# kanyu369/ADNM-UNet

Measured on AMD Instinct MI355X. Metric: sequences/sec training ADNM-UNet 5->20x128x128, higher is better.
Workload: dtype bf16; 1 GPU; ADNM-UNet create_ADNMUNet(5,20,6) 128x128 full training step (fwd + enRainfallLoss + bwd + clip_grad_norm_ + AdamW), recipe parameters, synthetic radar frames in HBM; per_gpu_batch=4, global_batch=4, frames=5->20, parallelism=single, launch=hipGraph replay

## Files before the change

adnm-unet_amd/adnm_hip/ops.py:

```python
import math
import os
import threading

import torch

from . import lib

_DT = {torch.float32: lib.F32, torch.bfloat16: lib.BF16}

MFMA_PREC = [0]
_PREC_NAMES = {"f32": 0, "fp32": 0, "bf16": 1, "fp8": 2}


def set_mfma_precision(name):
    MFMA_PREC[0] = _PREC_NAMES[name]


def mfma_precision():
    return ("f32", "bf16", "fp8")[MFMA_PREC[0]]


class QuantTable:
    CAP = 2048

# ... 623 lines not shown
                row = ent["rows"][k]
                if row < 0:
                    return None
                return ent["shadow"].data_ptr() + off, 2, QUANT.scale_b_view(ent["dev"], row)
        return None


FOLDS = FoldRegistry()
SPLITWS = SplitWorkspaces()
SHADOWS = ShadowRegistry()
GRADS = GradRegistry()
SIDE = SideStreams()
grad_dst = GRADS.take


class _NoDefer:
    def deferring(self):
        return False

    def __enter__(self):
        return False

    def __exit__(self, *exc):
        return False


_NODEFER = _NoDefer()


def _need_gpu(t):
    if not t.is_cuda:
        raise RuntimeError("adnm_hip kernels run on the GPU only (there is no CPU fallback); got a CPU tensor")


def k_rownorm_fwd(x2, w, b, scale, shift, eps, mean, out=None):
    _need_gpu(x2)
    M, d = x2.shape
    y = out if out is not None else torch.empty((M, d), dtype=x2.dtype, device=x2.device)
    mu = torch.empty(M if mean else 1, dtype=torch.float32, device=x2.device)
    rstd = torch.empty(M, dtype=torch.float32, device=x2.device)
    px, ldx = _rows(x2)
    py, ldy = _rows(y)
    lib.call("adnm_rownorm_fwd", px, ldx, _p(_f32(w)), _p(_f32(b)), _p(scale), _p(shift), py, ldy, mu.data_ptr(),
             rstd.data_ptr(), M, d, float(eps), int(mean), _dt(x2), _stream())
    return y, mu, rstd


def k_rownorm_bwd(dy2, x2, w, b, scale, mu, rstd, mean, want_b, want_affine, dx_out=None, dres=None, shift=None, defer=False):
    M, d = x2.shape
    dev = x2.device
    dx = dx_out if dx_out is not None else torch.empty((M, d), dtype=x2.dtype, device=dev)
    dw = grad_dst(w.data_ptr(), (d,), dev)
    db = grad_dst(b.data_ptr(), (d,), dev) if want_b else None
    dsc = grad_dst(scale.data_ptr() if scale is not None else 0, (), dev) if want_affine else None
    dsh = grad_dst(shift.data_ptr() if shift is not None else 0, (), dev) if want_affine else None
    nb = lib.query("adnm_rownorm_bwd_ws_bytes", M, d)
    ws = _ws(nb, dev)
    pdy, lddy = _rows(dy2)
    px, ldx = _rows(x2)
    pdx, lddx = _rows(dx)
    pres, ldres = _rows(dres) if dres is not None else (None, 0)
    with FOLDS.defer(dev, ws) if defer else _NODEFER:
        lib.call("adnm_rownorm_bwd", pdy, lddy, px, ldx, _p(w), _p(b), _p(scale), mu.data_ptr(), rstd.data_ptr(), pdx, lddx,
                 dw.data_ptr(), _p(db), _p(dsc), _p(dsh), pres, ldres, ws.data_ptr(), nb, M, d, int(mean), _dt(x2), _stream())
    return dx, dw, db, dsc, dsh


def k_ssd_fwd(x, Bm, Cm, dt_raw, dt_bias, A_log, D, B, L, H, P, N, G, y=None, ln=None):
    _need_gpu(x)
    dev = x.device
    M = B * L
    if y is None:
        y = torch.empty((M, H * P), dtype=x.dtype, device=dev)
    kv = torch.empty((B, H, N, P), dtype=torch.float32, device=dev)
    nb = lib.query("adnm_ssd_ws_bytes", B, L, H, P, N, G)
    ws = _ws(nb, dev)
    px, ldx = _rows(x)
    pb, ldb = _rows(Bm)
    pc, ldc = _rows(Cm)
    pt, ldt = _rows(dt_raw)
    py, ldy = _rows(y)
    if ln is not None:
        lw, lb, yn, eps = ln
        mu = torch.empty(M, dtype=torch.float32, device=dev)
        rstd = torch.empty(M, dtype=torch.float32, device=dev)
        pn, ldn = _rows(yn)
        extra = (_p(_f32(lw)), _p(_f32(lb)), pn, ldn, mu.data_ptr(), rstd.data_ptr(), float(eps))
    else:
        extra = (None, None, None, 0, None, None, 0.0)
    lib.call("adnm_ssd_reduce_fwd", px, ldx, pb, ldb, pc, ldc, pt, ldt, 1, _p(_f32(dt_bias)), _p(_f32(A_log)), _p(_f32(D)), 1, py,
             ldy, kv.data_ptr(), *extra, ws.data_ptr(), nb, B, L, H, P, N, G, _dt(x), _stream())
    return (y, kv, mu, rstd) if ln is not None else (y, kv)


def k_ssd_bwd(dy, x, Bm, Cm, dt_raw, dt_bias, A_log, D, kv, dx, dBm, dCm, ddt, B, L, H, P, N, G):
    dev = x.device
    dbias = torch.empty(H, dtype=torch.float32, device=dev)
    dA = torch.empty(H, dtype=torch.float32, device=dev)
    dD = torch.empty(H, dtype=torch.float32, device=dev)
    nb = lib.query("adnm_ssd_ws_bytes", B, L, H, P, N, G)
    ws = _ws(nb, dev)
    a = []
    for t in (dy, x, Bm, Cm, dt_raw):
        a += list(_rows(t))
    g = []
    for t in (dx, dBm, dCm, ddt):
        g += list(_rows(t))
    with FOLDS.defer(dev, ws):
        lib.call("adnm_ssd_reduce_bwd", a[0], a[1], a[2], a[3], a[4], a[5], a[6], a[7], a[8], a[9], 1, _p(dt_bias), _p(A_log), _p(D), 1,
                 kv.data_ptr(), g[0], g[1], g[2], g[3], g[4], g[5], g[6], g[7], dbias.data_ptr(), dA.data_ptr(), dD.data_ptr(),
                 ws.data_ptr(), nb, B, L, H, P, N, G, _dt(x), _stream())
    return dbias, dA, dD


def k_dwconv_fwd(x, wt, bias, B, H, W, C, K, act, y=None, addend=None, chan_major=False):
    _need_gpu(x)
    if y is None:
        y = torch.empty((B * H * W, C), dtype=x.dtype, device=x.device)
    px, ldx = _rows(x)
    py, ldy = _rows(y)
    pa, lda = _rows(addend) if addend is not None else (None, 0)
    lib.call("adnm_dwconv_fwd", px, ldx, _p(_f32(wt)), _p(_f32(bias)), pa, lda, py, ldy, B, H, W, C, K, K, act, int(chan_major), _dt(x), _stream())
    return y


def k_dwconv_bwd(dy, x, wt, bias, B, H, W, C, K, act, dx=None, want_bias=False, want_w=True, chan_major=False, want_dx=True):
    dev = x.device
    if not want_dx:
        assert act == lib.ACT_NONE and want_w
    if dx is None and want_dx:
        dx = torch.empty((B * H * W, C), dtype=x.dtype, device=dev)
    dwt = torch.empty((C, K * K) if chan_major else (K * K, C), dtype=torch.float32, device=dev) if want_w else None
    db = torch.empty(C, dtype=torch.float32, device=dev) if want_bias else None
    dpre = torch.empty((B * H * W, C), dtype=x.dtype, device=dev) if act != lib.ACT_NONE else None
    nb = lib.query("adnm_dwconv_bwd_ws_bytes", B, H, W, C, K, K)
    ws = _ws(nb, dev)
    pdy, lddy = _rows(dy)
    px, ldx = _rows(x)
    pdx, lddx = _rows(dx) if dx is not None else (None, 0)
    if not want_w:
        lib.call("adnm_dwconv_bwd", pdy, lddy, px, ldx, _p(wt), _p(bias), _p(dpre), pdx, lddx, None, None, ws.data_ptr(),
                 nb, B, H, W, C, K, K, act, int(chan_major), _dt(x), _stream())
        return dx, dwt, db
    if want_dx:
        lib.call("adnm_dwconv_bwd", pdy, lddy, px, ldx, _p(wt), _p(bias), _p(dpre), pdx, lddx, None, None, ws.data_ptr(),
                 nb, B, H, W, C, K, K, act, int(chan_major), _dt(x), _stream())
    g, ldg = (dpre.data_ptr(), C) if dpre is not None else (pdy, lddy)
    pdw, pdb, dt_ = _p(dwt), _p(db), _dt(x)
    SIDE.submit(dev, (dy, x, dpre), FOLDS.defer(dev, ws, dy, x, dpre), lambda: lib.call(
        "adnm_dwconv_wgrad", g, ldg, px, ldx, pdw, pdb, ws.data_ptr(), nb, B, H, W, C, K, K, int(chan_major), dt_, _stream()))
    return dx, dwt, db


def k_haar_dwt(x, B, H, W, C, cx=1):
    _need_gpu(x)
    h2, w2 = (H + 1) // 2, (W + 1) // 2
    y = torch.empty((B * h2 * w2, 4 * C), dtype=x.dtype, device=x.device)
    px, ldx = _rows(x)
    lib.call("adnm_haar_dwt", px, ldx, cx, y.data_ptr(), B, H, W, C, _dt(x), _stream())
    return y


def k_wt_level(x, B, H, W, C, cx, taps, K, flip=False):
    _need_gpu(x)
    h2, w2 = (H + 1) // 2, (W + 1) // 2
    sub = torch.empty((B * h2 * w2, 4 * C), dtype=torch.float32, device=x.device)
    tag = torch.empty_like(sub)
    px, ldx = _rows(x)
    lib.call("adnm_wt_level", px, ldx, cx, _f32(taps).data_ptr(), sub.data_ptr(), tag.data_ptr(), B, H, W, C, K, int(flip), _stream())
    return sub, tag


def k_haar_idwt(s, ll_add, B, H, W, C, y_add=(), up=()):
    _need_gpu(s)
    assert s.is_contiguous() and (ll_add is None or ll_add.is_contiguous()) and len(up) <= 2 and all(u.is_contiguous() and u.dtype == s.dtype for u in up)
    adds = [a if a.is_contiguous() else a.contiguous() for a in y_add if a is not None]
    assert len(adds) <= 2
    adds += [None] * (2 - len(adds))
    ups = list(up) + [None] * (2 - len(up))
    y = torch.empty((B * H * W, C), dtype=s.dtype, device=s.device)
    lib.call("adnm_haar_idwt", s.data_ptr(), _p(ups[0]), _p(ups[1]), _p(ll_add), _p(adds[0]), _p(adds[1]), y.data_ptr(), B, H, W, C, _dt(s), _stream())
    return y


def k_haar_synthesis(bands, shapes, B, C, y_add=()):
    n = len(bands)
    nxt, top = None, n
    while top > 0:
        lo = max(top - 3, 0)
        hh, ww = shapes[lo]
        nxt = k_haar_idwt(bands[lo], nxt, B, hh, ww, C, y_add=y_add if lo == 0 else (), up=tuple(bands[lo + 1:top]))
        top = lo
    return nxt


def k_instnorm_fwd(x, scale, shift, B, HW, C, eps, act):
    _need_gpu(x)
    assert x.is_contiguous()
    dev = x.device
    y = torch.empty_like(x)
    mu = torch.empty((B, C), dtype=torch.float32, device=dev)
    rstd = torch.empty((B, C), dtype=torch.float32, device=dev)
    nb = lib.query("adnm_instnorm_ws_bytes", B, HW, C)
    ws = _ws(nb, dev)
    lib.call("adnm_instnorm_fwd", x.data_ptr(), _p(scale), _p(shift), y.data_ptr(), mu.data_ptr(), rstd.data_ptr(), ws.data_ptr(), nb,
             B, HW, C, float(eps), act, _dt(x), _stream())
    return y, mu, rstd


def k_instnorm_bwd(dy, x, scale, shift, mu, rstd, B, HW, C, act, want_affine=True):
    dev = x.device
    assert dy.is_contiguous() and x.is_contiguous()
    dx = torch.empty_like(x)
    dsc = grad_dst(scale.data_ptr() if scale is not None else 0, (), dev) if want_affine else None
    dsh = grad_dst(shift.data_ptr() if shift is not None else 0, (), dev) if want_affine else None
    nb = lib.query("adnm_instnorm_ws_bytes", B, HW, C)
    ws = _ws(nb, dev)
    with FOLDS.defer(dev, ws):
        lib.call("adnm_instnorm_bwd", dy.data_ptr(), x.data_ptr(), _p(scale), _p(shift), mu.data_ptr(), rstd.data_ptr(), dx.data_ptr(),
                 _p(dsc), _p(dsh), ws.data_ptr(), nb, B, HW, C, act, _dt(x), _stream())
    return dx, dsc, dsh


def k_gate_fwd(h, F):
    _need_gpu(h)
    M = h.shape[0]
    y = torch.empty((M, F), dtype=h.dtype, device=h.device)
    ph, ldh = _rows(h)
    lib.call("adnm_gate_fwd", ph, ldh, y.data_ptr(), F, M, F, _dt(h), _stream())
    return y


def k_gate_bwd(dy, h, F):
    M = h.shape[0]
    dh = torch.empty((M, 2 * F), dtype=h.dtype, device=h.device)
    pdy, lddy = _rows(dy)
    ph, ldh = _rows(h)
    lib.call("adnm_gate_bwd", pdy, lddy, ph, ldh, dh.data_ptr(), 2 * F, M, F, _dt(h), _stream())
    return dh


def tap_major(w):
    c = w.shape[0]
    return w.reshape(c, -1).t().contiguous().float()


class RowNormFn(torch.autograd.Function):

    @staticmethod
    def forward(ctx, x, w, b, scale, shift, eps, mean):
        shp = x.shape
        x2 = x.reshape(-1, shp[-1])
        if x2.stride(-1) != 1:
            x2 = x2.contiguous()
        y, mu, rstd = k_rownorm_fwd(x2, w, b, scale, shift, eps, mean)
        ctx.save_for_backward(x2, w, b, scale, mu, rstd)
        ctx.mean, ctx.shp, ctx.has_shift, ctx.shift = mean, shp, shift is not None, shift
        return y.view(shp)

    @staticmethod
    def backward(ctx, dy):
        x2, w, b, scale, mu, rstd = ctx.saved_tensors
        dy2 = dy.reshape(-1, ctx.shp[-1])
        if dy2.stride(-1) != 1:
            dy2 = dy2.contiguous()
        dx, dw, db, dsc, dsh = k_rownorm_bwd(dy2, x2, w, b, scale, mu, rstd, ctx.mean, b is not None,
                                            scale is not None or ctx.has_shift, shift=ctx.shift, defer=True)
        return (dx.view(ctx.shp), dw, db, dsc if scale is not None else None, dsh if ctx.has_shift else None, None, None)


def rownorm(x, w, b=None, scale=None, shift=None, eps=1e-5, mean=True):
    return RowNormFn.apply(x, w, b, scale, shift, eps, mean)


class RowNormTapFn(torch.autograd.Function):

    @staticmethod
    def forward(ctx, x, w, b, scale, shift, eps, mean):
        shp = x.shape
        x2 = x.reshape(-1, shp[-1])
        if x2.stride(-1) != 1:
            x2 = x2.contiguous()
        y, mu, rstd = k_rownorm_fwd(x2, w, b, scale, shift, eps, mean)
        ctx.save_for_backward(x2, w, b, scale, mu, rstd)
        ctx.mean, ctx.shp, ctx.has_shift, ctx.shift = mean, shp, shift is not None, shift
        ctx.set_materialize_grads(False)
        return y.view(shp), x

    @staticmethod
    def backward(ctx, dy, dres):
        x2, w, b, scale, mu, rstd = ctx.saved_tensors
        d = ctx.shp[-1]
        if dy is None:
            return (dres, None, None, None, None, None, None)
        dy2 = dy.reshape(-1, d)
        if dy2.stride(-1) != 1:
            dy2 = dy2.contiguous()
        if dres is not None:
            dres = dres.reshape(-1, d)
            if dres.stride(-1) != 1:
                dres = dres.contiguous()
        dx, dw, db, dsc, dsh = k_rownorm_bwd(dy2, x2, w, b, scale, mu, rstd, ctx.mean, b is not None,
                                            scale is not None or ctx.has_shift, dres=dres, shift=ctx.shift, defer=True)
        return (dx.view(ctx.shp), dw, db, dsc if scale is not None else None, dsh if ctx.has_shift else None, None, None)


def rownorm_tap(x, w, b=None, scale=None, shift=None, eps=1e-5, mean=True):
    return RowNormTapFn.apply(x, w, b, scale, shift, eps, mean)


class CatMixFn(torch.autograd.Function):

    @staticmethod
    def forward(ctx, x, r, f, a1, a2, a3, a4):
        shp = x.shape
        d = shp[-1]
        rows = lambda t: t.reshape(-1, d) if t.reshape(-1, d).stride(-1) == 1 else t.reshape(-1, d).contiguous()
        x2, r2 = rows(x), rows(r)
        f2 = rows(f) if f is not None else None
        _need_gpu(x2)
        M = x2.shape[0]
        y = torch.empty((M, 2 * d), dtype=x.dtype, device=x.device)
        (px, ldx), (pr, ldr) = _rows(x2), _rows(r2)
        pf, ldf = _rows(f2) if f2 is not None else (None, 0)
        lib.call("adnm_catmix_fwd", px, ldx, pr, ldr, pf, ldf, _p(a1), _p(a2), _p(a3), _p(a4), y.data_ptr(), M, d, _dt(y), _stream())
        ctx.save_for_backward(x2, r2, f2, a1, a2, a3, a4)
        ctx.shp = shp
        return y.view(*shp[:-1], 2 * d)

    @staticmethod
    def backward(ctx, dy):
        x2, r2, f2, a1, a2, a3, a4 = ctx.saved_tensors
        M, d = x2.shape
        g = dy.reshape(M, 2 * d)
        g = g if g.stride(-1) == 1 else g.contiguous()
        need = ctx.needs_input_grad
        mk = lambda on: torch.empty((M, d), dtype=x2.dtype, device=x2.device) if on else None
        dx, dr, df = mk(need[0]), mk(need[1]), mk(need[2] and f2 is not None)
        da = torch.empty(4, dtype=torch.float32, device=x2.device)
        nb = lib.query("adnm_catmix_bwd_ws_bytes", M, d)
        ws = _ws(nb, x2.device)
        (pg, ldg), (px, ldx), (pr, ldr) = _rows(g), _rows(x2), _rows(r2)
        pf, ldf = _rows(f2) if f2 is not None else (None, 0)
        with FOLDS.defer(x2.device, ws):
            lib.call("adnm_catmix_bwd", pg, ldg, px, ldx, pr, ldr, pf, ldf, _p(a1), _p(a2), _p(a3), _p(a4), _p(dx), _p(dr), _p(df), da.data_ptr(),
                     ws.data_ptr(), nb, M, d, _dt(g), _stream())
        v = lambda t: t.view(ctx.shp) if t is not None else None
        s = lambda a, i: da[i].view_as(a) if a is not None else None
        return v(dx), v(dr), v(df), s(a1, 0), s(a2, 1), s(a3 if f2 is not None else None, 2), s(a4 if f2 is not None else None, 3)


def _unsupported(op, why):
    raise RuntimeError(f"adnm_hip {op}: {why} (the HIP path has no PyTorch fallback)")


def catmix(x, r, f, a1, a2, a3=None, a4=None):
    _need_gpu(x)
    d = x.shape[-1]
    if r.shape != x.shape or (f is not None and f.shape != x.shape):
        _unsupported("catmix", f"operands must share one shape, got {tuple(x.shape)}, {tuple(r.shape)}" + (f", {tuple(f.shape)}" if f is not None else ""))
    if d % 4 or x.dtype not in _DT or any(a is not None and a.numel() != 1 for a in (a1, a2, a3, a4)):
        _unsupported("catmix", f"needs a channel count that is a multiple of 4 (got {d}), fp32/bf16 tokens and 1-element mixing parameters")
    return CatMixFn.apply(x, r, f, a1, a2, a3, a4)


class SSDReduceFn(torch.autograd.Function):

    @staticmethod
    def forward(ctx, x, Bm, Cm, dt_raw, dt_bias, A_log, D, G):
        B, L, H, P = x.shape
        N = Bm.shape[-1] // G
        M = B * L
        xs, bs, cs, ts = x.reshape(M, H * P), Bm.reshape(M, -1), Cm.reshape(M, -1), dt_raw.reshape(M, H)
        xs, bs, cs, ts = [t if t.stride(-1) == 1 else t.contiguous() for t in (xs, bs, cs, ts)]
        y, kv = k_ssd_fwd(xs, bs, cs, ts, dt_bias, A_log, D, B, L, H, P, N, G)
        ctx.save_for_backward(xs, bs, cs, ts, dt_bias, A_log, D, kv)
        ctx.dims = (B, L, H, P, N, G)
        return y.view(B, L, H, P)

    @staticmethod
    def backward(ctx, dy):
        xs, bs, cs, ts, dt_bias, A_log, D, kv = ctx.saved_tensors
        B, L, H, P, N, G = ctx.dims
        M = B * L
        dy2 = dy.reshape(M, H * P)
        dy2 = dy2 if dy2.stride(-1) == 1 else dy2.contiguous()
        dx, dB, dC, ddt = (torch.empty_like(t, memory_format=torch.contiguous_format) for t in (xs, bs, cs, ts))
        dbias, dA, dD = k_ssd_bwd(dy2, xs, bs, cs, ts, dt_bias, A_log, D, kv, dx, dB, dC, ddt, B, L, H, P, N, G)
        return dx.view(B, L, H, P), dB.view(B, L, -1), dC.view(B, L, -1), ddt.view(B, L, H), dbias, dA, dD, None


def ssd_reduce(x, Bm, Cm, dt_raw, dt_bias, A_log, D, groups=1):
# ... 129 lines not shown
            else:
                dm = k_haar_dwt(cur, B, hh, ww, C, cx)
            dtags.append(dm)
            cur, cx = dm, 4
        dlw = [None] * levels
        for i in range(levels - 1, -1, -1):
            hh, ww = shapes[i]
            h2, w2 = (hh + 1) // 2, (ww + 1) // 2
            if fused:
                _, dlw[i], _ = k_dwconv_bwd(dtags[i], subs[i], level_wt[i], None, B, h2, w2, 4 * C, K, lib.ACT_NONE, want_dx=False)
            else:
                dsub, dlw[i], _ = k_dwconv_bwd(dtags[i], subs[i], level_wt[i], None, B, h2, w2, 4 * C, K, lib.ACT_NONE, want_dx=need_dx)
                dsubs.insert(0, dsub)
        if not need_dx:
            dx = None
        elif levels == 0:
            dx = dxb if dalias is None else dxb + dalias.reshape(B * H * W, C)
        else:
            dx = k_haar_synthesis(dsubs, shapes, B, C, y_add=(dxb, dalias.reshape(B * H * W, C) if dalias is not None else None))
        return (dx.view(B, H * W, C) if dx is not None else None, None, None, None, dbase, dbb, *dlw)


def wtconv(x, H, W, K, base_wt, base_bias, level_wts, tap=False):
    y, xa = WTConvFn.apply(x, H, W, K, base_wt, base_bias, *level_wts)
    return (y, xa) if tap else y


class ADNMixerFn(torch.autograd.Function):

    @staticmethod
    def forward(ctx, u, w_in, taps, tb, dt_bias, A_log, D, ln_w, ln_b, w_out, H, W, P, N, scan_chunk=0, scan_groups=2, qkeys=(None, None),
                narrow=(None, None, None, None)):
        n_in = (narrow[0].data_ptr(), 1 if narrow[0].dtype == torch.bfloat16 else 2, narrow[1]) if narrow[0] is not None else None
        n_out = (narrow[2].data_ptr(), 1 if narrow[2].dtype == torch.bfloat16 else 2, narrow[3]) if narrow[2] is not None else None
        Bsz, L, dm = u.shape
        M = Bsz * L
        di = w_out.shape[1] // 2
        cx = taps.shape[1] - di
        nh = di // P
        u2 = u.reshape(M, dm)
        u2 = u2 if u2.is_contiguous() else u2.contiguous()
        st = low_storage(M, [(w_in.shape[0], dm), (dm, 2 * di), (2 * di, dm), (dm, w_in.shape[0])]) if scan_chunk == 0 else u.dtype
        proj = k_linear(u2, w_in, None, qkey=qkeys[0], out_dtype=st, narrow=n_in)
        wide = torch.empty((M, 2 * di + cx), dtype=st, device=u.device)
        cat, xbc = wide[:, :2 * di], wide[:, 2 * di:]
        k_dwconv_fwd(proj[:, :di + cx], taps, tb, Bsz, H, W, di + cx, 3, lib.ACT_SILU, y=wide[:, di:])
        if scan_chunk == 0:
            if di == 64:
                y, kv, mu, rstd = k_ssd_fwd(xbc[:, :di], xbc[:, di:di + 2 * N], xbc[:, di + 2 * N:], proj[:, di + cx:], dt_bias, A_log, D,
                                            Bsz, L, nh, P, N, 2, ln=(ln_w, ln_b, cat[:, :di], 1e-5))
            else:
                y, kv = k_ssd_fwd(xbc[:, :di], xbc[:, di:di + 2 * N], xbc[:, di + 2 * N:], proj[:, di + cx:], dt_bias, A_log, D,
                                  Bsz, L, nh, P, N, 2)
                mu = None
        else:
            y = torch.empty((M, di), dtype=u.dtype, device=u.device)
            Ns = N // scan_groups
            kv = torch.stack([k_ssd_scan_fwd(xbc[:, e * P:di], 2 * P, xbc[:, di + e * N:di + (e + 1) * N], xbc[:, di + 2 * N + e * N:di + 2 * N + (e + 1) * N],
                                             proj[:, di + cx + e:], 2, dt_bias[e:], A_log[e:], D[e:], 2, y[:, e * P:], 2 * P, Bsz, L, nh // 2, P, Ns,
                                             scan_groups, scan_chunk, e == 1) for e in (0, 1)])
            mu = None
        if mu is None:
            _, mu, rstd = k_rownorm_fwd(y, ln_w, ln_b, None, None, 1e-5, True, out=cat[:, :di])
        out = k_linear(cat, w_out, None, qkey=qkeys[1], out_dtype=u.dtype, narrow=n_out)
        ctx.save_for_backward(u2, w_in, taps, tb, dt_bias, A_log, D, ln_w, ln_b, w_out, proj, wide, y, kv, mu, rstd)
        ctx.dims = (Bsz, L, dm, H, W, P, N, di, cx, nh, scan_chunk, scan_groups)
        ctx.qkeys = qkeys
        ctx.narrow = (n_in, n_out, narrow)
        return out.view(Bsz, L, dm)

    @staticmethod
    def backward(ctx, dout):
        (u2, w_in, taps, tb, dt_bias, A_log, D, ln_w, ln_b, w_out, proj, wide, y, kv, mu, rstd) = ctx.saved_tensors
        Bsz, L, dm, H, W, P, N, di, cx, nh, scan_chunk, scan_groups = ctx.dims
        M = Bsz * L
        cat, xbc = wide[:, :2 * di], wide[:, 2 * di:]
        do = dout.reshape(M, dm)
        do = do if do.is_contiguous() else do.contiguous()
        dw_out, _ = k_linear_dw(do, cat, False)
        dwide = torch.empty_like(wide)
        dcat, dxbc = dwide[:, :2 * di], dwide[:, 2 * di:]
        k_linear_dx(do, w_out, out=dcat, qkey=ctx.qkeys[1], narrow=ctx.narrow[1])
        dy, dln_w, dln_b, _, _ = k_rownorm_bwd(dcat[:, :di], y, ln_w, ln_b, None, mu, rstd, True, True, False, defer=True)
        dproj = torch.empty_like(proj)
        if scan_chunk == 0:
            ddtb, dA, dD = k_ssd_bwd(dy, xbc[:, :di], xbc[:, di:di + 2 * N], xbc[:, di + 2 * N:], proj[:, di + cx:], dt_bias, A_log, D, kv,
                                     dxbc[:, :di], dxbc[:, di:di + 2 * N], dxbc[:, di + 2 * N:], dproj[:, di + cx:], Bsz, L, nh, P, N, 2)
        else:
            Ns = N // scan_groups
            parts = [k_ssd_scan_bwd(dy[:, e * P:], 2 * P, xbc[:, e * P:di], 2 * P, xbc[:, di + e * N:di + (e + 1) * N],
                                    xbc[:, di + 2 * N + e * N:di + 2 * N + (e + 1) * N], proj[:, di + cx + e:], 2, dt_bias[e:], A_log[e:], D[e:], 2,
                                    kv[e], dxbc[:, e * P:di], 2 * P, dxbc[:, di + e * N:di + (e + 1) * N],
                                    dxbc[:, di + 2 * N + e * N:di + 2 * N + (e + 1) * N], dproj[:, di + cx + e:], 2, Bsz, L, nh // 2, P, Ns,
                                    scan_groups, scan_chunk, e == 1) for e in (0, 1)]
            ddtb, dA, dD = (torch.stack((parts[0][k], parts[1][k]), dim=1).reshape(nh) for k in range(3))
        _, dtaps, dtb = k_dwconv_bwd(dwide[:, di:], proj[:, :di + cx], taps, tb, Bsz, H, W, di + cx, 3, lib.ACT_SILU, dx=dproj[:, :di + cx],
                                     want_bias=tb is not None)
        du = k_linear_dx(dproj, w_in, qkey=ctx.qkeys[0], out_dtype=u2.dtype, narrow=ctx.narrow[0])
        dw_in, _ = k_linear_dw(dproj, u2, False)
        return (du.view(Bsz, L, dm), dw_in, dtaps, dtb, ddtb, dA, dD, dln_w, dln_b, dw_out, None, None, None, None, None, None, None, None)


def adn_mixer(u, w_in, taps, tb, dt_bias, A_log, D, ln_w, ln_b, w_out, H, W, P, N, scan_chunk=0, scan_groups=2, qkeys=(None, None),
              narrow=(None, None, None, None)):
    return ADNMixerFn.apply(u, w_in, taps, tb, dt_bias, A_log, D, ln_w, ln_b, w_out, H, W, P, N, scan_chunk, scan_groups, qkeys, narrow)


class FeedForwardFn(torch.autograd.Function):

    @staticmethod
    def forward(ctx, x, w_in, b_in, dw, b_dw, w_out, b_out, H, W):
        B, L, d = x.shape
        M = B * L
        F4, F2 = w_in.shape[0], w_out.shape[1]
        x2 = x.reshape(M, d)
        x2 = x2 if x2.is_contiguous() else x2.contiguous()
        w_in, w_out = w_in.contiguous(), w_out.contiguous()
        wt = dw.reshape(F4, 9)
        if wt.dtype != torch.float32 or not wt.is_contiguous():
            wt = wt.contiguous().float()
        st = low_storage(M, [(F4, d), (d, F4), (d, F2), (F2, d)])
        h1 = k_linear(x2, w_in, b_in, out_dtype=st)
        h2 = k_dwconv_fwd(h1, wt, b_dw, B, H, W, F4, 3, lib.ACT_NONE, chan_major=True)
        g = k_gate_fwd(h2, F2)
        out = k_linear(g, w_out, b_out, out_dtype=x.dtype)
        ctx.save_for_backward(x2, w_in, b_in, wt, b_dw, w_out, b_out, h1, h2, g)
        ctx.meta = (B, L, d, H, W, F4, F2, dw.shape)
        return out.view(B, L, w_out.shape[0])

    @staticmethod
    def backward(ctx, dout):
        x2, w_in, b_in, wt, b_dw, w_out, b_out, h1, h2, g = ctx.saved_tensors
        B, L, d, H, W, F4, F2, dwshape = ctx.meta
        M = B * L
        do = dout.reshape(M, w_out.shape[0])
        do = do if do.is_contiguous() else do.contiguous()
        dg = k_linear_dx(do, w_out, out_dtype=g.dtype)
        dw_out, db_out = k_linear_dw(do, g, b_out is not None, w_out.data_ptr(), b_out.data_ptr() if b_out is not None else 0)
        dh2 = k_gate_bwd(dg, h2, F2)
        dh1, dwt, db_dw = k_dwconv_bwd(dh2, h1, wt, b_dw, B, H, W, F4, 3, lib.ACT_NONE, want_bias=b_dw is not None, chan_major=True)
        dx = k_linear_dx(dh1, w_in, out_dtype=x2.dtype) if ctx.needs_input_grad[0] else None
        dw_in, db_in = k_linear_dw(dh1, x2, b_in is not None, w_in.data_ptr(), b_in.data_ptr() if b_in is not None else 0)
        return (dx.view(B, L, d) if dx is not None else None, dw_in, db_in, dwt.view(dwshape), db_dw, dw_out, db_out, None, None)


def feedforward(x, w_in, b_in, dw, b_dw, w_out, b_out, H, W):
    _need_gpu(x)
    F4, F2 = w_in.shape[0], w_out.shape[1]
    if (x.dtype != torch.float32 or x.dim() != 3 or x.shape[1] != H * W or F4 != 2 * F2 or F2 % 4 or tuple(dw.shape) != (F4, 1, 3, 3)
            or w_in.shape[1] != x.shape[-1]):
        _unsupported("feedforward", f"is 1x1 d->4d, depthwise 3x3, gelu*sigmoid gate, 1x1 2d->d on fp32 (B, H*W, d) tokens with 8 | 4d, got "
                                    f"{x.dtype} {tuple(x.shape)}, weights {tuple(w_in.shape)}, {tuple(dw.shape)}, {tuple(w_out.shape)}")
    return FeedForwardFn.apply(x, w_in, b_in, dw, b_dw, w_out, b_out, H, W)


class LinCombFn(torch.autograd.Function):

    @staticmethod
    def forward(ctx, gamma, *args):
        n = len(args) // 2
        xs, ss = args[:n], args[n:]
        shp = xs[0].shape
        C = shp[-1]
        x2 = []
        for x in xs:
            t = x.reshape(-1, C)
            x2.append(t if t.stride(-1) == 1 else t.contiguous())
        M = x2[0].shape[0]
        y = torch.empty((M, C), dtype=xs[0].dtype, device=xs[0].device)
        ptr = [(None, 0)] * 3
        for i, t in enumerate(x2):
            ptr[i] = _rows(t)
        sp = [_p(s) for s in ss] + [None] * (3 - n)
        _need_gpu(x2[0])
        lib.call("adnm_lincomb_fwd", ptr[0][0], ptr[0][1], ptr[1][0], ptr[1][1], ptr[2][0], ptr[2][1], sp[0], sp[1], sp[2], _p(gamma),
                 y.data_ptr(), C, M, C, _dt(y), _stream())
        ctx.save_for_backward(gamma, *x2, *[s for s in ss if s is not None])
        ctx.meta = (n, shp, [s is not None for s in ss])
        return y.view(shp)

    @staticmethod
    def backward(ctx, dy):
        n, shp, has_s = ctx.meta
        saved = ctx.saved_tensors
        gamma, x2 = saved[0], saved[1:1 + n]
        it = iter(saved[1 + n:])
        ss = [next(it) if h else None for h in has_s]
        C = shp[-1]
        M = x2[0].shape[0]
        dev = x2[0].device
        g = dy.reshape(M, C)
        g = g if g.stride(-1) == 1 else g.contiguous()
        need_x = ctx.needs_input_grad[1:1 + n]
        dxs = [torch.empty((M, C), dtype=x2[0].dtype, device=dev) if need_x[i] else None for i in range(n)]
        dss, accmask = [], 0
        for i in range(n):
            if ss[i] is None:
                dss.append(None)
                continue
            t, acc = GRADS.take_accumulating(ss[i].data_ptr(), ss[i].shape, dev)
            dss.append(t)
            accmask |= (1 << (1 + i)) if acc else 0
        dgamma = grad_dst(gamma.data_ptr(), gamma.shape, dev) if gamma is not None else None
        nb = lib.query("adnm_lincomb_bwd_ws_bytes", M, C)
        ws = _ws(nb, dev)
        xp = [_rows(t) for t in x2] + [(None, 0)] * (3 - n)
        dxp = [(_p(t), C) for t in dxs] + [(None, 0)] * (3 - n)
        sp = [_p(s) for s in ss] + [None] * (3 - n)
        dsp = [_p(s) for s in dss] + [None] * (3 - n)
        pg, ldg = _rows(g)
        with FOLDS.defer(dev, ws) as deferred:
            if accmask:
                assert deferred, "an accumulating gradient claim needs the deferred fold queue"
                lib.load().adnm_foldq_accumulate_next(accmask)
            lib.call("adnm_lincomb_bwd", pg, ldg, xp[0][0], xp[0][1], xp[1][0], xp[1][1], xp[2][0], xp[2][1], sp[0], sp[1], sp[2], _p(gamma),
                     dxp[0][0], dxp[0][1], dxp[1][0], dxp[1][1], dxp[2][0], dxp[2][1], dsp[0], dsp[1], dsp[2], _p(dgamma), ws.data_ptr(), nb,
                     M, C, _dt(g), _stream())
        return (dgamma, *[d.view(shp) if d is not None else None for d in dxs],
                *[None if (accmask >> (1 + i)) & 1 else d for i, d in enumerate(dss)])


def lincomb(xs, scalars, gamma=None):
    C = xs[0].shape[-1]
    _need_gpu(xs[0])
    if gamma is None and C % 4 and xs[0].numel() % 4 == 0 and all(x.shape == xs[0].shape and x.is_contiguous() for x in xs):
        shp = xs[0].shape
        return lincomb([x.view(-1, 4) for x in xs], scalars).view(shp)
    if C % 4 or C > 2048 or not 1 <= len(xs) <= 3 or any(s is not None and s.numel() != 1 for s in scalars):
        _unsupported("lincomb", f"needs 1-3 operands with 4 | C <= 2048 channels and 1-element scalars, got {len(xs)} operands, C={C}")
    return LinCombFn.apply(gamma, *xs, *scalars)


class MixNormFn(torch.autograd.Function):

    @staticmethod
    def forward(ctx, gamma, w, b, scale, shift, eps, mean, x0, x1, s0, s1):
        shp = x0.shape
        d = shp[-1]
        rows = lambda t: t.reshape(-1, d) if t.reshape(-1, d).stride(-1) == 1 else t.reshape(-1, d).contiguous()
        a2, b2 = rows(x0), rows(x1)
        _need_gpu(a2)
        M, dev = a2.shape[0], a2.device
        x = torch.empty((M, d), dtype=torch.float32, device=dev)
        xn = torch.empty((M, d), dtype=torch.float32, device=dev)
        mu = torch.empty(M, dtype=torch.float32, device=dev) if mean else None
        rstd = torch.empty(M, dtype=torch.float32, device=dev)
        (pa, lda), (pb, ldb) = _rows(a2), _rows(b2)
        lib.call("adnm_mixnorm_fwd", pa, lda, pb, ldb, _p(s0), _p(s1), _p(gamma), w.data_ptr(), _p(b), _p(scale), _p(shift), x.data_ptr(), d,
                 xn.data_ptr(), d, _p(mu), rstd.data_ptr(), M, d, float(eps), int(mean), _stream())
        ctx.save_for_backward(gamma, w, b, scale, a2, b2, s0, s1, mu, rstd)
        ctx.meta = (shp, mean, shift)
        ctx.set_materialize_grads(False)
        return xn.view(shp), x.view(shp)

    @staticmethod
    def backward(ctx, dxn, dres):
        gamma, w, b, scale, a2, b2, s0, s1, mu, rstd = ctx.saved_tensors
        shp, mean, shift = ctx.meta
        M, d = a2.shape
        dev = a2.device
        rows = lambda t: t.reshape(M, d) if t.reshape(M, d).stride(-1) == 1 else t.reshape(M, d).contiguous()
        if dxn is None:
            dxn = torch.zeros((M, d), dtype=torch.float32, device=dev)
        dxn = rows(dxn)
        dres = rows(dres) if dres is not None else None
        need = ctx.needs_input_grad
        dx0 = torch.empty((M, d), dtype=torch.float32, device=dev) if need[7] else None
        dx1 = torch.empty((M, d), dtype=torch.float32, device=dev) if need[8] else None
        dss, accmask = [], 0
        for i, sk in enumerate((s0, s1)):
            if sk is None:
                dss.append(None)
                continue
            t, acc = GRADS.take_accumulating(sk.data_ptr(), sk.shape, dev)
            dss.append(t)
            accmask |= (1 << (1 + i)) if acc else 0
        dgamma = grad_dst(gamma.data_ptr(), gamma.shape, dev) if gamma is not None else None
        dw = grad_dst(w.data_ptr(), (d,), dev)
        db = grad_dst(b.data_ptr(), (d,), dev) if b is not None else None
        affine = scale is not None or shift is not None
        dsc = grad_dst(scale.data_ptr() if scale is not None else 0, (), dev) if affine else None
        dsh = grad_dst(shift.data_ptr() if shift is not None else 0, (), dev) if affine else None
        nb = lib.query("adnm_mixnorm_bwd_ws_bytes", M, d)
        ws = _ws(nb, dev)
        (pg, ldg), (pa, lda), (pb, ldb) = _rows(dxn), _rows(a2), _rows(b2)
        pr, ldr = _rows(dres) if dres is not None else (None, 0)
        with FOLDS.defer(dev, ws) as deferred:
            if accmask:
                assert deferred, "an accumulating gradient claim needs the deferred fold queue"
                lib.load().adnm_foldq_accumulate_next(accmask)
            lib.call("adnm_mixnorm_bwd", pg, ldg, pr, ldr, pa, lda, pb, ldb, _p(s0), _p(s1), _p(gamma), w.data_ptr(), _p(b), _p(scale), _p(mu),
                     rstd.data_ptr(), _p(dx0), d, _p(dx1), d, _p(dss[0]), _p(dss[1]), _p(dgamma), dw.data_ptr(), _p(db), _p(dsc), _p(dsh),
                     ws.data_ptr(), nb, M, d, int(mean), _stream())
        ds = [None if (accmask >> (1 + i)) & 1 else t for i, t in enumerate(dss)]
        return (dgamma, dw, db, dsc if scale is not None else None, dsh if shift is not None else None, None, None,
                dx0.view(shp) if dx0 is not None else None, dx1.view(shp) if dx1 is not None else None, ds[0], ds[1])


def mixnorm(xs, scalars, gamma, w, b=None, scale=None, shift=None, eps=1e-5, mean=True):
    _need_gpu(xs[0])
    d = xs[0].shape[-1]
    if (len(xs) != 2 or xs[0].shape != xs[1].shape or any(x.dtype != torch.float32 for x in xs) or d % 4 or d > 1024
            or any(sk is not None and sk.numel() != 1 for sk in scalars)):
        _unsupported("mixnorm", f"mixes two same-shape fp32 token tensors with 4 | d <= 1024 channels and 1-element scalars, got "
                                f"{[tuple(x.shape) for x in xs]} {[x.dtype for x in xs]}")
    return MixNormFn.apply(gamma, w, b, scale, shift, eps, mean, xs[0], xs[1], scalars[0], scalars[1])
# ... 1115 lines not shown
```

adnm-unet_amd/csrc/dwconv.hip:

```cpp
#include "adnm_common.h"

namespace {

constexpr int kBlock = 256;
constexpr int TW = 4;

__device__ __forceinline__ float4 f4zero() { return make_float4(0.f, 0.f, 0.f, 0.f); }
__device__ __forceinline__ void fma4(float4& a, const float4& w, const float4& x) {
  a.x = fmaf(w.x, x.x, a.x); a.y = fmaf(w.y, x.y, a.y); a.z = fmaf(w.z, x.z, a.z); a.w = fmaf(w.w, x.w, a.w);
}
__device__ __forceinline__ float4 apply_act(float4 v, int act) {
  if (act == ADNM_ACT_SILU) return make_float4(siluf_(v.x), siluf_(v.y), siluf_(v.z), siluf_(v.w));
  if (act == ADNM_ACT_GELU) return make_float4(geluf_(v.x), geluf_(v.y), geluf_(v.z), geluf_(v.w));
  return v;
}
__device__ __forceinline__ float4 apply_act_grad(float4 v, int act) {
  if (act == ADNM_ACT_SILU) return make_float4(silu_gradf_(v.x), silu_gradf_(v.y), silu_gradf_(v.z), silu_gradf_(v.w));
  if (act == ADNM_ACT_GELU) return make_float4(gelu_gradf_(v.x), gelu_gradf_(v.y), gelu_gradf_(v.z), gelu_gradf_(v.w));
  return make_float4(1.f, 1.f, 1.f, 1.f);
}

template <typename T>
struct CVec;
template <>
struct CVec<float> {
  static constexpr int N = 4, Q = 1;
  float4 q[1];
};
template <>
struct CVec<uint16_t> {
  static constexpr int N = 8, Q = 2;
  float4 q[2];
};
template <typename T>
__device__ __forceinline__ CVec<T> cv_zero() {
  CVec<T> v;
#pragma unroll
  for (int i = 0; i < CVec<T>::Q; ++i) v.q[i] = f4zero();
  return v;
}
__device__ __forceinline__ CVec<float> cv_ld(const float* p) {
  CVec<float> v;
  v.q[0] = *reinterpret_cast<const float4*>(p);
  return v;
}
__device__ __forceinline__ CVec<uint16_t> cv_ld(const uint16_t* p) {
  const uint4 r = *reinterpret_cast<const uint4*>(p);
  CVec<uint16_t> v;
  v.q[0] = make_float4(__uint_as_float(r.x << 16), __uint_as_float(r.x & 0xffff0000u), __uint_as_float(r.y << 16), __uint_as_float(r.y & 0xffff0000u));
  v.q[1] = make_float4(__uint_as_float(r.z << 16), __uint_as_float(r.z & 0xffff0000u), __uint_as_float(r.w << 16), __uint_as_float(r.w & 0xffff0000u));
  return v;
}
__device__ __forceinline__ void cv_st(float* p, const CVec<float>& v) { *reinterpret_cast<float4*>(p) = v.q[0]; }
__device__ __forceinline__ void cv_st(uint16_t* p, const CVec<uint16_t>& v) {
  uint4 r;
  r.x = (uint32_t)f32_to_bf16(v.q[0].x) | ((uint32_t)f32_to_bf16(v.q[0].y) << 16);
  r.y = (uint32_t)f32_to_bf16(v.q[0].z) | ((uint32_t)f32_to_bf16(v.q[0].w) << 16);
  r.z = (uint32_t)f32_to_bf16(v.q[1].x) | ((uint32_t)f32_to_bf16(v.q[1].y) << 16);
  r.w = (uint32_t)f32_to_bf16(v.q[1].z) | ((uint32_t)f32_to_bf16(v.q[1].w) << 16);
  *reinterpret_cast<uint4*>(p) = r;
}
template <typename T>
__device__ __forceinline__ CVec<T> cv_ldf(const float* p) {
  CVec<T> v;
#pragma unroll
  for (int i = 0; i < CVec<T>::Q; ++i) v.q[i] = *reinterpret_cast<const float4*>(p + 4 * i);
  return v;
}
template <typename T>
__device__ __forceinline__ void cv_stf(float* p, const CVec<T>& v) {
#pragma unroll
  for (int i = 0; i < CVec<T>::Q; ++i) *reinterpret_cast<float4*>(p + 4 * i) = v.q[i];
}
template <typename T>
__device__ __forceinline__ void cv_fma(CVec<T>& a, const CVec<T>& w, const CVec<T>& x) {
#pragma unroll
  for (int i = 0; i < CVec<T>::Q; ++i) fma4(a.q[i], w.q[i], x.q[i]);
}
template <typename T>
__device__ __forceinline__ void cv_add(CVec<T>& a, const CVec<T>& x) {
#pragma unroll
  for (int i = 0; i < CVec<T>::Q; ++i) a.q[i].x += x.q[i].x, a.q[i].y += x.q[i].y, a.q[i].z += x.q[i].z, a.q[i].w += x.q[i].w;
}

template <typename T, int K, int MODE, bool WCM>
__global__ __launch_bounds__(kBlock) void dwconv_kernel(const T* __restrict__ x, int64_t ldx, const float* __restrict__ wgt,
                                                        const float* __restrict__ bias, const T* __restrict__ aux,
                                                        int64_t ldaux, T* __restrict__ y, int64_t ldy, int B, int H, int W,
                                                        int C, int act) {
  constexpr int R = K / 2, N = CVec<T>::N, Q = CVec<T>::Q;
  using V = CVec<T>;
  const int C4 = C / N;
  const int WT = (W + TW - 1) / TW;
  const int64_t total = (int64_t)B * H * WT * C4;
  const unsigned nb = gridDim.x, q8 = nb >> 3, r8 = nb & 7, xcd = blockIdx.x & 7, loc = blockIdx.x >> 3;
  const unsigned bid = (xcd < r8 ? xcd * (q8 + 1) : r8 * (q8 + 1) + (xcd - r8) * q8) + loc;
  const int64_t idx = (int64_t)bid * kBlock + threadIdx.x;
  if (idx >= total) return;
  const int cg = (int)(idx % C4);
  int64_t t = idx / C4;
  const int wt = (int)(t % WT);
  t /= WT;
  const int h = (int)(t % H);
  const int b = (int)(t / H);
  const int c = cg * N;
  const int w0 = wt * TW;
  float wcmv[WCM ? N * K * K : 1];
  if (WCM) {
#pragma unroll
    for (int q = 0; q < N * K * K / 4; ++q) {
      const float4 t4 = *reinterpret_cast<const float4*>(wgt + (int64_t)c * (K * K) + 4 * q);
      wcmv[4 * q] = t4.x; wcmv[4 * q + 1] = t4.y; wcmv[4 * q + 2] = t4.z; wcmv[4 * q + 3] = t4.w;
    }
  }
  V acc[TW];
#pragma unroll
  for (int i = 0; i < TW; ++i) acc[i] = cv_zero<T>();
#pragma unroll
  for (int i = 0; i < K; ++i) {
    const int hh = h + i - R;
    if (hh < 0 || hh >= H) continue;
    const T* xr = x + ((int64_t)b * H + hh) * W * ldx + c;
    V row[TW + K - 1];
#pragma unroll
    for (int j = 0; j < TW + K - 1; ++j) {
      const int ww = w0 + j - R;
      row[j] = (ww >= 0 && ww < W) ? cv_ld(xr + (int64_t)ww * ldx) : cv_zero<T>();
    }
#pragma unroll
    for (int j = 0; j < K; ++j) {
      const int tap = (MODE == 2) ? ((K - 1 - i) * K + (K - 1 - j)) : (i * K + j);
      V wv;
      if (WCM) {
#pragma unroll
        for (int qq = 0; qq < Q; ++qq)
          wv.q[qq] = make_float4(wcmv[(WCM ? (4 * qq) * K * K : 0) + tap * WCM], wcmv[(WCM ? (4 * qq + 1) * K * K : 0) + tap * WCM],
                                 wcmv[(WCM ? (4 * qq + 2) * K * K : 0) + tap * WCM], wcmv[(WCM ? (4 * qq + 3) * K * K : 0) + tap * WCM]);
      } else {
        wv = cv_ldf<T>(wgt + (int64_t)tap * C + c);
      }
#pragma unroll
      for (int p = 0; p < TW; ++p) cv_fma(acc[p], wv, row[p + j]);
    }
  }
  V bv = cv_zero<T>();
  if (MODE != 2 && bias) bv = cv_ldf<T>(bias + c);
#pragma unroll
  for (int p = 0; p < TW; ++p) {
    const int ww = w0 + p;
    if (ww >= W) break;
    const int64_t pix = ((int64_t)b * H + h) * W + ww;
    V v = acc[p];
    if (MODE == 0) {
      cv_add(v, bv);
#pragma unroll
      for (int qq = 0; qq < Q; ++qq) v.q[qq] = apply_act(v.q[qq], act);
      if (aux) cv_add(v, cv_ld(aux + pix * ldaux + c));
    } else if (MODE == 1) {
      cv_add(v, bv);
      const V d = cv_ld(aux + pix * ldaux + c);
#pragma unroll
      for (int qq = 0; qq < Q; ++qq) {
        const float4 g = apply_act_grad(v.q[qq], act);
        v.q[qq] = make_float4(d.q[qq].x * g.x, d.q[qq].y * g.y, d.q[qq].z * g.z, d.q[qq].w * g.w);
      }
    }
    cv_st(y + pix * ldy + c, v);
  }
}

constexpr int kWgSlices = 2;

template <typename T, int K>
__device__ __forceinline__ void dwconv_wgrad_body(const T* __restrict__ dpre, int64_t ldd, const T* __restrict__ x, int64_t ldx,
                                                  float* __restrict__ part, int B, int H, int W, int C, int cgb, int wcm, const int bx,
                                                  const int by, const int nby) {
  constexpr int R = K / 2;
  constexpr int NT = K * K, N = CVec<T>::N;
  using V = CVec<T>;
  const int C4 = C / N;
  __shared__ __attribute__((aligned(16))) float red[K][K + 1][64][N];
  const int wv = threadIdx.x >> 6;
  const int i = wv % K;
  const int sl = wv / K;
  const int lane = threadIdx.x & 63;
  const int cgl = lane & (cgb - 1);
  const int slot = lane / cgb;
  const int slots = 64 / cgb;
  const int cg = bx * cgb + cgl;
  const bool cv = cg < C4;
  const int c = cv ? cg * N : 0;
  const int WT = (W + TW - 1) / TW;
  const int64_t tiles = (int64_t)B * H * WT;
  V aw[K];
  V ab = cv_zero<T>();
#pragma unroll
  for (int k = 0; k < K; ++k) aw[k] = cv_zero<T>();
  if (cv) {
    const unsigned nb = (unsigned)nby, q8 = nb >> 3, r8 = nb & 7, xcd = (unsigned)by & 7, loc = (unsigned)by >> 3;
    const int64_t bid = (xcd < r8 ? xcd * (q8 + 1) : r8 * (q8 + 1) + (xcd - r8) * q8) + loc;
    const int64_t tpb = (tiles + nb - 1) / nb;
    const int64_t tbeg = bid * tpb, tend = (tbeg + tpb < tiles) ? tbeg + tpb : tiles;
    const int64_t stride = (int64_t)slots * kWgSlices;
    for (int64_t t0 = tbeg + sl * slots + slot; t0 < tend; t0 += 2 * stride) {
      V g[2][TW], row[2][TW + K - 1];
      bool live[2];
#pragma unroll
      for (int u = 0; u < 2; ++u) {
        const int64_t t = t0 + u * stride;
        const int wt = (int)(t % WT);
        const int h = (int)((t / WT) % H);
        const int b = (int)(t / ((int64_t)WT * H));
        const int hh = h + i - R;
        live[u] = t < tend && hh >= 0 && hh < H;
        const int w0 = wt * TW;
#pragma unroll
        for (int p = 0; p < TW; ++p) {
          const int ww = w0 + p;
          g[u][p] = (live[u] && ww < W) ? cv_ld(dpre + (((int64_t)b * H + h) * W + ww) * ldd + c) : cv_zero<T>();
        }
        const T* xr = x + ((int64_t)b * H + (live[u] ? hh : 0)) * W * ldx + c;
#pragma unroll
        for (int j = 0; j < TW + K - 1; ++j) {
          const int ww = w0 + j - R;
          row[u][j] = (live[u] && ww >= 0 && ww < W) ? cv_ld(xr + (int64_t)ww * ldx) : cv_zero<T>();
        }
      }
#pragma unroll
      for (int u = 0; u < 2; ++u) {
        if (i == R) {
#pragma unroll
          for (int p = 0; p < TW; ++p) cv_add(ab, g[u][p]);
        }
#pragma unroll
        for (int j = 0; j < K; ++j)
#pragma unroll
          for (int p = 0; p < TW; ++p) cv_fma(aw[j], g[u][p], row[u][p + j]);
      }
    }
  }
#pragma unroll
  for (int j = 0; j <= K; ++j) {
    V& v = j < K ? aw[j] : ab;
#pragma unroll
    for (int qq = 0; qq < V::Q; ++qq) {
      v.q[qq].x = wave_sum_from(v.q[qq].x, cgb); v.q[qq].y = wave_sum_from(v.q[qq].y, cgb);
      v.q[qq].z = wave_sum_from(v.q[qq].z, cgb); v.q[qq].w = wave_sum_from(v.q[qq].w, cgb);
    }
  }
  if (sl == 1) {
#pragma unroll
    for (int j = 0; j <= K; ++j) cv_stf<T>(&red[i][j][lane][0], j < K ? aw[j] : ab);
  }
  __syncthreads();
  if (sl == 0) {
    float* dst = part + (int64_t)by * (NT + 1) * C;
#pragma unroll
    for (int j = 0; j <= K; ++j) {
      if (j == K && i != R) break;
      V v = j < K ? aw[j] : ab;
      cv_add(v, cv_ldf<T>(&red[i][j][lane][0]));
      if (lane < cgb && cv) {
        if (wcm && j < K) {
          float* q = dst + (int64_t)c * NT + i * K + j;
#pragma unroll
          for (int qq = 0; qq < V::Q; ++qq) {
            q[(4 * qq) * NT] = v.q[qq].x; q[(4 * qq + 1) * NT] = v.q[qq].y; q[(4 * qq + 2) * NT] = v.q[qq].z; q[(4 * qq + 3) * NT] = v.q[qq].w;
          }
        } else {
          cv_stf<T>(dst + (int64_t)(j < K ? i * K + j : NT) * C + c, v);
        }
      }
    }
  }
}

template <typename T, int K>
__global__ __launch_bounds__(64 * K * kWgSlices) void dwconv_wgrad_kernel(const T* __restrict__ dpre, int64_t ldd, const T* __restrict__ x,
                                                              int64_t ldx, float* __restrict__ part, int B, int H, int W, int C,
                                                              int cgb, int wcm) {
  dwconv_wgrad_body<T, K>(dpre, ldd, x, ldx, part, B, H, W, C, cgb, wcm, (int)blockIdx.x, (int)blockIdx.y, (int)gridDim.y);
}

constexpr int kMaxWg = 16;
struct WgLeaf {
  const float* dpre;
  int64_t ldd;
  const float* x;
  int64_t ldx;
  float* part;
  int B, H, W, C, cgb, wcm, gx, npb;
};
struct MultiWg {
  int count, blk_end[kMaxWg];
  WgLeaf p[kMaxWg];
};
template <int K>
__global__ __launch_bounds__(64 * K * kWgSlices) void dwconv_wgrad_multi_kernel(MultiWg by_value) {
  (void)by_value;
  const auto& m = *(const __attribute__((address_space(4))) MultiWg*)__builtin_amdgcn_kernarg_segment_ptr();
  int k = 0;
  while (k + 1 < m.count && (int)blockIdx.x >= m.blk_end[k]) ++k;
  const int lin = (int)blockIdx.x - (k ? m.blk_end[k - 1] : 0);
  const int gx = m.p[k].gx;
  dwconv_wgrad_body<float, K>(m.p[k].dpre, m.p[k].ldd, m.p[k].x, m.p[k].ldx, m.p[k].part, m.p[k].B, m.p[k].H, m.p[k].W, m.p[k].C, m.p[k].cgb,
                              m.p[k].wcm, lin % gx, lin / gx, m.p[k].npb);
}

template <typename T>
__global__ __launch_bounds__(kBlock) void dwconv_wgrad3_roll_kernel(const T* __restrict__ dpre, int64_t ldd, const T* __restrict__ x, int64_t ldx,
                                                                    float* __restrict__ part, int B, int H, int W, int C, int cgb, int SEG,
                                                                    int nseg, int wcm) {
  constexpr int K = 3, NT = 9, N = CVec<T>::N;
  using V = CVec<T>;
  __shared__ __attribute__((aligned(16))) float red[kBlock / 64 - 1][NT + 1][64][N];
  const int C4 = C / N;
  const int WT = (W + TW - 1) / TW;
  const int cgl = threadIdx.x & (cgb - 1), sp = threadIdx.x / cgb, spb = kBlock / cgb;
  const int cg = blockIdx.x * cgb + cgl;
  const int64_t S = (int64_t)B * nseg * WT, sidx = (int64_t)blockIdx.y * spb + sp;
  const bool cv = cg < C4, live = cv && sidx < S;
// ... 144 lines not shown
  float* dst = part + (int64_t)by * (NT + 1) * C;
#pragma unroll
  for (int k = 0; k <= NT; ++k) {
    float4 v = k < NT ? aw[k] : ab;
    v.x = wave_sum_from(v.x, cgb), v.y = wave_sum_from(v.y, cgb), v.z = wave_sum_from(v.z, cgb), v.w = wave_sum_from(v.w, cgb);
    if (wave > 0) *reinterpret_cast<float4*>(&red[wave - 1][lane][0]) = v;
    __syncthreads();
    if (wave == 0 && lane < cgb) {
#pragma unroll
      for (int wv = 0; wv < kBlock / 64 - 1; ++wv) {
        const float4 o = *reinterpret_cast<const float4*>(&red[wv][lane][0]);
        v.x += o.x, v.y += o.y, v.z += o.z, v.w += o.w;
      }
      if (cv) {
        if (wcm && k < NT) {
          float* q = dst + (int64_t)c * NT + k;
          q[0] = v.x, q[NT] = v.y, q[2 * NT] = v.z, q[3 * NT] = v.w;
        } else {
          *reinterpret_cast<float4*>(dst + (int64_t)k * C + c) = v;
        }
      }
    }
    __syncthreads();
  }
}

__global__ __launch_bounds__(kBlock) void dwconv_wgrad5_walk_kernel(const float* __restrict__ dpre, int64_t ldd, const float* __restrict__ x, int64_t ldx,
                                                                    float* __restrict__ part, int B, int H, int W, int C, int cgb, int SEG, int nseg,
                                                                    int wcm) {
  dwconv_wgrad_walk_body<5, kWalkTW>(dpre, ldd, x, ldx, part, B, H, W, C, cgb, SEG, nseg, wcm, (int)blockIdx.x, (int)blockIdx.y);
}

struct WalkLeaf {
  const float* dpre;
  int64_t ldd;
  const float* x;
  int64_t ldx;
  float* part;
  int B, H, W, C, cgb, wcm, gx, npb, seg, nseg;
};
struct MultiWalk {
  int count, blk_end[kMaxWg];
  WalkLeaf p[kMaxWg];
};
__global__ __launch_bounds__(kBlock) void dwconv_wgrad5_walk_multi_kernel(MultiWalk by_value) {
  (void)by_value;
  const auto& m = *(const __attribute__((address_space(4))) MultiWalk*)__builtin_amdgcn_kernarg_segment_ptr();
  int k = 0;
  while (k + 1 < m.count && (int)blockIdx.x >= m.blk_end[k]) ++k;
  const int lin = (int)blockIdx.x - (k ? m.blk_end[k - 1] : 0);
  const int gx = m.p[k].gx;
  dwconv_wgrad_walk_body<5, kWalkTW>(m.p[k].dpre, m.p[k].ldd, m.p[k].x, m.p[k].ldx, m.p[k].part, m.p[k].B, m.p[k].H, m.p[k].W, m.p[k].C, m.p[k].cgb,
                                     m.p[k].seg, m.p[k].nseg, m.p[k].wcm, lin % gx, lin / gx);
}

struct WGeo {
  int cgb, gx, npb, rows;
  int seg, nseg;
};
WGeo wgeo(int64_t B, int64_t H, int64_t W, int64_t C, int K, int cn = 4) {
  WGeo g;
  const int64_t C4 = C / cn;
  g.cgb = 1;
  while (g.cgb < 64 && g.cgb < C4) g.cgb <<= 1;
  g.gx = (int)adnm_cdiv(C4, g.cgb);
  const int slots = 64 / g.cgb;
  const int64_t tiles = B * H * adnm_cdiv(W, TW);
  static const int grouped_tpl = [] {
    const char* e = getenv("ADNM_DW_WG_TPL");
    const int v = e ? atoi(e) : 0;
    return v > 0 ? v : 16;
  }();
  const bool walker = K == 3 && H * W >= 128 * 128;
  const int64_t tmax = !walker && adnm_leafq_active() ? grouped_tpl : 8;
  int64_t tpl = (tiles * g.gx) / ((int64_t)slots * 256);
  if (tmax > 8 && tpl >= 8) tpl = tmax;
  tpl = tpl < 2 ? 2 : (tpl > tmax ? tmax : tpl);
  int64_t npb = adnm_cdiv(tiles, (int64_t)slots * tpl);
  int64_t cap = (4 << 20) / ((int64_t)(K * K + 1) * C * 4);
  if (cap > 1024) cap = 1024;
  if (cap < 32) cap = 32;
  if (npb > cap) npb = cap;
  if (npb < 1) npb = 1;
  g.npb = (int)npb;
  g.rows = g.npb;
  g.seg = g.nseg = 0;
  if (walker) {
    const int64_t WT = adnm_cdiv(W, TW);
    int64_t seg = (H * B * WT * C4) / 65536;
    seg = seg < 2 ? 2 : (seg > 16 ? 16 : seg);
    if (seg > H) seg = H;
    g.seg = (int)seg;
    g.nseg = (int)adnm_cdiv(H, seg);
    const int64_t S = B * g.nseg * WT;
    g.npb = (int)adnm_cdiv(S, kBlock / g.cgb);
    g.rows = g.npb;
  }
  return g;
}

WGeo wgeo_walk5(int64_t B, int64_t H, int64_t W, int64_t C) {
  WGeo g;
  const int64_t C4 = C / 4;
  g.cgb = 1;
  while (g.cgb < 64 && g.cgb < C4) g.cgb <<= 1;
  g.gx = (int)adnm_cdiv(C4, g.cgb);
  const int64_t WT = adnm_cdiv(W, kWalkTW);
  static const int seg_min = [] {
    const char* e = getenv("ADNM_DW_WALK_SEG");
    const int v = e ? atoi(e) : 0;
    return v > 0 ? v : 16;
  }();
  int64_t seg = (H * B * WT * C4) / 65536;
  seg = seg < seg_min ? seg_min : (seg > 64 ? 64 : seg);
  if (seg > H) seg = H;
  g.seg = (int)seg;
  g.nseg = (int)adnm_cdiv(H, seg);
  g.npb = (int)adnm_cdiv(B * g.nseg * WT, kBlock / g.cgb);
  g.rows = g.npb;
  return g;
}

int check(const char* who, const void* x, int64_t B, int64_t H, int64_t W, int64_t C, int KH, int KW, int act, int dtype) {
  ADNM_REQUIRE(x, "%s: null pointer", who);
  ADNM_REQUIRE(B > 0 && H > 0 && W > 0 && C > 0 && C % 4 == 0, "%s: shape B=%lld H=%lld W=%lld C=%lld (C must be a multiple of 4)", who,
               (long long)B, (long long)H, (long long)W, (long long)C);
  ADNM_REQUIRE(KH == KW && (KH == 3 || KH == 5), "%s: kernel %dx%d not in {3x3, 5x5}", who, KH, KW);
  ADNM_REQUIRE(act >= ADNM_ACT_NONE && act <= ADNM_ACT_GELU, "%s: bad activation %d", who, act);
  ADNM_REQUIRE(dtype == ADNM_F32 || dtype == ADNM_BF16, "%s: bad dtype %d", who, dtype);
  ADNM_REQUIRE(dtype == ADNM_F32 || C % 8 == 0, "%s: bf16 tokens move 8 channels (16 bytes) per lane: C=%lld must be a multiple of 8", who, (long long)C);
  ADNM_REQUIRE(B * H * W * C < (1ll << 40), "%s: tensor too large", who);
  return ADNM_OK;
}

template <typename T, int MODE>
void launch_conv(const void* x, int64_t ldx, const float* wgt, const float* bias, const void* aux, int64_t ldaux, void* y, int64_t ldy,
                 int64_t B, int64_t H, int64_t W, int64_t C, int K, int act, int wcm, hipStream_t st) {
  const int64_t total = B * H * adnm_cdiv(W, TW) * (C / CVec<T>::N);
  const unsigned grid = (unsigned)adnm_cdiv(total, kBlock);
#define ADNM_DWCONV(KK, WCMV)                                                                                                       \
  dwconv_kernel<T, KK, MODE, WCMV><<<grid, kBlock, 0, st>>>((const T*)x, ldx, wgt, bias, (const T*)aux, ldaux, (T*)y, ldy, (int)B, (int)H, \
                                                            (int)W, (int)C, act)
  ADNM_PROF(K == 3 ? "dwconv_k3" : "dwconv_k5", st, (double)sizeof(T) * B * H * W * C * (MODE == 1 ? 3 : (aux ? 3 : 2)));
  if (K == 3) {
    if (wcm) ADNM_DWCONV(3, true);
    else ADNM_DWCONV(3, false);
  } else {
    if (wcm) ADNM_DWCONV(5, true);
    else ADNM_DWCONV(5, false);
  }
#undef ADNM_DWCONV
}

template <typename T>
void launch_wgrad(const void* dpre, int64_t ldd, const void* x, int64_t ldx, float* part, float* dwgt, float* dbias, int64_t B, int64_t H,
                  int64_t W, int64_t C, int K, int wcm, hipStream_t st) {
  if (K == 5 && sizeof(T) == 4) {
    const WGeo g = wgeo_walk5(B, H, W, C);
    static_assert(sizeof(WalkLeaf) <= sizeof(AdnmLeaf::args), "WalkLeaf must fit a leaf record");
    WalkLeaf w{(const float*)dpre, ldd, (const float*)x, ldx, part, (int)B, (int)H, (int)W, (int)C, g.cgb, wcm, g.gx, g.npb, g.seg, g.nseg};
    AdnmLeaf leaf;
    leaf.kind = ADNM_LEAF_DWCONV_WGRAD_K5, leaf.grid = g.gx * g.npb, leaf.prec = 0, leaf.prof = "dwconv_wgrad_k5", leaf.bytes = 4.0 * B * H * W * C * 2;
    memcpy(leaf.args, &w, sizeof(w));
    if (!adnm_leafq_push(leaf)) {
      ADNM_PROF("dwconv_wgrad_k5", st, 4.0 * B * H * W * C * 2);
      dwconv_wgrad5_walk_kernel<<<dim3(g.gx, g.npb), kBlock, 0, st>>>((const float*)dpre, ldd, (const float*)x, ldx, part, (int)B, (int)H, (int)W, (int)C, g.cgb,
                                                                     g.seg, g.nseg, wcm);
    }
    adnm_launch_fold("dwconv_wgrad_fold", part, g.rows, 26 * (int)C, {dwgt, 25 * (int)C}, {dbias, (int)C}, {nullptr, 0}, {nullptr, 0}, st);
    return;
  }
  const WGeo g = wgeo(B, H, W, C, K, CVec<T>::N);
  const dim3 grid(g.gx, g.npb);
  if (K == 3 && g.seg > 0)
    { ADNM_PROF("dwconv_wgrad_k3", st, (double)sizeof(T) * B * H * W * C * 2); dwconv_wgrad3_roll_kernel<T><<<grid, kBlock, 0, st>>>((const T*)dpre, ldd, (const T*)x, ldx, part, (int)B, (int)H, (int)W, (int)C, g.cgb, g.seg, g.nseg, wcm); }
  else {
    bool queued = false;
    if (sizeof(T) == 4) {
      static_assert(sizeof(WgLeaf) <= sizeof(AdnmLeaf::args), "WgLeaf must fit a leaf record");
      WgLeaf w{(const float*)dpre, ldd, (const float*)x, ldx, part, (int)B, (int)H, (int)W, (int)C, g.cgb, wcm, (int)g.gx, (int)g.npb};
      AdnmLeaf leaf;
      leaf.kind = K == 3 ? ADNM_LEAF_DWCONV_WGRAD_K3 : ADNM_LEAF_DWCONV_WGRAD_K5, leaf.grid = (int)(g.gx * g.npb), leaf.prec = 0;
      leaf.prof = K == 3 ? "dwconv_wgrad_k3" : "dwconv_wgrad_k5", leaf.bytes = 4.0 * B * H * W * C * 2;
      memcpy(leaf.args, &w, sizeof(w));
      queued = adnm_leafq_push(leaf);
    }
    if (!queued) {
      if (K == 3)
        { ADNM_PROF("dwconv_wgrad_k3", st, (double)sizeof(T) * B * H * W * C * 2); dwconv_wgrad_kernel<T, 3><<<grid, 64 * 3 * kWgSlices, 0, st>>>((const T*)dpre, ldd, (const T*)x, ldx, part, (int)B, (int)H, (int)W, (int)C, g.cgb, wcm); }
      else
        { ADNM_PROF("dwconv_wgrad_k5", st, (double)sizeof(T) * B * H * W * C * 2); dwconv_wgrad_kernel<T, 5><<<grid, 64 * 5 * kWgSlices, 0, st>>>((const T*)dpre, ldd, (const T*)x, ldx, part, (int)B, (int)H, (int)W, (int)C, g.cgb, wcm); }
    }
  }
  adnm_launch_fold("dwconv_wgrad_fold", part, g.rows, (K * K + 1) * (int)C, {dwgt, K * K * (int)C}, {dbias, (int)C}, {nullptr, 0}, {nullptr, 0}, st);
}

}

extern "C" int adnm_dwconv_fwd(const void* x, int64_t ldx, const float* wgt, const float* bias, const void* addend, int64_t ldadd,
                               void* y, int64_t ldy, int64_t B, int64_t H, int64_t W, int64_t C, int KH, int KW, int act, int wlayout,
                               int dtype, adnm_stream_t stream) {
  if (int rc = check("dwconv_fwd", x, B, H, W, C, KH, KW, act, dtype)) return rc;
  ADNM_REQUIRE(wgt && y, "dwconv_fwd: null pointer");
  ADNM_REQUIRE(wlayout == 0 || wlayout == 1, "dwconv_fwd: weight layout %d not in {0 tap-major, 1 channel-major}", wlayout);
  const int al = dtype == ADNM_BF16 ? 8 : 4;
  ADNM_REQUIRE(ldx >= C && ldy >= C && ldx % al == 0 && ldy % al == 0 && (!addend || (ldadd >= C && ldadd % al == 0)) &&
                   ((uintptr_t)x | (uintptr_t)y | (uintptr_t)addend) % 16 == 0,
               "dwconv_fwd: pixel strides must be >= C, rows and strides 16-byte aligned");
  hipStream_t st = (hipStream_t)stream;
  if (dtype == ADNM_F32) launch_conv<float, 0>(x, ldx, wgt, bias, addend, ldadd, y, ldy, B, H, W, C, KH, act, wlayout, st);
  else launch_conv<uint16_t, 0>(x, ldx, wgt, bias, addend, ldadd, y, ldy, B, H, W, C, KH, act, wlayout, st);
  ADNM_CHECK_LAUNCH("dwconv_fwd");
  return ADNM_OK;
}

extern "C" int64_t adnm_dwconv_bwd_ws_bytes(int64_t B, int64_t H, int64_t W, int64_t C, int KH, int KW) {
  if (B <= 0 || H <= 0 || W <= 0 || C < 4) return 0;
  int64_t rows = wgeo(B, H, W, C, KH).rows;
  if (C % 8 == 0) {
    const int64_t r8 = wgeo(B, H, W, C, KH, 8).rows;
    rows = r8 > rows ? r8 : rows;
  }
  if (KH == 5) {
    const int64_t r5 = wgeo_walk5(B, H, W, C).rows;
    rows = r5 > rows ? r5 : rows;
  }
  return rows * (KH * KW + 1) * C * (int64_t)sizeof(float);
}

extern "C" int adnm_dwconv_bwd(const void* dy, int64_t lddy, const void* x, int64_t ldx, const float* wgt, const float* bias,
                               void* dpre, void* dx, int64_t lddx, float* dwgt, float* dbias, void* ws, int64_t ws_bytes, int64_t B,
                               int64_t H, int64_t W, int64_t C, int KH, int KW, int act, int wlayout, int dtype, adnm_stream_t stream) {
  if (int rc = check("dwconv_bwd", x, B, H, W, C, KH, KW, act, dtype)) return rc;
  ADNM_REQUIRE(dy && wgt && dx, "dwconv_bwd: null pointer");
  ADNM_REQUIRE(wlayout == 0 || wlayout == 1, "dwconv_bwd: weight layout %d not in {0 tap-major, 1 channel-major}", wlayout);
  ADNM_REQUIRE(act == ADNM_ACT_NONE || dpre, "dwconv_bwd: dpre scratch required when an activation is fused");
  const int al = dtype == ADNM_BF16 ? 8 : 4;
  ADNM_REQUIRE(ldx >= C && lddy >= C && lddx >= C && ldx % al == 0 && lddy % al == 0 && lddx % al == 0 &&
                   ((uintptr_t)x | (uintptr_t)dy | (uintptr_t)dx | (uintptr_t)dpre) % 16 == 0,
               "dwconv_bwd: pixel strides must be >= C, rows and strides 16-byte aligned");
  if (!ws || ws_bytes < adnm_dwconv_bwd_ws_bytes(B, H, W, C, KH, KW)) {
    adnm_set_error("dwconv_bwd: workspace %lld < %lld bytes", (long long)ws_bytes, (long long)adnm_dwconv_bwd_ws_bytes(B, H, W, C, KH, KW));
    return ADNM_EWORKSPACE;
  }
  hipStream_t st = (hipStream_t)stream;
  const void* g = dy;
  int64_t ldg = lddy;
  if (dtype == ADNM_F32) {
    if (act != ADNM_ACT_NONE) {
      launch_conv<float, 1>(x, ldx, wgt, bias, dy, lddy, dpre, C, B, H, W, C, KH, act, wlayout, st);
      g = dpre; ldg = C;
    }
    launch_conv<float, 2>(g, ldg, wgt, nullptr, nullptr, 0, dx, lddx, B, H, W, C, KH, 0, wlayout, st);
    if (dwgt) launch_wgrad<float>(g, ldg, x, ldx, (float*)ws, dwgt, dbias, B, H, W, C, KH, wlayout, st);
  } else {
    if (act != ADNM_ACT_NONE) {
      launch_conv<uint16_t, 1>(x, ldx, wgt, bias, dy, lddy, dpre, C, B, H, W, C, KH, act, wlayout, st);
      g = dpre; ldg = C;
    }
    launch_conv<uint16_t, 2>(g, ldg, wgt, nullptr, nullptr, 0, dx, lddx, B, H, W, C, KH, 0, wlayout, st);
    if (dwgt) launch_wgrad<uint16_t>(g, ldg, x, ldx, (float*)ws, dwgt, dbias, B, H, W, C, KH, wlayout, st);
  }
  ADNM_CHECK_LAUNCH("dwconv_bwd");
  return ADNM_OK;
}

extern "C" int adnm_dwconv_wgrad(const void* g, int64_t ldg, const void* x, int64_t ldx, float* dwgt, float* dbias, void* ws, int64_t ws_bytes,
                                 int64_t B, int64_t H, int64_t W, int64_t C, int KH, int KW, int wlayout, int dtype, adnm_stream_t stream) {
  if (int rc = check("dwconv_wgrad", x, B, H, W, C, KH, KW, ADNM_ACT_NONE, dtype)) return rc;
  ADNM_REQUIRE(g && dwgt, "dwconv_wgrad: null pointer");
  ADNM_REQUIRE(wlayout == 0 || wlayout == 1, "dwconv_wgrad: weight layout %d not in {0 tap-major, 1 channel-major}", wlayout);
  const int al = dtype == ADNM_BF16 ? 8 : 4;
  ADNM_REQUIRE(ldx >= C && ldg >= C && ldx % al == 0 && ldg % al == 0 && ((uintptr_t)x | (uintptr_t)g) % 16 == 0,
               "dwconv_wgrad: pixel strides must be >= C, rows and strides 16-byte aligned");
  if (!ws || ws_bytes < adnm_dwconv_bwd_ws_bytes(B, H, W, C, KH, KW)) {
    adnm_set_error("dwconv_wgrad: workspace %lld < %lld bytes", (long long)ws_bytes, (long long)adnm_dwconv_bwd_ws_bytes(B, H, W, C, KH, KW));
    return ADNM_EWORKSPACE;
  }
  hipStream_t st = (hipStream_t)stream;
  if (dtype == ADNM_F32) launch_wgrad<float>(g, ldg, x, ldx, (float*)ws, dwgt, dbias, B, H, W, C, KH, wlayout, st);
  else launch_wgrad<uint16_t>(g, ldg, x, ldx, (float*)ws, dwgt, dbias, B, H, W, C, KH, wlayout, st);
  ADNM_CHECK_LAUNCH("dwconv_wgrad");
  return ADNM_OK;
}


int adnm_dwconv_wgrad_launch_multi(const AdnmLeaf* const* items, int n, int K, hipStream_t st) {
  if (K == 5) {
    for (int i = 0; i < n;) {
      MultiWalk m;
      m.count = 0;
      int blocks = 0;
      double bytes = 0;
      for (; i < n && m.count < kMaxWg; ++i) {
        memcpy(&m.p[m.count], items[i]->args, sizeof(WalkLeaf));
        blocks += items[i]->grid;
        m.blk_end[m.count++] = blocks;
        bytes += items[i]->bytes;
      }
      for (int k = m.count; k < kMaxWg; ++k) m.blk_end[k] = blocks;
      ADNM_PROF("dwconv_wgrad_k5", st, bytes);
      dwconv_wgrad5_walk_multi_kernel<<<(unsigned)blocks, kBlock, 0, st>>>(m);
    }
    ADNM_CHECK_LAUNCH("dwconv_wgrad (grouped)");
    return ADNM_OK;
  }
  for (int i = 0; i < n;) {
    MultiWg m;
    m.count = 0;
    int blocks = 0;
    double bytes = 0;
    for (; i < n && m.count < kMaxWg; ++i) {
      memcpy(&m.p[m.count], items[i]->args, sizeof(WgLeaf));
      blocks += items[i]->grid;
      m.blk_end[m.count++] = blocks;
      bytes += items[i]->bytes;
    }
    for (int k = m.count; k < kMaxWg; ++k) m.blk_end[k] = blocks;
    ADNM_PROF("dwconv_wgrad_k3", st, bytes);
    dwconv_wgrad_multi_kernel<3><<<(unsigned)blocks, 64 * 3 * kWgSlices, 0, st>>>(m);
  }
  ADNM_CHECK_LAUNCH("dwconv_wgrad (grouped)");
  return ADNM_OK;
}
```

adnm-unet_amd/csrc/elementwise.hip:

```cpp
#include "adnm_common.h"

namespace {
constexpr int kBlock = 256;

template <typename T>
__global__ __launch_bounds__(kBlock) void gate_fwd_kernel(const T* __restrict__ h, int64_t ldh, T* __restrict__ y, int64_t ldy,
                                                          int64_t M, int F) {
  const int F4 = F >> 2;
  const int64_t total = M * F4;
  for (int64_t i = (int64_t)blockIdx.x * kBlock + threadIdx.x; i < total; i += (int64_t)gridDim.x * kBlock) {
    const int64_t m = i / F4;
    const int f = (int)(i % F4) * 4;
    const float4 a = Io<T>::ld4(h + m * ldh + f), b = Io<T>::ld4(h + m * ldh + F + f);
    Io<T>::st4(y + m * ldy + f, make_float4(geluf_(a.x) * sigmoidf_(b.x), geluf_(a.y) * sigmoidf_(b.y), geluf_(a.z) * sigmoidf_(b.z),
                                            geluf_(a.w) * sigmoidf_(b.w)));
  }
}

template <typename T>
__global__ __launch_bounds__(kBlock) void gate_bwd_kernel(const T* __restrict__ dy, int64_t lddy, const T* __restrict__ h, int64_t ldh,
                                                          T* __restrict__ dh, int64_t lddh, int64_t M, int F) {
  const int F4 = F >> 2;
  const int64_t total = M * F4;
  for (int64_t i = (int64_t)blockIdx.x * kBlock + threadIdx.x; i < total; i += (int64_t)gridDim.x * kBlock) {
    const int64_t m = i / F4;
    const int f = (int)(i % F4) * 4;
    const float4 a = Io<T>::ld4(h + m * ldh + f), b = Io<T>::ld4(h + m * ldh + F + f), g = Io<T>::ld4(dy + m * lddy + f);
    const float av[4] = {a.x, a.y, a.z, a.w}, bv[4] = {b.x, b.y, b.z, b.w}, gv[4] = {g.x, g.y, g.z, g.w};
    float d1[4], d2[4];
#pragma unroll
    for (int k = 0; k < 4; ++k) {
      const float s = sigmoidf_(bv[k]);
      d1[k] = gv[k] * s * gelu_gradf_(av[k]);
      d2[k] = gv[k] * geluf_(av[k]) * s * (1.f - s);
    }
    Io<T>::st4(dh + m * lddh + f, make_float4(d1[0], d1[1], d1[2], d1[3]));
    Io<T>::st4(dh + m * lddh + F + f, make_float4(d2[0], d2[1], d2[2], d2[3]));
  }
}

template <typename T>
__global__ __launch_bounds__(kBlock) void igate_fwd_kernel(const T* __restrict__ x, const float* __restrict__ enh, const float* __restrict__ thr,
                                                           T* __restrict__ y, int64_t n4) {
  const float a = *enh, t = *thr;
  for (int64_t i = (int64_t)blockIdx.x * kBlock + threadIdx.x; i < n4; i += (int64_t)gridDim.x * kBlock) {
    const float4 v = Io<T>::ld4(x + i * 4);
    Io<T>::st4(y + i * 4, make_float4(siluf_(a * (v.x - t)), siluf_(a * (v.y - t)), siluf_(a * (v.z - t)), siluf_(a * (v.w - t))));
  }
}

template <typename T>
__global__ __launch_bounds__(kBlock) void igate_bwd_kernel(const T* __restrict__ dy, const T* __restrict__ x, const float* __restrict__ enh,
                                                           const float* __restrict__ thr, T* __restrict__ dx, float* __restrict__ part,
                                                           int64_t n4) {
  __shared__ float sm[2][kBlock / 64];
  const float a = *enh, t = *thr;
  float s1 = 0.f, s2 = 0.f;
  for (int64_t i = (int64_t)blockIdx.x * kBlock + threadIdx.x; i < n4; i += (int64_t)gridDim.x * kBlock) {
    const float4 v = Io<T>::ld4(x + i * 4), g = Io<T>::ld4(dy + i * 4);
    const float xv[4] = {v.x, v.y, v.z, v.w}, gv[4] = {g.x, g.y, g.z, g.w};
    float o[4];
#pragma unroll
    for (int k = 0; k < 4; ++k) {
      const float d = xv[k] - t, gp = gv[k] * silu_gradf_(a * d);
      o[k] = gp * a;
      s1 = fmaf(gp, d, s1);
      s2 += gp;
    }
    Io<T>::st4(dx + i * 4, make_float4(o[0], o[1], o[2], o[3]));
  }
  s1 = wave_sum(s1);
  s2 = wave_sum(s2);
  if ((threadIdx.x & 63) == 0) { sm[0][threadIdx.x >> 6] = s1; sm[1][threadIdx.x >> 6] = s2; }
  __syncthreads();
  if (threadIdx.x == 0) {
    part[blockIdx.x * 2] = (sm[0][0] + sm[0][1]) + (sm[0][2] + sm[0][3]);
    part[blockIdx.x * 2 + 1] = -a * ((sm[1][0] + sm[1][1]) + (sm[1][2] + sm[1][3]));
  }
}

template <typename T>
__global__ __launch_bounds__(kBlock) void catmix_fwd_kernel(const T* __restrict__ x, int64_t ldx, const T* __restrict__ r, int64_t ldr,
                                                            const T* __restrict__ f, int64_t ldf, const float* __restrict__ a1,
                                                            const float* __restrict__ a2, const float* __restrict__ a3,
                                                            const float* __restrict__ a4, T* __restrict__ y, int64_t M, int d) {
  const int d4 = d >> 2;
  const float s1 = a1 ? *a1 : 1.f, s2 = a2 ? *a2 : 1.f, s3 = (f && a3) ? *a3 : 1.f, s4 = (f && a4) ? *a4 : 1.f;
  for (int64_t i = (int64_t)blockIdx.x * kBlock + threadIdx.x; i < M * d4; i += (int64_t)gridDim.x * kBlock) {
    const int64_t m = i / d4;
    const int c = (int)(i % d4) * 4;
    const float4 xv = Io<T>::ld4(x + m * ldx + c), rv = Io<T>::ld4(r + m * ldr + c);
    float4 l = make_float4(s1 * xv.x, s1 * xv.y, s1 * xv.z, s1 * xv.w), q = make_float4(s2 * rv.x, s2 * rv.y, s2 * rv.z, s2 * rv.w);
    if (f) {
      const float4 fv = Io<T>::ld4(f + m * ldf + c);
      l = make_float4(fmaf(s3, fv.x, l.x), fmaf(s3, fv.y, l.y), fmaf(s3, fv.z, l.z), fmaf(s3, fv.w, l.w));
      q = make_float4(fmaf(s4, fv.x, q.x), fmaf(s4, fv.y, q.y), fmaf(s4, fv.z, q.z), fmaf(s4, fv.w, q.w));
    }
    Io<T>::st4(y + m * 2 * d + c, l);
    Io<T>::st4(y + m * 2 * d + d + c, q);
  }
}

template <typename T>
__global__ __launch_bounds__(kBlock) void catmix_bwd_kernel(const T* __restrict__ dy, int64_t lddy, const T* __restrict__ x, int64_t ldx,
                                                            const T* __restrict__ r, int64_t ldr, const T* __restrict__ f, int64_t ldf,
                                                            const float* __restrict__ a1, const float* __restrict__ a2,
                                                            const float* __restrict__ a3, const float* __restrict__ a4, T* __restrict__ dx,
                                                            T* __restrict__ dr, T* __restrict__ df, float* __restrict__ part, int64_t M, int d) {
  __shared__ float sm[4][kBlock / 64];
  const int d4 = d >> 2;
  const float s1 = a1 ? *a1 : 1.f, s2 = a2 ? *a2 : 1.f, s3 = (f && a3) ? *a3 : 1.f, s4 = (f && a4) ? *a4 : 1.f;
  float acc[4] = {0.f, 0.f, 0.f, 0.f};
  for (int64_t i = (int64_t)blockIdx.x * kBlock + threadIdx.x; i < M * d4; i += (int64_t)gridDim.x * kBlock) {
    const int64_t m = i / d4;
    const int c = (int)(i % d4) * 4;
    const float4 gl = Io<T>::ld4(dy + m * lddy + c), gr = Io<T>::ld4(dy + m * lddy + d + c);
    const float4 xv = Io<T>::ld4(x + m * ldx + c), rv = Io<T>::ld4(r + m * ldr + c);
    acc[0] += gl.x * xv.x + gl.y * xv.y + gl.z * xv.z + gl.w * xv.w;
    acc[1] += gr.x * rv.x + gr.y * rv.y + gr.z * rv.z + gr.w * rv.w;
    if (dx) Io<T>::st4(dx + m * d + c, make_float4(s1 * gl.x, s1 * gl.y, s1 * gl.z, s1 * gl.w));
    if (dr) Io<T>::st4(dr + m * d + c, make_float4(s2 * gr.x, s2 * gr.y, s2 * gr.z, s2 * gr.w));
    if (f) {
      const float4 fv = Io<T>::ld4(f + m * ldf + c);
      acc[2] += gl.x * fv.x + gl.y * fv.y + gl.z * fv.z + gl.w * fv.w;
      acc[3] += gr.x * fv.x + gr.y * fv.y + gr.z * fv.z + gr.w * fv.w;
      if (df)
        Io<T>::st4(df + m * d + c, make_float4(fmaf(s3, gl.x, s4 * gr.x), fmaf(s3, gl.y, s4 * gr.y), fmaf(s3, gl.z, s4 * gr.z),
                                               fmaf(s3, gl.w, s4 * gr.w)));
    }
  }
#pragma unroll
  for (int k = 0; k < 4; ++k) {
    acc[k] = wave_sum(acc[k]);
    if ((threadIdx.x & 63) == 0) sm[k][threadIdx.x >> 6] = acc[k];
  }
  __syncthreads();
  if (threadIdx.x < 4) part[blockIdx.x * 4 + threadIdx.x] = (sm[threadIdx.x][0] + sm[threadIdx.x][1]) + (sm[threadIdx.x][2] + sm[threadIdx.x][3]);
}

__global__ __launch_bounds__(kBlock) void rainloss_kernel(const float* __restrict__ pred, const float* __restrict__ tgt, float* __restrict__ grad,
                                                          float* __restrict__ part, int64_t n, float omega, float alpha, float gamma) {
  __shared__ float sm[kBlock / 64];
  const float inv_n = 1.0f / (float)n;
  float acc = 0.f;
  for (int64_t i = (int64_t)blockIdx.x * kBlock + threadIdx.x; i < n; i += (int64_t)gridDim.x * kBlock) {
    const float p = pred[i], t = tgt[i], diff = p - t;
    const bool over = p >= t, heavy = t >= 0.7f;
    const float w = over ? 1.0f - omega : omega;
    const float wi = heavy ? alpha * __expf(t) : 0.f;
    float e = w * fabsf(diff) * (1.0f + wi);
    float g = w * (1.0f + wi) * (diff > 0.f ? 1.f : (diff < 0.f ? -1.f : 0.f));
    if (gamma != 0.f && heavy && !over) {
      const float ex = __expf(alpha * (t - p));
      e += gamma * (ex - 1.0f);
      g -= gamma * alpha * ex;
    }
    acc += e;
    grad[i] = g * inv_n;
  }
  acc = wave_sum(acc);
  if ((threadIdx.x & 63) == 0) sm[threadIdx.x >> 6] = acc;
  __syncthreads();
  if (threadIdx.x == 0) part[blockIdx.x] = ((sm[0] + sm[1]) + (sm[2] + sm[3])) * inv_n;
}

constexpr int kC1Threads = 1024;
__global__ __launch_bounds__(kC1Threads) void conv1d3_kernel(const float* __restrict__ x, const float* __restrict__ w, const float* __restrict__ bias,
                                                             const float* __restrict__ dy, float* __restrict__ y, float* __restrict__ dx,
                                                             float* __restrict__ dwb, int B, int n) {
  __shared__ float sm[4][kC1Threads / 64];
  const float w0 = w[0], w1 = w[1], w2 = w[2], bv = bias ? bias[0] : 0.f;
  float a0 = 0.f, a1 = 0.f, a2 = 0.f, ab = 0.f;
  const int total = B * n;
  for (int base = threadIdx.x; base < total; base += 4 * kC1Threads) {
    float xm[4], xc[4], xp[4], gm[4], gc[4], gp[4];
#pragma unroll
    for (int u = 0; u < 4; ++u) {
      const int idx = base + u * kC1Threads, i = idx % n;
      const bool ok = idx < total;
      xm[u] = ok && i > 0 ? x[idx - 1] : 0.f;
      xc[u] = ok ? x[idx] : 0.f;
      xp[u] = ok && i + 1 < n ? x[idx + 1] : 0.f;
      if (dy) {
        gm[u] = ok && i > 0 ? dy[idx - 1] : 0.f;
        gc[u] = ok ? dy[idx] : 0.f;
        gp[u] = ok && i + 1 < n ? dy[idx + 1] : 0.f;
      }
    }
#pragma unroll
    for (int u = 0; u < 4; ++u) {
      const int idx = base + u * kC1Threads;
      if (idx >= total) break;
      if (!dy) {
        y[idx] = fmaf(w0, xm[u], fmaf(w1, xc[u], fmaf(w2, xp[u], bv)));
      } else {
        dx[idx] = fmaf(w0, gp[u], fmaf(w1, gc[u], w2 * gm[u]));
        a0 = fmaf(gc[u], xm[u], a0); a1 = fmaf(gc[u], xc[u], a1); a2 = fmaf(gc[u], xp[u], a2); ab += gc[u];
      }
    }
  }
  if (!dy) return;
  float acc[4] = {a0, a1, a2, ab};
#pragma unroll
  for (int k = 0; k < 4; ++k) {
    acc[k] = wave_sum(acc[k]);
    if ((threadIdx.x & 63) == 0) sm[k][threadIdx.x >> 6] = acc[k];
  }
  __syncthreads();
  if (threadIdx.x < 4) {
    float t = 0.f;
#pragma unroll
    for (int q = 0; q < kC1Threads / 64; ++q) t += sm[threadIdx.x][q];
    dwb[threadIdx.x] = t;
  }
}

unsigned grid_for(int64_t total) {
  int64_t g = adnm_cdiv(total, kBlock);
  return (unsigned)(g < 2048 ? (g < 1 ? 1 : g) : 2048);
}
}

extern "C" int adnm_gate_fwd(const void* h, int64_t ldh, void* y, int64_t ldy, int64_t M, int64_t F, int dtype, adnm_stream_t stream) {
  ADNM_REQUIRE(h && y, "gate_fwd: null pointer");
  ADNM_REQUIRE(M > 0 && F > 0 && F % 4 == 0 && ldh >= 2 * F && ldy >= F && ldh % 4 == 0 && ldy % 4 == 0, "gate_fwd: bad shape M=%lld F=%lld",
               (long long)M, (long long)F);
  ADNM_REQUIRE(dtype == ADNM_F32 || dtype == ADNM_BF16, "gate_fwd: bad dtype %d", dtype);
  hipStream_t st = (hipStream_t)stream;
  if (dtype == ADNM_F32) { ADNM_PROF("gate_fwd", st, 4.0 * M * F * 3); gate_fwd_kernel<float><<<grid_for(M * F / 4), kBlock, 0, st>>>((const float*)h, ldh, (float*)y, ldy, M, (int)F); }
  else { ADNM_PROF("gate_fwd", st, 2.0 * M * F * 3); gate_fwd_kernel<uint16_t><<<grid_for(M * F / 4), kBlock, 0, st>>>((const uint16_t*)h, ldh, (uint16_t*)y, ldy, M, (int)F); }
  ADNM_CHECK_LAUNCH("gate_fwd");
  return ADNM_OK;
}

extern "C" int adnm_gate_bwd(const void* dy, int64_t lddy, const void* h, int64_t ldh, void* dh, int64_t lddh, int64_t M, int64_t F,
                             int dtype, adnm_stream_t stream) {
  ADNM_REQUIRE(dy && h && dh, "gate_bwd: null pointer");
  ADNM_REQUIRE(M > 0 && F > 0 && F % 4 == 0 && ldh >= 2 * F && lddh >= 2 * F && lddy >= F && ldh % 4 == 0 && lddh % 4 == 0 && lddy % 4 == 0,
               "gate_bwd: bad shape M=%lld F=%lld", (long long)M, (long long)F);
  ADNM_REQUIRE(dtype == ADNM_F32 || dtype == ADNM_BF16, "gate_bwd: bad dtype %d", dtype);
  hipStream_t st = (hipStream_t)stream;
  if (dtype == ADNM_F32)
    { ADNM_PROF("gate_bwd", st, 4.0 * M * F * 5); gate_bwd_kernel<float><<<grid_for(M * F / 4), kBlock, 0, st>>>((const float*)dy, lddy, (const float*)h, ldh, (float*)dh, lddh, M, (int)F); }
  else
    { ADNM_PROF("gate_bwd", st, 2.0 * M * F * 5); gate_bwd_kernel<uint16_t><<<grid_for(M * F / 4), kBlock, 0, st>>>((const uint16_t*)dy, lddy, (const uint16_t*)h, ldh, (uint16_t*)dh, lddh, M, (int)F); }
  ADNM_CHECK_LAUNCH("gate_bwd");
  return ADNM_OK;
}

extern "C" int64_t adnm_igate_bwd_ws_bytes(int64_t n) { return (int64_t)(n / 4 / kBlock + 1 < 512 ? n / 4 / kBlock + 1 : 512) * 2 * sizeof(float); }

extern "C" int adnm_igate_fwd(const void* x, const float* enhance, const float* threshold, void* y, int64_t n, int dtype, adnm_stream_t stream) {
  ADNM_REQUIRE(x && enhance && threshold && y, "igate_fwd: null pointer");
  ADNM_REQUIRE(n > 0 && n % 4 == 0, "igate_fwd: element count %lld must be a positive multiple of 4", (long long)n);
  ADNM_REQUIRE(dtype == ADNM_F32 || dtype == ADNM_BF16, "igate_fwd: bad dtype %d", dtype);
  hipStream_t st = (hipStream_t)stream;
  ADNM_PROF("igate_fwd", st, (dtype == ADNM_F32 ? 8.0 : 4.0) * n);
  if (dtype == ADNM_F32) igate_fwd_kernel<float><<<grid_for(n / 4), kBlock, 0, st>>>((const float*)x, enhance, threshold, (float*)y, n / 4);
  else igate_fwd_kernel<uint16_t><<<grid_for(n / 4), kBlock, 0, st>>>((const uint16_t*)x, enhance, threshold, (uint16_t*)y, n / 4);
  ADNM_CHECK_LAUNCH("igate_fwd");
  return ADNM_OK;
}

extern "C" int adnm_igate_bwd(const void* dy, const void* x, const float* enhance, const float* threshold, void* dx, float* denhance,
                              float* dthreshold, void* ws, int64_t ws_bytes, int64_t n, int dtype, adnm_stream_t stream) {
  ADNM_REQUIRE(dy && x && enhance && threshold && dx && denhance && dthreshold, "igate_bwd: null pointer");
  ADNM_REQUIRE(n > 0 && n % 4 == 0, "igate_bwd: element count %lld must be a positive multiple of 4", (long long)n);
  ADNM_REQUIRE(dtype == ADNM_F32 || dtype == ADNM_BF16, "igate_bwd: bad dtype %d", dtype);
  if (!ws || ws_bytes < adnm_igate_bwd_ws_bytes(n)) {
    adnm_set_error("igate_bwd: workspace too small");
    return ADNM_EWORKSPACE;
  }
  hipStream_t st = (hipStream_t)stream;
  int64_t g = n / 4 / kBlock + 1;
  const unsigned grid = (unsigned)(g < 512 ? g : 512);
  {
    ADNM_PROF("igate_bwd", st, (dtype == ADNM_F32 ? 12.0 : 6.0) * n);
    if (dtype == ADNM_F32) igate_bwd_kernel<float><<<grid, kBlock, 0, st>>>((const float*)dy, (const float*)x, enhance, threshold, (float*)dx, (float*)ws, n / 4);
    else igate_bwd_kernel<uint16_t><<<grid, kBlock, 0, st>>>((const uint16_t*)dy, (const uint16_t*)x, enhance, threshold, (uint16_t*)dx, (float*)ws, n / 4);
  }
  adnm_launch_fold("igate_bwd_fold", (const float*)ws, (int)grid, 2, {denhance, 1}, {dthreshold, 1}, {nullptr, 0}, {nullptr, 0}, st);
  ADNM_CHECK_LAUNCH("igate_bwd");
  return ADNM_OK;
}

namespace {
__global__ __launch_bounds__(kBlock) void igate_res_fwd_kernel(const float* __restrict__ x, const float* __restrict__ res, const float* __restrict__ gama,
                                                               const float* __restrict__ enh, const float* __restrict__ thr, float* __restrict__ y,
                                                               int B, int L, int C4, int per_token) {
  const float a = *enh, t = *thr, gm = *gama;
  const int64_t n4 = (int64_t)B * L * C4;
  for (int64_t i = (int64_t)blockIdx.x * kBlock + threadIdx.x; i < n4; i += (int64_t)gridDim.x * kBlock) {
    const int c = (int)(i % C4), b = (int)(i / ((int64_t)L * C4));
    const float4 v = Io<float>::ld4(x + i * 4), r = Io<float>::ld4(res + (per_token ? i : (int64_t)b * C4 + c) * 4);
    Io<float>::st4(y + i * 4, make_float4(siluf_(a * (fmaf(gm, r.x, v.x) - t)), siluf_(a * (fmaf(gm, r.y, v.y) - t)),
                                          siluf_(a * (fmaf(gm, r.z, v.z) - t)), siluf_(a * (fmaf(gm, r.w, v.w) - t))));
  }
}

__global__ __launch_bounds__(kBlock) void igate_res_bwd_kernel(const float* __restrict__ dy, const float* __restrict__ x, const float* __restrict__ res,
                                                               const float* __restrict__ gama, const float* __restrict__ enh,
                                                               const float* __restrict__ thr, float* __restrict__ dx, float* __restrict__ dres,
                                                               float* __restrict__ spart, int B, int L, int C4, int per_token) {
  __shared__ float4 sm[16][16];
  __shared__ float ss[3][kBlock / 64];
  const float a = *enh, t = *thr, gm = *gama;
  const int chunks = (C4 + 15) / 16;
  const int b = blockIdx.x / chunks, cl = threadIdx.x & 15, sl = threadIdx.x >> 4;
  const int cq = (blockIdx.x % chunks) * 16 + cl;
  const bool valid = cq < C4;
  const int c = valid ? cq : 0;
  float4 r4 = Io<float>::ld4(res + (per_token ? 0 : ((int64_t)b * C4 + c) * 4));
  float dr[4] = {0.f, 0.f, 0.f, 0.f}, s_g = 0.f, s_e = 0.f, s_t = 0.f;
  for (int l = valid ? sl : L; l < L; l += 16) {
    const int64_t off = (((int64_t)b * L + l) * C4 + c) * 4;
    const float4 v = Io<float>::ld4(x + off), g = Io<float>::ld4(dy + off);
    if (per_token) r4 = Io<float>::ld4(res + off);
    const float rv[4] = {r4.x, r4.y, r4.z, r4.w};
    const float xv[4] = {v.x, v.y, v.z, v.w}, gv[4] = {g.x, g.y, g.z, g.w};
    float o[4];
#pragma unroll
    for (int k = 0; k < 4; ++k) {
      const float d = fmaf(gm, rv[k], xv[k]) - t, gp = gv[k] * silu_gradf_(a * d);
      o[k] = gp * a;
      dr[k] += o[k];
      s_g = fmaf(o[k], rv[k], s_g);
      s_e = fmaf(gp, d, s_e);
      s_t += gp;
    }
    Io<float>::st4(dx + off, make_float4(o[0], o[1], o[2], o[3]));
    if (per_token) Io<float>::st4(dres + off, make_float4(gm * o[0], gm * o[1], gm * o[2], gm * o[3]));
  }
  sm[sl][cl] = make_float4(dr[0], dr[1], dr[2], dr[3]);
  s_g = wave_sum(s_g), s_e = wave_sum(s_e), s_t = wave_sum(s_t);
  if ((threadIdx.x & 63) == 0) ss[0][threadIdx.x >> 6] = s_g, ss[1][threadIdx.x >> 6] = s_e, ss[2][threadIdx.x >> 6] = s_t;
  __syncthreads();
  if (sl == 0 && valid && !per_token) {
    float4 acc = sm[0][cl];
#pragma unroll
    for (int k = 1; k < 16; ++k) acc.x += sm[k][cl].x, acc.y += sm[k][cl].y, acc.z += sm[k][cl].z, acc.w += sm[k][cl].w;
    Io<float>::st4(dres + ((int64_t)b * C4 + c) * 4, make_float4(gm * acc.x, gm * acc.y, gm * acc.z, gm * acc.w));
  }
  if (threadIdx.x == 0) {
    float* sp = spart + (int64_t)blockIdx.x * 4;
    sp[0] = (ss[0][0] + ss[0][1]) + (ss[0][2] + ss[0][3]);
    sp[1] = (ss[1][0] + ss[1][1]) + (ss[1][2] + ss[1][3]);
    sp[2] = -a * ((ss[2][0] + ss[2][1]) + (ss[2][2] + ss[2][3]));
    sp[3] = 0.f;
  }
}
int64_t igate_res_blocks(int64_t B, int64_t C) { return B * adnm_cdiv(C / 4, 16); }
}

extern "C" int64_t adnm_igate_res_bwd_ws_bytes(int64_t B, int64_t L, int64_t C) {
  if (B < 1 || L < 1 || C < 4 || C % 4) return -1;
  return igate_res_blocks(B, C) * 4 * (int64_t)sizeof(float);
}

extern "C" int adnm_igate_res_fwd(const float* x, const float* res, int per_token, const float* gama, const float* enhance, const float* threshold,
                                  float* y, int64_t B, int64_t L, int64_t C, adnm_stream_t stream) {
  ADNM_REQUIRE(x && res && gama && enhance && threshold && y, "igate_res_fwd: null pointer");
  ADNM_REQUIRE(B > 0 && L > 0 && C > 0 && C % 4 == 0 && B * L * C < (1ll << 31), "igate_res_fwd: bad shape B=%lld L=%lld C=%lld (4 | C)", (long long)B,
               (long long)L, (long long)C);
  hipStream_t st = (hipStream_t)stream;
  ADNM_PROF("igate_fwd", st, 4.0 * (2.0 * B * L * C + B * C));
  igate_res_fwd_kernel<<<grid_for(B * L * C / 4), kBlock, 0, st>>>(x, res, gama, enhance, threshold, y, (int)B, (int)L, (int)(C / 4), per_token);
  ADNM_CHECK_LAUNCH("igate_res_fwd");
  return ADNM_OK;
}

extern "C" int adnm_igate_res_bwd(const float* dy, const float* x, const float* res, int per_token, const float* gama, const float* enhance,
                                  const float* threshold, float* dx, float* dres, float* dgama, float* denhance, float* dthreshold, void* ws, int64_t ws_bytes, int64_t B,
                                  int64_t L, int64_t C, adnm_stream_t stream) {
  ADNM_REQUIRE(dy && x && res && gama && enhance && threshold && dx && dres && dgama && denhance && dthreshold, "igate_res_bwd: null pointer");
  ADNM_REQUIRE(B > 0 && L > 0 && C > 0 && C % 4 == 0 && B * L * C < (1ll << 31), "igate_res_bwd: bad shape B=%lld L=%lld C=%lld (4 | C)", (long long)B,
               (long long)L, (long long)C);
  if (!ws || ws_bytes < adnm_igate_res_bwd_ws_bytes(B, L, C)) {
    adnm_set_error("igate_res_bwd: workspace %lld < %lld bytes", (long long)ws_bytes, (long long)adnm_igate_res_bwd_ws_bytes(B, L, C));
    return ADNM_EWORKSPACE;
  }
  hipStream_t st = (hipStream_t)stream;
  const int64_t blocks = igate_res_blocks(B, C);
  float* spart = (float*)ws;
  {
    ADNM_PROF("igate_bwd", st, 4.0 * (3.0 * B * L * C + 2.0 * B * C));
    igate_res_bwd_kernel<<<(unsigned)blocks, kBlock, 0, st>>>(dy, x, res, gama, enhance, threshold, dx, dres, spart, (int)B, (int)L, (int)(C / 4),
                                                               per_token);
// ... 175 lines not shown
```

adnm-unet_amd/models/ADNMUNet.py:

```python
import math
import os
from functools import partial

import torch
import torch.nn as nn
import torch.nn.functional as F

from adnm_hip import ops
from .ADNssd import Mamba2, StandardAttention
from .model_untils import *
from .model_untils import (BiasFree_LayerNorm, RMSNorm, Mlp, Swish, FeedForward, PatchEmbed, WTLayer, DownSample, UpSample,
                           Channel_Att_Bridge, EncoderToDecoder, OutProj, Conv2dLayer, DropPath, _hw)


def _merge(mod, x, residual, features):
    if residual is not None:
        x = ops.catmix(x, residual, features, mod.alpha1, mod.alpha2, mod.alpha3, mod.alpha4)
    elif features is not None:
        x = ops.lincomb([x, features], [None, mod.alpha3])
    return x


def _mix_normed(norm, xs, scalars, scale, shift, gamma=None):
    if isinstance(norm, (RMSNorm, BiasFree_LayerNorm)):
# ... 49 lines not shown
        if xn is None:
            xn, x = _normed(self.norm1_layers[0], x, self.scale1[0], self.shift1[0])
        for i in range(n):
            beta1, beta2 = (self.beta1, self.beta2) if n == 1 else (self.beta1[i:i + 1], self.beta2[i:i + 1])
            xn, x = _mix_normed(self.norm2_layers[i], [x, self.drop_path_layers[i](self.mixer_layers[i](xn, h, w))], [beta1, beta2],
                                self.scale2[i], self.shift2[i])
            f = self.ffns[i].forward_tokens(xn, h, w)
            if i + 1 < n:
                xn, x = _mix_normed(self.norm1_layers[i + 1], [x, f], [beta1, beta2], self.scale1[i + 1], self.shift1[i + 1])
            elif then is not None and self.dim == self.out_dim:
                return _mix_normed(then.norm1_layers[0], [x, f], [beta1, beta2], then.scale1[0], then.shift1[0], self.gamma)
            else:
                x = ops.lincomb([x, f], [beta1, beta2], self.gamma)
        if self.dim != self.out_dim:
            x = ops.linear(x, self.out_proj.weight, self.out_proj.bias)
        return x


class Attention(nn.Module):
    def __init__(self, dim, out_dim=None, headdim=4):
        super().__init__()
        self.dim = dim
        self.out_dim = out_dim or dim
        self.attn_norm1 = BiasFree_LayerNorm(dim)
        self.attn_norm2 = BiasFree_LayerNorm(dim)
        self.attn_layer = StandardAttention(dim, heads=dim // headdim, dim_head=headdim, dropout=0.)
        self.attn_mlp = Mlp(dim)
        self.attn_scale1 = nn.Parameter(torch.tensor(1.))
        self.attn_shift1 = nn.Parameter(torch.tensor(0.))
        self.attn_scale2 = nn.Parameter(torch.tensor(1.))
        self.attn_shift2 = nn.Parameter(torch.tensor(0.))
        if self.dim != self.out_dim:
            self.out_proj = nn.Linear(dim, out_dim)
        self.gamma = nn.Parameter(1 * torch.ones(dim))
        for n in ("alpha1", "alpha2", "alpha3", "alpha4", "beta1", "beta2", "beta3", "beta4"):
            setattr(self, n, nn.Parameter(torch.tensor(1, dtype=torch.float)))

    def forward(self, hidden_states, residual=None, features=None, inference_params=None, use_checkpoint=False):
        x = _merge(self, hidden_states, residual, features)
        b, l, d = x.shape
        h, w = _hw(l)
        xn, x = self.attn_norm1.tap(x, self.attn_scale1, self.attn_shift1)
        xn, x = self.attn_norm2.mix_tap([x, self.attn_layer(xn, h, w)], [self.beta1, self.beta2], self.attn_scale2, self.attn_shift2)
        x = ops.lincomb([x, self.attn_mlp(xn)], [self.beta3, self.beta4], self.gamma)
        if self.dim != self.out_dim:
            x = ops.linear(x, self.out_proj.weight, self.out_proj.bias)
        return x


def create_block(d_model, out_dim, headdim=None, ssm_cfg=None, num_layers=1, norm_epsilon=1e-5, drop_path=0., drop=0.,
                 rms_norm=True, residual_in_fp32=True, fused_add_norm=True, layer_idx=None, d_state=16, device=None, dtype=None):
    if ssm_cfg is None:
        ssm_cfg = {}
    if headdim is None:
        headdim = 4 if d_model <= 32 else 8 if d_model <= 256 else 16 if d_model <= 512 else 24 if d_model <= 768 else 32
    mixer = partial(Mamba2, layer_idx=layer_idx, d_model=d_model, headdim=headdim, linear_attn_duality=True, d_state=d_state, **ssm_cfg)
    norm_layer = partial(nn.LayerNorm if not rms_norm else RMSNorm, eps=norm_epsilon)
    block = Block(dim=d_model, out_dim=out_dim, mixer=mixer, num_layers=num_layers, norm_layer=norm_layer, drop_path=drop_path,
                  drop=drop, fused_add_norm=fused_add_norm, residual_in_fp32=residual_in_fp32)
    block.layer_idx = layer_idx
    return block


def _init_weights(module, n_layer, initializer_range=0.02, rescale_prenorm_residual=True, n_residuals_per_layer=1):
    if isinstance(module, nn.Linear):
        if module.bias is not None and not getattr(module.bias, "_no_reinit", False):
            nn.init.zeros_(module.bias)
    elif isinstance(module, nn.Embedding):
        nn.init.normal_(module.weight, std=initializer_range)
    if rescale_prenorm_residual:
        for name, p in module.named_parameters():
            if name in ("out_proj.weight", "fc2.weight"):
                nn.init.kaiming_uniform_(p, a=math.sqrt(5))
                with torch.no_grad():
                    p /= math.sqrt(n_residuals_per_layer * n_layer)


def segm_init_weights(m):
    if isinstance(m, nn.Linear):
        nn.init.trunc_normal_(m.weight, std=0.02, a=-2.0, b=2.0)
        if m.bias is not None:
            nn.init.constant_(m.bias, 0)
    elif isinstance(m, nn.LayerNorm):
        nn.init.constant_(m.bias, 0)
        nn.init.constant_(m.weight, 1.0)


class Encoder(nn.Module):
    def __init__(self, img_size=256, depth=[1, 1, 1], embed_dim=[64, 128, 128], headdim=8, in_channels=5, kernel=[5, 4, 3],
                 ratio=[2, 2, 2], wt_levels=[4, 3, 2], simple_patch=False, norm_epsilon=1e-5, ssm_cfg=None, InstanceNorm=True):
        super().__init__()
        if simple_patch:
            raise NotImplementedError("simple_patch=True is unused by create_ADNMUNet")
        self.img_size, self.depth, self.embed_dim = img_size, depth, embed_dim
        self.in_channels, self.kernel, self.ratio = in_channels, kernel, ratio
        self.encoder1 = PatchEmbed(img_size=img_size, patch_size=ratio[0], in_channels=in_channels, embed_dim=embed_dim[0],
                                   kernel=kernel[0], wt_levels=wt_levels[0], InstanceNorm=InstanceNorm)
        self.down_sample1 = DownSample(dim=embed_dim[0], ratio=ratio[0])
        self.encoder2 = WTLayer(embed_dim[0], embed_dim[1], kernel=kernel[1], wt_levels=wt_levels[1], InstanceNorm=InstanceNorm)
        self.down_sample2 = DownSample(dim=embed_dim[1], ratio=ratio[1])
        self.encoder3 = WTLayer(embed_dim[1], embed_dim[2], kernel=kernel[2], wt_levels=wt_levels[2], InstanceNorm=InstanceNorm)
        self.down_sample3 = DownSample(dim=embed_dim[2], ratio=ratio[2])
        self.attn = Attention(dim=embed_dim[2], headdim=headdim)
        blk = lambda i, n: create_block(d_model=embed_dim[i], out_dim=embed_dim[i + 1], headdim=headdim, num_layers=n,
                                        ssm_cfg=ssm_cfg, norm_epsilon=norm_epsilon)
        self.encoder4 = blk(2, depth[0])
        self.down_sample4 = DownSample(dim=embed_dim[3], ratio=ratio[3])
        self.encoder5 = blk(3, depth[1])
        self.down_sample5 = DownSample(dim=embed_dim[4], ratio=ratio[4])
        self.encoder6 = blk(4, depth[2])
        self.attn2 = Attention(embed_dim[5], headdim=headdim)

    def forward(self, x):
        x, lo, res = self.forward_lo(x)
        x, hi = self.forward_hi(x)
        return x, lo + hi, res

    def forward_lo(self, x):
        x = x.flatten(2).transpose(1, 2)
        skips = []
        x, res = self.encoder1(x)
        d, x = self.down_sample1.tap(x)
        skips.append(x)
        x = self.encoder2(d)
        d, x = self.down_sample2.tap(x)
        skips.append(x)
        x = self.encoder3(d)
        d, x = self.down_sample3.tap(x)
        skips.append(x)
        x = self.attn(d)
        skips.append(x)
        return x, skips, res

    def forward_hi(self, x):
        skips = []
        x = self.encoder4(x)
        d, x = self.down_sample4.tap(x)
        skips.append(x)
        x = self.encoder5(d)
        d, x = self.down_sample5.tap(x)
        skips.append(x)
        x = self.encoder6(d)
        skips.append(x)
        x = self.attn2(x)
        return x, skips

    def lo_modules(self):
        return [self.encoder1, self.down_sample1, self.encoder2, self.down_sample2, self.encoder3, self.down_sample3, self.attn]

    def hi_modules(self):
        return [self.encoder4, self.down_sample4, self.encoder5, self.down_sample5, self.encoder6, self.attn2]


class Decoder(nn.Module):
    def __init__(self, img_size=256, depth=[1, 1, 1], embed_dim=[64, 128, 128], headdim=8, refine_dim=[32, 32, 32], kernel=[5, 4, 3],
                 ratio=[2, 2, 2], wt_levels=[4, 3, 2], simple_patch=False, norm_epsilon=1e-5, ssm_cfg=None, InstanceNorm=True,
                 compute_dead_branches=False):
        super().__init__()
        self.img_size, self.depth, self.embed_dim, self.kernel, self.ratio = img_size, depth, embed_dim, kernel, ratio
        self.compute_dead_branches = compute_dead_branches
        blk = lambda d, o, n: create_block(d_model=d, out_dim=o, headdim=headdim, num_layers=n, ssm_cfg=ssm_cfg, norm_epsilon=norm_epsilon)
        self.decoder1 = blk(embed_dim[5], embed_dim[4], depth[2])
        self.up_sample1 = UpSample(dim=embed_dim[4], ratio=ratio[4])
        self.decoder2 = blk(embed_dim[4] * 2, embed_dim[3], depth[1])
        self.up_sample2 = UpSample(dim=embed_dim[3], ratio=ratio[3])
        self.decoder3 = blk(embed_dim[3] * 2, embed_dim[2], depth[0])
        self.attn = Attention(embed_dim[2], embed_dim[2], headdim=headdim)
        self.up_sample3 = UpSample(dim=embed_dim[2], ratio=ratio[2])
        self.decoder4 = WTLayer(embed_dim[2] * 2, embed_dim[1], kernel=kernel[2], wt_levels=wt_levels[2], if_res=True, InstanceNorm=InstanceNorm)
        self.up_sample4 = UpSample(dim=embed_dim[1], ratio=ratio[1])
        self.decoder5 = WTLayer(embed_dim[1] * 2, embed_dim[0], kernel=kernel[1], wt_levels=wt_levels[1], if_res=True, InstanceNorm=InstanceNorm)
        self.up_sample5 = UpSample(dim=embed_dim[0], ratio=ratio[0])
        self.decoder6 = WTLayer(embed_dim[0] * 2, embed_dim[0], kernel=kernel[0], wt_levels=wt_levels[0], if_res=True, InstanceNorm=InstanceNorm)
        self.decoder6_s = Conv2dLayer(embed_dim[0], refine_dim[0], kernel_size=1, stride=1, padding=0)
        c_list = list(embed_dim)
        c_list.insert(2, c_list[2])
        embed_dim.insert(2, embed_dim[2])
        self.fusion = Channel_Att_Bridge(c_list=c_list)
        self.e2ds = nn.ModuleList([EncoderToDecoder(embed_dim=c_list[len(c_list) - 1 - i], InstanceNorm=InstanceNorm)
                                   for i in range(len(c_list))])

    def forward(self, x, skips):
        skips, feats = self.forward_skips(skips)
        return self.forward_blocks(x, skips, feats)

    def forward_skips(self, skips):
        dead = self.compute_dead_branches
        aliases = []
        gates = self.fusion(skips, live=None if dead else {4, 5, 6}, alias_out=aliases)
        skips = aliases
        feats = [self.e2ds[i](x=skips[6 - i], res=gates[6 - i]) for i in range(7 if dead else 3)]
        return skips, feats

    def forward_blocks(self, x, skips, feats):
        f = lambda i: feats[i] if i < len(feats) else None
        x = self.up_sample1(self.decoder1(x, features=f(0)))
        x = self.up_sample2(self.decoder2(x, residual=skips[5], features=f(1)))
        x = self.decoder3(x, residual=skips[4], features=f(2))
        x = self.up_sample3(self.attn(x))
        x = self.up_sample4(self.decoder4(x, residual=skips[2], features=f(4)))
        x = self.up_sample5(self.decoder5(x, residual=skips[1], features=f(5)))
        x = self.decoder6(x, residual=skips[0], features=f(6))
        return self.decoder6_s.forward_tokens(x, self.img_size, self.img_size)

    def skip_modules(self):
        return [self.fusion, self.e2ds]

    def block_modules(self):
        return [self.decoder1, self.up_sample1, self.decoder2, self.up_sample2, self.decoder3, self.attn, self.up_sample3, self.decoder4,
                self.up_sample4, self.decoder5, self.up_sample5, self.decoder6, self.decoder6_s]


class Refiner(nn.Module):
    def __init__(self, img_size=256, refine_depth=[1, 1, 1, 1], refine_dim=[64, 128, 128], wt_levels=[4, 3, 2], out_channels=3,
                 refine_headdim=[4, 4, 4, 4], norm_epsilon=1e-5, out_expand=2, ssm_cfg=None, InstanceNorm=True):
        super().__init__()
        self.img_size, self.refine_depth = img_size, refine_depth
        blk = lambda i, o: create_block(d_model=refine_dim[i], out_dim=refine_dim[o], num_layers=refine_depth[i], ssm_cfg=ssm_cfg,
                                        norm_epsilon=norm_epsilon, headdim=refine_headdim[i])
        self.refiner1 = blk(0, 1)
        self.refiner2 = blk(1, 2)
        self.refiner3 = blk(2, 3)
        self.refiner4 = blk(3, -1)
        self.out_proj = OutProj(num_frames=out_channels, embed_dim=refine_dim[-1], img_size=[img_size, img_size],
                                wt_levels=wt_levels[0], out_expand=out_expand, InstanceNorm=InstanceNorm)

    def forward(self, x, res):
        x = self.refiner1(x, then=self.refiner2)
        x = self.refiner2(x, then=self.refiner3)
        x = self.refiner3(x, then=self.refiner4)
        return self.out_proj(self.refiner4(x), res)


class VisionMamba(nn.Module):
    def __init__(self, img_size=256, depth=[1, 1, 1], refine_depth=[1, 1], refine_dim=[32, 32, 32], refine_headdim=[8, 4],
                 embed_dim=[64, 128, 128], headdim=8, channels=5, out_channels=3, ssm_cfg=None, norm_epsilon=1e-5,
                 initializer_cfg=None, kernel=[5, 4, 3], ratio=[2, 2, 2], wt_levels=[4, 3, 2], out_expand=2, InstanceNorm=True,
                 simple_patch=False, e2d=True, compute_dead_branches=False, **kwargs):
        super().__init__()
        self.depth = depth
        self.encoder = Encoder(img_size=img_size, depth=depth, embed_dim=embed_dim, headdim=headdim, in_channels=channels, kernel=kernel,
                               ratio=ratio, wt_levels=wt_levels, simple_patch=simple_patch, norm_epsilon=norm_epsilon, InstanceNorm=InstanceNorm)
        self.decoder = Decoder(img_size=img_size, depth=depth, embed_dim=embed_dim, headdim=headdim, refine_dim=refine_dim, kernel=kernel,
                               ratio=ratio, wt_levels=wt_levels, norm_epsilon=norm_epsilon, InstanceNorm=InstanceNorm,
                               compute_dead_branches=compute_dead_branches)
        self.refiner = Refiner(img_size=img_size, refine_depth=refine_depth, refine_dim=refine_dim, refine_headdim=refine_headdim,
                               out_channels=out_channels, wt_levels=wt_levels, out_expand=out_expand, norm_epsilon=norm_epsilon,
                               InstanceNorm=InstanceNorm)
        self.apply(segm_init_weights)
        self.apply(partial(_init_weights, n_layer=len(depth), **(initializer_cfg if initializer_cfg is not None else {})))

    @torch.jit.ignore
    def no_weight_decay(self):
        return {"pos_embed", "cls_token", "temporal_pos_embedding"}

    def forward(self, x, mask=None):
        return self.forward_stage2(*self.forward_stage1(x))

    def forward_stages(self):
        enc, dec = self.encoder, self.decoder

        def s0(x):
            ops.prep_group(*enc.lo_modules())
            x, skips, res = enc.forward_lo(x.squeeze(2))
            return (x, res, *skips)

        def s1(x, res, *lo):
            ops.prep_group(*enc.hi_modules())
            x, hi = enc.forward_hi(x)
            return (x, res, *lo, *hi)

        def s2(x, res, *skips):
            skips, feats = dec.forward_skips(list(skips))
            return (x, res, *skips, *feats)

        def s3(x, res, *rest):
            ops.prep_group(*dec.block_modules())
            return (dec.forward_blocks(x, list(rest[:7]), list(rest[7:])), res)

        def s4(x, res):
            ops.prep_group(self.refiner)
            return (self.refiner(x, res).unsqueeze(2),)

        return [(s0, enc.lo_modules()), (s1, enc.hi_modules()), (s2, dec.skip_modules()), (s3, dec.block_modules()), (s4, [self.refiner])]

    def forward_stage1(self, x):
        ops.prep_group(self.encoder)
        x, skips, res = self.encoder(x.squeeze(2))
        return (x, res, *skips)

    def forward_stage2(self, x, res, *skips):
        ops.prep_group(self.decoder, self.refiner)
        return self.refiner(self.decoder(x, list(skips)), res).unsqueeze(2)

    def stage1_parameters(self):
        return self.encoder.parameters()


def get_scalar_parameters(model):
    return [p for p in model.parameters() if p.requires_grad and p.nelement() == 1]


def create_vm(img_size=256, depth=[1, 1, 1], refine_depth=[1, 1, 1, 1], refine_headdim=[4, 4, 4, 4], refine_dim=[32, 32, 32, 32],
              embed_dim=[32, 64, 128, 256, 512, 1024], headdim=4, channels=3, out_channels=3, ssm_cfg=None, norm_epsilon=1e-6,
              kernel=[5, 3, 3], ratio=[2, 2, 2, 2, 2, 2], wt_levels=[3, 1, 1], out_expand=2, InstanceNorm=True, initializer_cfg=None):
    return VisionMamba(img_size=img_size, depth=depth, refine_depth=refine_depth, refine_headdim=refine_headdim, refine_dim=refine_dim,
                       embed_dim=list(embed_dim), headdim=headdim, channels=channels, out_channels=out_channels, ssm_cfg=ssm_cfg,
                       norm_epsilon=norm_epsilon, initializer_cfg=initializer_cfg, kernel=kernel, ratio=ratio, wt_levels=wt_levels,
                       out_expand=out_expand, InstanceNorm=InstanceNorm)


def videomamba_middle(pretrained=False, **kwargs):
    model = create_vm(img_size=256, channels=5, norm_epsilon=1e-5, **kwargs)
    model.default_cfg = {}
    return model


def create_ADNMUNet(input_frames, output_frames, frame_interval, img_size=256, **overrides):
    refine_dim = [32, 32, 32, 32] if output_frames > 5 else [32, 32, 16, 16]
    if frame_interval < 120 / input_frames:
        InstanceNorm, kernel = True, [5, 5, 5]
    else:
        InstanceNorm, kernel = False, [5, 3, 3]
    model = VisionMamba(img_size=img_size, depth=[1, 1, 1], refine_depth=[1, 1, 1, 1], refine_headdim=[4, 4, 4, 4], refine_dim=refine_dim,
                        embed_dim=[32, 64, 128, 256, 512, 1024], headdim=4, channels=input_frames, out_channels=output_frames,
                        ssm_cfg=None, norm_epsilon=1e-6, initializer_cfg=None, kernel=kernel, ratio=[2, 2, 2, 2, 2, 2],
                        wt_levels=[3, 2, 1], out_expand=2, InstanceNorm=InstanceNorm, **overrides)
    if int(os.environ.get("WORLD_SIZE", "1")) > 1 and os.environ.get("ADNM_AUTO_DDP", "1") == "1":
        from adnm_hip import ddp
        ddp.attach(model)
    return model
```

adnm-unet_amd/models/model_untils.py:

```python
import math
import numbers

import torch
import torch.nn as nn
import torch.nn.functional as F

from adnm_hip import ops, lib
from models.WTConv2d import WTConv2d


def to_2tuple(x):
    return tuple(x) if isinstance(x, (tuple, list)) else (x, x)


def to_bchw(x):
    b, l, d = x.shape
    h = w = int(math.isqrt(l))
    return x.reshape(b, h, w, d).permute(0, 3, 1, 2)


def to_bld(x):
    return x.flatten(2).transpose(1, 2)


# ... 149 lines not shown
        if self._is_depthwise_same() and not self.norm and code is not None:
            x = ops.dwconv(x, self.conv.weight, self.conv.bias, h, w, code)
            fused_act = True
        elif self._is_depthwise_same():
            x = ops.dwconv(x, self.conv.weight, self.conv.bias, h, w, lib.ACT_NONE)
        elif self._is_pointwise():
            x = ops.linear(x, self.conv.weight.reshape(self.conv.out_channels, -1), self.conv.bias)
        elif self._is_dense3():
            fuse = not self.norm and code in (lib.ACT_NONE, lib.ACT_GELU)
            x = ops.conv3(x, self.conv.weight, self.conv.bias, h, w, code if fuse else lib.ACT_NONE)
            fused_act = fuse
        else:
            raise RuntimeError(f"Conv2dLayer: no HIP kernel for {self.conv} on tokens (depthwise 3x3/5x5, 1x1 and dense 3x3 'same' convs are implemented)")
        if self.norm:
            x, fused_act = self._norm_tokens(x, h, w, code)
        if self.act and not fused_act:
            x = _apply_act(self.act, x)
        return x

    def _norm_tokens(self, x, h, w, code):
        n = self.norm
        if isinstance(n, nn.InstanceNorm2d) and not n.affine and not n.track_running_stats and x.shape[-1] % 4 == 0:
            fuse = code in (lib.ACT_NONE, lib.ACT_GELU)
            return ops.instnorm(x, self.scale, self.shift, n.eps, code if fuse else lib.ACT_NONE), fuse
        raise RuntimeError(f"Conv2dLayer: no HIP kernel for the norm {n} on {x.shape[-1]} channels (affine-less InstanceNorm2d on a multiple "
                           "of 4 channels is implemented; the HIP path has no PyTorch fallback)")

    def _keeps_shape(self):
        c = self.conv
        if c.stride != (1, 1):
            return False
        if isinstance(c.padding, str):
            return c.padding == 'same'
        return all(2 * p == d * (k - 1) for p, d, k in zip(c.padding, c.dilation, c.kernel_size))

    def forward(self, x):
        if not self._keeps_shape():
            raise RuntimeError(f"Conv2dLayer: no HIP kernel for the shape-changing conv {self.conv} (stride-1 'same' convs are implemented; the HIP "
                               "path has no PyTorch fallback)")
        b, c, h, w = x.shape
        return nchw_view(self.forward_tokens(tokens_of(x), h, w), h, w)


class WTConvLayer(nn.Module):

    def __init__(self, in_channels, out_channels, kernel_size=3, stride=1, wt_levels=2, bias=True,
                 dropout=0, norm=None, act_func=None):
        super().__init__()
        self.dropout = nn.Dropout2d(dropout) if dropout > 0 else None
        self.conv = WTConv2d(in_channels, out_channels, kernel_size, stride, bias, wt_levels=wt_levels)
        self.norm = norm
        self.act = act_func() if act_func else None
        if norm:
            self.scale = nn.Parameter(torch.tensor(1.))
            self.shift = nn.Parameter(torch.tensor(0.))

    def forward_tokens(self, x, h, w, tap=False):
        if self.dropout:
            if self.training:
                raise RuntimeError("WTConvLayer: Dropout2d has no HIP kernel (the reference configuration uses dropout=0; no PyTorch fallback)")
        alias = None
        if tap:
            x, alias = self.conv.forward_tokens(x, h, w, tap=True)
        else:
            x = self.conv.forward_tokens(x, h, w)
        code = _act_code(self.act)
        fused = False
        if self.norm:
            n = self.norm
            if isinstance(n, nn.InstanceNorm2d) and not n.affine and x.shape[-1] % 4 == 0 and code in (lib.ACT_NONE, lib.ACT_GELU):
                x = ops.instnorm(x, self.scale, self.shift, n.eps, code)
                fused = True
            else:
                raise RuntimeError(f"WTConvLayer: no HIP kernel for the norm {n} with activation {self.act} on {x.shape[-1]} channels "
                                   "(affine-less InstanceNorm2d [+ GELU] on a multiple of 4 channels is implemented; no PyTorch fallback)")
        if self.act and not fused:
            x = _apply_act(self.act, x)
        return (x, alias) if tap else x

    def forward(self, x):
        b, c, h, w = x.shape
        y = nchw_view(self.forward_tokens(tokens_of(x), h, w), h, w)
        if self.conv.stride > 1:
            y = y[:, :, ::self.conv.stride, ::self.conv.stride]
        return y


class DeConv2dLayer(nn.Module):
    def __init__(self, in_channels, out_channels, ratio=4, kernel_size=(3, 3), groups=1,
                 bias=True, dropout=0, norm=None, act_func=None):
        super().__init__()
        padding_w = max(0, (kernel_size[1] - ratio + 1) // 2)
        output_padding_w = ratio - kernel_size[1] + 2 * padding_w
        if not (0 <= output_padding_w < ratio):
            raise ValueError(f"output_padding {output_padding_w} must satisfy 0 <= output_padding < {ratio}")
        self.dropout = nn.Dropout3d(dropout, inplace=False) if dropout > 0 else None
        self.trans_conv = nn.ConvTranspose2d(in_channels, out_channels, kernel_size, stride=(ratio, ratio),
                                             padding=(padding_w, padding_w),
                                             output_padding=(output_padding_w, output_padding_w), groups=groups, bias=bias)
        self.norm = norm if norm else None
        self.act = act_func() if act_func else None
        if norm:
            self.scale = nn.Parameter(torch.tensor(1.))
            self.shift = nn.Parameter(torch.tensor(0.))

    def adnm_nhwc_parameters(self):
        return [self.trans_conv.weight]

    def forward(self, x):
        c = self.trans_conv
        if (c.stride != (2, 2) or c.kernel_size != (3, 3) or c.padding != (1, 1) or c.output_padding != (1, 1) or c.groups != 1 or self.norm
                or self.act or self.dropout is not None):
            raise RuntimeError(f"DeConv2dLayer: the HIP transposed conv is k=3, s=2, p=1, output_padding=1 without norm/act, got {c} "
                               "(the HIP path has no PyTorch fallback)")
        b, ci, h, w = x.shape
        return nchw_view(ops.convt2x(tokens_of(x), c.weight, c.bias, h, w), 2 * h, 2 * w)


class FeedForward(nn.Module):

    def __init__(self, dim, ffn_expansion_factor=2, bias=True):
        super().__init__()
        hidden = int(dim * ffn_expansion_factor)
        self.project_in = Conv2dLayer(dim, hidden * 2, kernel_size=(1, 1), stride=(1, 1), padding=(0, 0), bias=bias)
        self.dwconv = Conv2dLayer(hidden * 2, hidden * 2, kernel_size=(3, 3), stride=(1, 1), padding=(1, 1),
                                  groups=hidden * 2, bias=bias)
        self.project_out = Conv2dLayer(hidden, dim, kernel_size=(1, 1), stride=(1, 1), padding=(0, 0), bias=bias)

    def forward_tokens(self, x, h, w):
        pi, dc, po = self.project_in.conv, self.dwconv.conv, self.project_out.conv
        return ops.feedforward(x, pi.weight.reshape(pi.out_channels, -1), pi.bias, dc.weight, dc.bias, po.weight.reshape(po.out_channels, -1), po.bias,
                               h, w)

    def forward(self, x):
        b, c, h, w = x.shape
        return nchw_view(self.forward_tokens(tokens_of(x), h, w), h, w)


class ConvFFD(nn.Module):
    def __init__(self, dim, bias=True):
        super().__init__()
        self.in_proj = nn.Linear(dim, dim * 2, bias=bias)
        self.dw_conv = Conv2dLayer(dim * 2, dim * 2, kernel_size=3, stride=1, padding=1, bias=bias, groups=dim * 2)
        self.out_proj = nn.Linear(dim * 2, dim, bias=bias)
        self.act = nn.GELU()

    def forward(self, x):
        b, l, d = x.shape
        h, w = _hw(l)
        x = ops.linear(x, self.in_proj.weight, self.in_proj.bias)
        c = self.dw_conv.conv
        x = ops.dwconv(x, c.weight, c.bias, h, w, lib.ACT_GELU)
        return ops.linear(x, self.out_proj.weight, self.out_proj.bias)


class PatchEmbed(nn.Module):
    def __init__(self, img_size=256, patch_size=2, in_channels=3, embed_dim=256, kernel=6, num_frames=5, target_frames=3,
                 wt_levels=2, ls_init_value=1, act=nn.GELU, InstanceNorm=True):
        super().__init__()
        img_size = to_2tuple(img_size)
        patch_size = to_2tuple(patch_size)
        self.num_patches = (img_size[1] // patch_size[1]) * (img_size[0] // patch_size[0])
        self.patches_resolution = [img_size[0] // patch_size[0], img_size[1] // patch_size[1]]
        self.img_size, self.patch_size = img_size, patch_size
        self.embed_dim, self.num_frames, self.target_frames = embed_dim, num_frames, target_frames
        self.gamma = nn.Parameter(ls_init_value * torch.ones(embed_dim)) if ls_init_value is not None else None
        self.conv1 = nn.Sequential(WTConvLayer(in_channels, in_channels, kernel_size=kernel, stride=1, bias=False,
                                               wt_levels=wt_levels, act_func=nn.GELU))
        self.conv2 = nn.Sequential(Conv2dLayer(in_channels, embed_dim, kernel_size=(3, 3), stride=(1, 1), padding=(1, 1),
                                               groups=1, bias=False, act_func=nn.GELU))
        self.conv3 = nn.Sequential(WTConvLayer(embed_dim, embed_dim, kernel_size=kernel, stride=1, bias=False, wt_levels=wt_levels,
                                               norm=nn.InstanceNorm2d(embed_dim) if InstanceNorm else nn.GroupNorm(4, embed_dim)))
        self.alpha1 = nn.Parameter(torch.tensor(1, dtype=torch.float))
        self.beta1 = nn.Parameter(torch.tensor(1, dtype=torch.float))
        self.alpha2 = nn.Parameter(torch.tensor(1, dtype=torch.float))
        self.beta2 = nn.Parameter(torch.tensor(1, dtype=torch.float))

    def forward(self, x):
        b, l, d = x.shape
        h, w = _hw(l)
        res = x[..., -1].reshape(b, h, w)
        x = ops.lincomb([self.conv1[0].forward_tokens(x, h, w).contiguous(), x.contiguous()], [self.alpha1, self.beta1])
        shortcut = self.conv2[0].forward_tokens(x, h, w)
        y, shortcut = self.conv3[0].forward_tokens(shortcut, h, w, tap=True)
        x = ops.lincomb([y, shortcut], [self.alpha2, self.beta2], self.gamma)
        return x, res


class WTLayer(nn.Module):
    def __init__(self, this_dim=128, next_dim=256, kernel=5, bias=True, wt_levels=2, ls_init_value=1, act=nn.GELU,
                 if_res=False, InstanceNorm=True):
        super().__init__()
        self.next_dim = next_dim
        norm_group = 8 if if_res else 4
        self.wtconv = WTConvLayer(this_dim, this_dim, kernel_size=kernel, stride=1, bias=bias, wt_levels=wt_levels,
                                  norm=nn.InstanceNorm2d(this_dim) if InstanceNorm else nn.GroupNorm(norm_group, this_dim))
        self.conv = Conv2dLayer(this_dim, next_dim, kernel_size=3, padding=1, stride=1, bias=True, act_func=nn.GELU)
        self.mlp = Mlp(this_dim)
        self.gamma = nn.Parameter(ls_init_value * torch.ones(this_dim)) if ls_init_value is not None else None
        self.alpha = nn.Parameter(torch.tensor(1, dtype=torch.float))
        self.beta = nn.Parameter(torch.tensor(1, dtype=torch.float))
        self.gama1 = nn.Parameter(torch.tensor(1, dtype=torch.float))
        self.gama2 = nn.Parameter(torch.tensor(1, dtype=torch.float))
        self.gama3 = nn.Parameter(torch.tensor(1, dtype=torch.float))
        self.gama4 = nn.Parameter(torch.tensor(1, dtype=torch.float))

    def forward(self, x, residual=None, features=None):
        if residual is not None:
            x = ops.catmix(x, residual, None, self.gama1, self.gama2)
        elif features is not None:
            x = ops.lincomb([x, features], [None, self.gama3])
        b, l, d = x.shape
        h, w = _hw(l)
        y, x = self.wtconv.forward_tokens(x, h, w, tap=True)
        x = ops.lincomb([y, x], [self.alpha, self.beta])
        x = self.mlp(x)
        if self.gamma is not None:
            x = ops.lincomb([x], [None], self.gamma)
        return self.conv.forward_tokens(x, h, w)


class DownSample(nn.Module):
    def __init__(self, dim=256, kernel=3, ratio=2):
        super().__init__()
        self.ratio = ratio
        self.dim = dim
        self.max_pool = nn.MaxPool2d(kernel_size=ratio, stride=ratio, padding=0)

    def forward(self, x, tap=False):
        b, l, d = x.shape
        h, w = _hw(l)
        if d % 4 or not 2 <= self.ratio <= 4:
            raise RuntimeError(f"DownSample: the HIP max-pool takes 4 | channels and ratio 2..4, got dim {d}, ratio {self.ratio}")
        return ops.maxpool(x, h, w, self.ratio, self.ratio, self.ratio, tap=tap)

    def tap(self, x):
        return self.forward(x, tap=True)


class UpSample(nn.Module):
    def __init__(self, dim=128, kernel=3, ratio=2, bias=True):
        super().__init__()
        self.ratio = ratio
        self.trans_conv = DeConv2dLayer(dim, dim, ratio=ratio, kernel_size=(kernel, kernel), bias=bias, act_func=None)

    def forward(self, x):
        b, l, d = x.shape
        h, w = _hw(l)
        tc = self.trans_conv
        c = tc.trans_conv
        if (self.ratio != 2 or c.kernel_size != (3, 3) or c.padding != (1, 1) or c.output_padding != (1, 1) or c.groups != 1 or tc.norm or tc.act
                or tc.dropout is not None):
            raise RuntimeError(f"UpSample: the HIP transposed conv is k=3, s=2, p=1, output_padding=1 without norm/act, got {c}")
        return ops.convt2x(x, c.weight, c.bias, h, w)


class IntensityGate(nn.Module):
    def __init__(self, threshold=0.):
        super().__init__()
        self.threshold = nn.Parameter(torch.tensor(threshold, dtype=torch.float))
        self.enhance = nn.Parameter(torch.tensor(1, dtype=torch.float))
        self.act = nn.SiLU()

    def forward(self, x):
        return ops.igate(x, self.enhance, self.threshold)


class Channel_Att_Bridge(nn.Module):

    def __init__(self, c_list=[8, 16, 32, 64, 128, 256], split_att='fc'):
        super().__init__()
        if split_att != 'fc':
            raise NotImplementedError("only split_att='fc' (the reference default) is implemented")
        c_list_sum = sum(c_list)
        self.split_att = split_att
        self.avgpool = nn.AdaptiveAvgPool2d(1)
        self.get_all_att = nn.Conv1d(1, 1, kernel_size=3, padding=1, bias=True)
        for i in range(7):
            setattr(self, f"att{i + 1}", nn.Linear(c_list_sum, c_list[i]))
        self.sigmoid1 = IntensityGate()

    def forward(self, t, live=None, alias_out=None):
        aliases, att = ops.bridge_pool([t[i] for i in range(len(t))])
        if alias_out is not None:
            alias_out[:] = aliases
        att = att.unsqueeze(1)
        att = ops.conv1d3(att, self.get_all_att.weight, self.get_all_att.bias)
        idx = [i for i in range(7) if live is None or i in live]
        lins = [getattr(self, f"att{i + 1}") for i in idx]
        gates = ops.bridge_heads(att, self.sigmoid1.enhance, self.sigmoid1.threshold, [l.weight for l in lins], [l.bias for l in lins])
        return dict(zip(idx, gates))


class EncoderToDecoder(nn.Module):

    def __init__(self, embed_dim=256, InstanceNorm=True):
        super().__init__()
        g = embed_dim // 4
        mk = lambda k, p: Conv2dLayer(embed_dim, embed_dim, kernel_size=k, stride=(1, 1), padding=p, bias=True, groups=g, act_func=nn.GELU)
        pw = lambda: Conv2dLayer(embed_dim, embed_dim, kernel_size=1, stride=1, padding=0, groups=embed_dim, bias=True)
        self.conv13pool = mk((1, 3), (0, 1))
        self.ffd13 = pw()
        self.act_func13 = IntensityGate()
        self.conv31pool = mk((3, 1), (1, 0))
        self.ffd31 = pw()
        self.act_func31 = IntensityGate()
        self.conv33pool = mk((3, 3), (1, 1))
        self.ffd33 = pw()
        self.act_func33 = IntensityGate()
        self.max_pool_13 = nn.MaxPool2d((1, 3), (1, 1), (0, 1))
        self.avg_pool_13 = nn.AvgPool2d((1, 3), (1, 1), (0, 1))
        self.max_pool_31 = nn.MaxPool2d((3, 1), (1, 1), (1, 0))
        self.avg_pool_31 = nn.AvgPool2d((3, 1), (1, 1), (1, 0))
        self.max_pool_33 = nn.MaxPool2d((3, 3), (1, 1), (1, 1))
        self.avg_pool_33 = nn.AvgPool2d((3, 3), (1, 1), (1, 1))
        self.conv33 = mk((3, 3), (1, 1))
        self.ffd = FeedForward(dim=embed_dim, bias=True)
        self.act = IntensityGate()
        self.norm = nn.InstanceNorm2d(embed_dim) if InstanceNorm else nn.GroupNorm(4, embed_dim)
        self.alpha1 = nn.Parameter(torch.tensor(0.33, dtype=torch.float))
        self.alpha2 = nn.Parameter(torch.tensor(0.33, dtype=torch.float))
        self.alpha3 = nn.Parameter(torch.tensor(0.33, dtype=torch.float))
        self.gama = nn.Parameter(torch.tensor(1, dtype=torch.float))
        self.gamma = nn.Parameter(1 * torch.ones(embed_dim))
        self.mlp = ConvFFD(embed_dim, bias=True)
        self.scale = nn.Parameter(torch.tensor(1.))
        self.shift = nn.Parameter(torch.tensor(0.))

    def forward(self, x, res):
        b, l, d = x.shape
        h, w = _hw(l)
        if not (isinstance(self.norm, nn.InstanceNorm2d) and d % 4 == 0):
            raise RuntimeError(f"EncoderToDecoder: the HIP kernels take InstanceNorm2d and a multiple of 4 channels, got {self.norm}, dim {d} "
                               "(the HIP path has no PyTorch fallback)")
        x = ops.igate_res(x, res, self.gama, self.act.enhance, self.act.threshold)
        x = ops.instnorm(x, self.scale, self.shift, self.norm.eps, lib.ACT_NONE)
        f13, f33 = self.ffd13.conv, self.ffd33.conv
        xp = ops.skipgate(x, h, w, (
            self.conv13pool.conv.weight, self.conv13pool.conv.bias, self.conv31pool.conv.weight, self.conv31pool.conv.bias,
            self.conv33pool.conv.weight, self.conv33pool.conv.bias, f13.weight.reshape(-1), f13.bias, f33.weight.reshape(-1), f33.bias,
            self.act_func13.enhance, self.act_func13.threshold, self.act_func33.enhance, self.act_func33.threshold,
            self.alpha1, self.alpha2, self.alpha3, self.gamma))
        return self.mlp(self.ffd.forward_tokens(xp, h, w))


class OutProj(nn.Module):
    def __init__(self, num_frames=3, embed_dim=256, img_size=[256, 256], act_func=Swish, wt_levels=2, ls_init_value=1,
                 out_expand=2, InstanceNorm=True):
        super().__init__()
        self.img_size = img_size
        self.embed_dim = embed_dim
        self.activation = act_func
        self.wtconv = WTConvLayer(embed_dim, embed_dim, kernel_size=5, stride=1, bias=False, wt_levels=3, act_func=nn.GELU,
                                  norm=nn.InstanceNorm2d(embed_dim) if InstanceNorm else nn.GroupNorm(4, embed_dim))
        self.conv = nn.Sequential(
            Conv2dLayer(embed_dim, embed_dim * out_expand, kernel_size=(3, 3), stride=(1, 1), padding=(1, 1), bias=False, act_func=nn.GELU),
            Conv2dLayer(embed_dim * out_expand, num_frames, kernel_size=(1, 1), stride=(1, 1), padding=(0, 0), bias=False, act_func=nn.GELU))
        self.conv2 = Conv2dLayer(num_frames, num_frames, kernel_size=3, stride=1, bias=False, act_func=self.activation)
        self.alpha1 = nn.Parameter(torch.tensor(1., dtype=torch.float))
        self.alpha2 = nn.Parameter(torch.tensor(1., dtype=torch.float))
        self.gamma = nn.Parameter(ls_init_value * torch.ones(embed_dim)) if ls_init_value is not None else None
        self.alpha = nn.Parameter(torch.tensor(1., dtype=torch.float))
        self.beta = nn.Parameter(torch.tensor(1., dtype=torch.float))

    def forward(self, x, residual):
        h, w = self.img_size[0], self.img_size[1]
        b, l, d = x.shape
        y, x = self.wtconv.forward_tokens(x, h, w, tap=True)
        x = ops.lincomb([y, x], [self.alpha, self.beta], self.gamma)
        x = self.conv[0].forward_tokens(x, h, w)
        x = self.conv[1].forward_tokens(x, h, w)
        if residual is not None:
            x = ops.lincomb([x, residual.reshape(b, l, 1).expand(b, l, x.shape[-1]).contiguous()], [self.alpha1, self.alpha2])
        x = self.conv2.forward_tokens(x, h, w)
        return nchw_view(x, h, w)
```

include/adnm_hip.h:

```cpp
#ifndef ADNM_HIP_H
#define ADNM_HIP_H

#include <stdint.h>
#include <stddef.h>

#ifdef __cplusplus
extern "C" {
#endif

typedef void* adnm_stream_t;

enum { ADNM_F32 = 0, ADNM_BF16 = 1 };
enum { ADNM_ACT_NONE = 0, ADNM_ACT_SILU = 1, ADNM_ACT_GELU = 2 };
enum { ADNM_OK = 0, ADNM_EINVAL = -1, ADNM_ELAUNCH = -2, ADNM_EWORKSPACE = -3 };
enum { ADNM_MFMA_F32 = 0, ADNM_MFMA_BF16 = 1, ADNM_MFMA_FP8 = 2, ADNM_MFMA_FP8_GRAD = 3 };
enum { ADNM_B_F32 = 0, ADNM_B_BF16 = 1, ADNM_B_FP8 = 2 };

int adnm_quant_update(float* table, int64_t n, float* state, float headroom, adnm_stream_t stream);

const char* adnm_last_error(void);
int adnm_abi_version(void);

int adnm_prof_enable(int on);
int64_t adnm_prof_collect(char* buf, int64_t buflen);

void* adnm_foldq_create(void);
int adnm_foldq_destroy(void* q);
int adnm_foldq_bind(void* q);
int64_t adnm_foldq_pending(void* q);
int adnm_foldq_flush(void* q, adnm_stream_t stream);
int adnm_foldq_clear(void* q);
int adnm_foldq_accumulate_next(int mask);

void* adnm_leafq_create(void);
int adnm_leafq_destroy(void* q);
int adnm_leafq_bind(void* q);
int64_t adnm_leafq_pending(void* q);
int adnm_leafq_flush(void* q, adnm_stream_t stream);
int adnm_leafq_clear(void* q);

int adnm_rownorm_fwd(const void* x, int64_t ldx, const float* w, const float* b, const float* scale,
                     const float* shift, void* y, int64_t ldy, float* mu, float* rstd, int64_t M, int64_t d,
                     float eps, int subtract_mean, int dtype, adnm_stream_t stream);
int64_t adnm_rownorm_bwd_ws_bytes(int64_t M, int64_t d);
int adnm_rownorm_bwd(const void* dy, int64_t lddy, const void* x, int64_t ldx, const float* w, const float* b,
                     const float* scale, const float* mu, const float* rstd, void* dx, int64_t lddx, float* dw,
                     float* db, float* dscale, float* dshift, const void* dres, int64_t lddres, void* ws, int64_t ws_bytes,
                     int64_t M, int64_t d, int subtract_mean, int dtype, adnm_stream_t stream);

int64_t adnm_ssd_ws_bytes(int64_t B, int64_t L, int64_t H, int64_t P, int64_t N, int64_t G);
int adnm_ssd_reduce_fwd(const void* x, int64_t ldx, const void* Bm, int64_t ldb, const void* Cm, int64_t ldc,
                        const void* dt_raw, int64_t lddt, int64_t dt_hstride, const float* dt_bias,
                        const float* A_log, const float* D, int64_t p_hstride, void* y, int64_t ldy, float* kv,
                        const float* ln_w, const float* ln_b, void* yn, int64_t ldyn, float* ln_mu, float* ln_rstd,
                        float ln_eps, void* ws, int64_t ws_bytes, int64_t B, int64_t L, int64_t H, int64_t P, int64_t N,
                        int64_t G, int dtype, adnm_stream_t stream);
int adnm_ssd_reduce_bwd(const void* dy, int64_t lddy, const void* x, int64_t ldx, const void* Bm, int64_t ldb,
                        const void* Cm, int64_t ldc, const void* dt_raw, int64_t lddt, int64_t dt_hstride,
                        const float* dt_bias, const float* A_log, const float* D, int64_t p_hstride,
                        const float* kv, void* dx, int64_t lddx, void* dBm, int64_t lddb, void* dCm, int64_t lddc,
                        void* ddt_raw, int64_t ldddt, float* ddt_bias, float* dA_log, float* dD, void* ws,
                        int64_t ws_bytes, int64_t B, int64_t L, int64_t H, int64_t P, int64_t N, int64_t G,
                        int dtype, adnm_stream_t stream);

int64_t adnm_ssd_scan_ws_bytes(int64_t B, int64_t L, int64_t H, int64_t N, int64_t chunk, int backward);
int adnm_ssd_scan_fwd(const void* x, int64_t ldx, int64_t x_hstride, const void* Bm, int64_t ldb, const void* Cm,
                      int64_t ldc, const void* dt_raw, int64_t lddt, int64_t dt_hstride, const float* dt_bias,
                      const float* A_log, const float* D, int64_t p_hstride, void* y, int64_t ldy, int64_t y_hstride,
                      float* S_in, void* ws, int64_t ws_bytes, int64_t B, int64_t L, int64_t H, int64_t P, int64_t N,
                      int64_t G, int64_t chunk, int reverse, int dtype, adnm_stream_t stream);
int adnm_ssd_scan_bwd(const void* dy, int64_t lddy, int64_t dy_hstride, const void* x, int64_t ldx, int64_t x_hstride,
                      const void* Bm, int64_t ldb, const void* Cm, int64_t ldc, const void* dt_raw, int64_t lddt,
                      int64_t dt_hstride, const float* dt_bias, const float* A_log, const float* D, int64_t p_hstride,
                      const float* S_in, void* dx, int64_t lddx, int64_t dx_hstride, void* dBm, int64_t lddb, void* dCm,
                      int64_t lddc, void* ddt_raw, int64_t ldddt, int64_t ddt_hstride, float* ddt_bias, float* dA_log,
                      float* dD, void* ws, int64_t ws_bytes, int64_t B, int64_t L, int64_t H, int64_t P, int64_t N,
                      int64_t G, int64_t chunk, int reverse, int dtype, adnm_stream_t stream);

int adnm_dwconv_fwd(const void* x, int64_t ldx, const float* wgt, const float* bias, const void* addend,
                    int64_t ldadd, void* y, int64_t ldy, int64_t B, int64_t H, int64_t W, int64_t C, int KH,
                    int KW, int act, int wlayout, int dtype, adnm_stream_t stream);
int64_t adnm_dwconv_bwd_ws_bytes(int64_t B, int64_t H, int64_t W, int64_t C, int KH, int KW);
int adnm_dwconv_bwd(const void* dy, int64_t lddy, const void* x, int64_t ldx, const float* wgt,
                    const float* bias, void* dpre, void* dx, int64_t lddx, float* dwgt, float* dbias, void* ws,
                    int64_t ws_bytes, int64_t B, int64_t H, int64_t W, int64_t C, int KH, int KW, int act,
                    int wlayout, int dtype, adnm_stream_t stream);
int adnm_dwconv_wgrad(const void* g, int64_t ldg, const void* x, int64_t ldx, float* dwgt, float* dbias, void* ws, int64_t ws_bytes,
                      int64_t B, int64_t H, int64_t W, int64_t C, int KH, int KW, int wlayout, int dtype, adnm_stream_t stream);

int adnm_haar_dwt(const void* x, int64_t ldx, int64_t cx, void* y, int64_t B, int64_t H, int64_t W, int64_t C,
                  int dtype, adnm_stream_t stream);
int adnm_wt_level(const float* x, int64_t ldx, int64_t cx, const float* taps, float* sub, float* tag, int64_t B, int64_t H, int64_t W,
                  int64_t C, int K, int flip, adnm_stream_t stream);
int adnm_haar_idwt(const void* s, const void* up1, const void* up2, const void* ll_add, const void* y_add1, const void* y_add2, void* y,
                   int64_t B, int64_t H, int64_t W, int64_t C, int dtype, adnm_stream_t stream);

int adnm_maxpool_fwd(const void* x, void* y, int64_t B, int64_t H, int64_t W, int64_t C, int kh, int kw, int stride,
                     int dtype, adnm_stream_t stream);
int adnm_maxpool_bwd(const void* dy, const void* x, const void* dx_add, void* dx, int64_t B, int64_t H, int64_t W, int64_t C, int kh,
                     int kw, int stride, int dtype, adnm_stream_t stream);

int64_t adnm_instnorm_ws_bytes(int64_t B, int64_t HW, int64_t C);
int adnm_instnorm_fwd(const void* x, const float* scale, const float* shift, void* y, float* mu, float* rstd,
                      void* ws, int64_t ws_bytes, int64_t B, int64_t HW, int64_t C, float eps, int act, int dtype,
                      adnm_stream_t stream);
int adnm_instnorm_bwd(const void* dy, const void* x, const float* scale, const float* shift, const float* mu,
                      const float* rstd, void* dx, float* dscale, float* dshift, void* ws, int64_t ws_bytes,
                      int64_t B, int64_t HW, int64_t C, int act, int dtype, adnm_stream_t stream);

int adnm_gate_fwd(const void* h, int64_t ldh, void* y, int64_t ldy, int64_t M, int64_t F, int dtype,
                  adnm_stream_t stream);
int adnm_gate_bwd(const void* dy, int64_t lddy, const void* h, int64_t ldh, void* dh, int64_t lddh, int64_t M,
                  int64_t F, int dtype, adnm_stream_t stream);

int adnm_igate_fwd(const void* x, const float* enhance, const float* threshold, void* y, int64_t n, int dtype,
                   adnm_stream_t stream);
int64_t adnm_igate_bwd_ws_bytes(int64_t n);
int adnm_igate_bwd(const void* dy, const void* x, const float* enhance, const float* threshold, void* dx, float* denhance,
                   float* dthreshold, void* ws, int64_t ws_bytes, int64_t n, int dtype, adnm_stream_t stream);
int adnm_igate_res_fwd(const float* x, const float* res, int per_token, const float* gama, const float* enhance,
                       const float* threshold, float* y, int64_t B, int64_t L, int64_t C, adnm_stream_t stream);
int64_t adnm_igate_res_bwd_ws_bytes(int64_t B, int64_t L, int64_t C);
int adnm_igate_res_bwd(const float* dy, const float* x, const float* res, int per_token, const float* gama, const float* enhance,
                       const float* threshold, float* dx, float* dres, float* dgama, float* denhance, float* dthreshold, void* ws,
                       int64_t ws_bytes, int64_t B, int64_t L, int64_t C, adnm_stream_t stream);


int adnm_skipgate_fwd(const float* x, const float* const* params, float* pooled, float* conv, float* out, int64_t B, int64_t H, int64_t W,
                      int64_t C, adnm_stream_t stream);
int64_t adnm_skipgate_grad_floats(int64_t C);
int64_t adnm_skipgate_bwd_ws_bytes(int64_t B, int64_t H, int64_t W, int64_t C);
int adnm_skipgate_bwd(const float* dout, const float* x, const float* const* params, const float* pooled, const float* conv, float* dx,
                      float* dparams, void* ws, int64_t ws_bytes, int64_t B, int64_t H, int64_t W, int64_t C, adnm_stream_t stream);

int adnm_attn4_fwd(const float* qkv, float* out, float* lse, int64_t B, int64_t L, int64_t heads, float scale, adnm_stream_t stream);
int adnm_attn4_bwd(const float* dout, const float* qkv, const float* out, const float* lse, float* dqkv, int64_t B, int64_t L, int64_t heads,
                   float scale, adnm_stream_t stream);

int adnm_emul_fwd(const float* a, int64_t lda, const float* b, int64_t ldb, float* y, int64_t M, int64_t C, adnm_stream_t stream);
int adnm_emul_bwd(const float* dy, const float* a, int64_t lda, const float* b, int64_t ldb, float* da, float* db, int64_t M, int64_t C,
                  adnm_stream_t stream);
int adnm_chancopy(const float* x, int64_t ldx, int64_t Cin, float* y, int64_t Cout, int64_t M, adnm_stream_t stream);
int adnm_conv1d3_fwd(const float* x, const float* w, const float* bias, float* y, int64_t B, int64_t n, adnm_stream_t stream);
int adnm_conv1d3_bwd(const float* dy, const float* x, const float* w, float* dx, float* dwb, int64_t B, int64_t n, adnm_stream_t stream);
int adnm_bridge_heads_fwd(const float* att, const float* const* W, const float* const* bias, const int64_t* C, int nheads,
                          const float* enhance, const float* threshold, float* const* z, float* const* y, int64_t B, int64_t S,
                          adnm_stream_t stream);
int64_t adnm_bridge_heads_bwd_ws_bytes(int64_t total, int64_t B, int64_t S);
int adnm_bridge_heads_bwd(const float* att, const float* const* W, const int64_t* C, int nheads, const float* enhance,
                          const float* threshold, const float* const* z, const float* const* dy, float* datt, float* const* dW,
                          float* const* dbias, float* denhance, float* dthreshold, void* ws, int64_t ws_bytes, int64_t B, int64_t S,
                          adnm_stream_t stream);

int64_t adnm_bridge_pool_ws_bytes(int64_t B, int64_t S);
int adnm_bridge_pool_fwd(int64_t n, const float* const* x, const int64_t* L, const int64_t* C, float* att, void* ws, int64_t ws_bytes, int64_t B,
                         adnm_stream_t stream);
int adnm_bridge_pool_bwd(int64_t n, const float* const* dxa, const float* datt, const int64_t* L, const int64_t* C, float* const* dx, int64_t B,
                         adnm_stream_t stream);

int64_t adnm_colsum_ws_bytes(int64_t rows, int64_t n);
int adnm_colsum(const float* x, float* out, int64_t rows, int64_t n, void* ws, int64_t ws_bytes, adnm_stream_t stream);

#define ADNM_SKGEMM_NT 0
#define ADNM_SKGEMM_NN 1
#define ADNM_SKGEMM_TN 2
int adnm_skgemm_supported(int op, int64_t M, int64_t N, int64_t K);
int64_t adnm_skgemm_ws_bytes(int op, int64_t M, int64_t N, int64_t K);
int adnm_skgemm(int op, const float* a, int64_t lda, const void* b, int64_t ldb, int b_dtype, const float* b_scale, const float* bias, float* c,
                int64_t ldc, float* dbias, void* ws, int64_t ws_bytes, void* slabs_uc, int64_t slabs_uc_bytes, int64_t M, int64_t N, int64_t K,
                int prec, float* q, adnm_stream_t stream);
int64_t adnm_skgemm_counter_bytes(int op, int64_t M, int64_t N, int64_t K);
void* adnm_uncached_alloc(int64_t bytes);
int adnm_uncached_free(void* ptr);

int64_t adnm_rainloss_ws_bytes(int64_t n);
int adnm_rainloss(const float* pred, const float* target, float* loss, float* grad, void* ws, int64_t ws_bytes, int64_t n, float omega_t,
                  float alpha, float gamma, adnm_stream_t stream);

int adnm_catmix_fwd(const void* x, int64_t ldx, const void* r, int64_t ldr, const void* f, int64_t ldf, const float* a1, const float* a2,
                    const float* a3, const float* a4, void* y, int64_t M, int64_t d, int dtype, adnm_stream_t stream);
int64_t adnm_catmix_bwd_ws_bytes(int64_t M, int64_t d);
int adnm_catmix_bwd(const void* dy, int64_t lddy, const void* x, int64_t ldx, const void* r, int64_t ldr, const void* f, int64_t ldf,
                    const float* a1, const float* a2, const float* a3, const float* a4, void* dx, void* dr, void* df, float* da, void* ws,
                    int64_t ws_bytes, int64_t M, int64_t d, int dtype, adnm_stream_t stream);

int adnm_lincomb_fwd(const void* x0, int64_t ld0, const void* x1, int64_t ld1, const void* x2, int64_t ld2,
                     const float* s0, const float* s1, const float* s2, const float* gamma, void* y, int64_t ldy,
                     int64_t M, int64_t C, int dtype, adnm_stream_t stream);
int64_t adnm_lincomb_bwd_ws_bytes(int64_t M, int64_t C);
int adnm_lincomb_bwd(const void* dy, int64_t lddy, const void* x0, int64_t ld0, const void* x1, int64_t ld1,
                     const void* x2, int64_t ld2, const float* s0, const float* s1, const float* s2,
                     const float* gamma, void* dx0, int64_t lddx0, void* dx1, int64_t lddx1, void* dx2, int64_t lddx2,
                     float* ds0, float* ds1, float* ds2, float* dgamma, void* ws, int64_t ws_bytes, int64_t M, int64_t C,
                     int dtype, adnm_stream_t stream);

int adnm_mixnorm_fwd(const float* x0, int64_t ld0, const float* x1, int64_t ld1, const float* s0, const float* s1, const float* gamma,
                     const float* w, const float* b, const float* scale, const float* shift, float* ymix, int64_t ldm, float* yn,
                     int64_t ldn, float* mu, float* rstd, int64_t M, int64_t d, float eps, int subtract_mean, adnm_stream_t stream);
int64_t adnm_mixnorm_bwd_ws_bytes(int64_t M, int64_t d);
int adnm_mixnorm_bwd(const float* dyn, int64_t lddyn, const float* dres, int64_t lddres, const float* x0, int64_t ld0, const float* x1,
                     int64_t ld1, const float* s0, const float* s1, const float* gamma, const float* w, const float* b, const float* scale,
                     const float* mu, const float* rstd, float* dx0, int64_t lddx0, float* dx1, int64_t lddx1, float* ds0, float* ds1,
                     float* dgamma, float* dw, float* db, float* dscale, float* dshift, void* ws, int64_t ws_bytes, int64_t M, int64_t d,
                     int subtract_mean, adnm_stream_t stream);

int64_t adnm_adamw_ws_bytes(void);
int adnm_adamw_step(float* p, const float* g, float* m, float* v, int64_t n, float* state, float lr, float beta1,
                    float beta2, float eps, float weight_decay, float max_norm, void* ws, int64_t ws_bytes, void* shadow, int shadow_dtype,
                    const int* seg_end, const int* seg_rec, int64_t nseg, float* wtab, const float* hyper, adnm_stream_t stream);
int adnm_shadow_refresh(const float* p, int64_t n, void* shadow, int shadow_dtype, const int* seg_end, const int* seg_rec, int64_t nseg,
                        float* wtab, int collect, adnm_stream_t stream);

int64_t adnm_conv3_ws_bytes(int64_t B, int64_t H, int64_t W, int64_t K, int64_t N);
int adnm_conv3_fwd(const float* in, int64_t ldin, const float* w, int64_t ws_n, int64_t ws_tap, int64_t ws_k, const float* bias,
                   float* out, int64_t ldo, float* pre, int64_t ldpre, void* ws, int64_t ws_bytes, int64_t B, int64_t H, int64_t W,
                   int64_t K, int64_t N, int act, int prec, float* q, adnm_stream_t stream);
int adnm_conv3_dgrad(const float* dout, int64_t lddo, const float* pre, int64_t ldpre, int act, const float* w, int64_t ws_n,
                     int64_t ws_tap, int64_t ws_k, float* din, int64_t lddin, void* ws, int64_t ws_bytes, int64_t B, int64_t H,
                     int64_t W, int64_t K, int64_t N, int prec, float* q, adnm_stream_t stream);
int64_t adnm_conv3_wgrad_ws_bytes(int64_t B, int64_t H, int64_t W, int64_t K, int64_t N);
int adnm_conv3_wgrad(const float* dout, int64_t lddo, const float* pre, int64_t ldpre, int act, const float* in, int64_t ldin,
                     float* dw, float* dbias, void* ws, int64_t ws_bytes, int64_t B, int64_t H, int64_t W, int64_t K, int64_t N,
                     int prec, adnm_stream_t stream);

int adnm_convt_col2im(const float* cols, int64_t ldc, int64_t col_tap_stride, int64_t col_c_stride, const float* bias, float* out,
                      int64_t ldo, int64_t B, int64_t H, int64_t W, int64_t C, adnm_stream_t stream);
int adnm_convt_im2col(const float* dout, int64_t lddo, float* dcols, int64_t ldc, int64_t col_tap_stride, int64_t col_c_stride,
                      int64_t B, int64_t H, int64_t W, int64_t C, adnm_stream_t stream);

int adnm_radar_ingest(const void* src_u8, float* dst, int64_t frames, int64_t H0, int64_t W0, int64_t S, float mul, adnm_stream_t stream);
int64_t adnm_eval_counts_ws_bytes(int64_t frames, int64_t hw, int64_t nthr);
int adnm_eval_counts(const float* truth, const float* pred, float* out, const float* thresholds_host, int64_t nthr, float value_scale,
                     void* ws, int64_t ws_bytes, int64_t frames, int64_t hw, adnm_stream_t stream);
int64_t adnm_eval_ssim_ws_bytes(int64_t frames, int64_t H, int64_t W);
int adnm_eval_ssim(const float* truth, const float* pred, float* out, float value_scale, void* ws, int64_t ws_bytes, int64_t frames,
                   int64_t H, int64_t W, adnm_stream_t stream);

int adnm_act_fwd(const float* x, float* y, int64_t n, int act, adnm_stream_t stream);
int adnm_act_bwd(const float* dy, const float* pre, float* dpre, int64_t n, int act, adnm_stream_t stream);
int adnm_swish_fwd(const float* x, const float* beta, float* y, int64_t n, adnm_stream_t stream);
int64_t adnm_swish_bwd_ws_bytes(int64_t n);
int adnm_swish_bwd(const float* dy, const float* x, const float* beta, float* dx, float* dbeta, void* ws, int64_t ws_bytes, int64_t n,
                   adnm_stream_t stream);

int adnm_cast_f32_bf16(const void* src, void* dst, int64_t n, float scale, adnm_stream_t stream);
int adnm_cast_bf16_f32(const void* src, void* dst, int64_t n, float scale, adnm_stream_t stream);

int adnm_tsgemm_supported(int64_t M, int64_t N, int64_t K);
int adnm_tsgemm_nt(const void* x, int64_t ldx, const float* w, int64_t ws_n, int64_t ws_k, const float* bias, void* y,
                   int64_t ldy, int64_t M, int64_t N, int64_t K, int prec, float* q, int x_dtype, int y_dtype, adnm_stream_t stream);
int adnm_tsgemm_tn_supported(int64_t M, int64_t N, int64_t K);
int64_t adnm_tsgemm_tn_ws_bytes(int64_t M, int64_t N, int64_t K);
int adnm_tsgemm_tn(const void* dy, int64_t lddy, const void* x, int64_t ldx, float* dw, float* dbias, void* ws,
                   int64_t ws_bytes, int64_t M, int64_t N, int64_t K, int dy_dtype, int x_dtype, adnm_stream_t stream);

int adnm_adnprep_fwd(float* const* params, float* const* prepped, int64_t d_model, int64_t d_inner, int64_t gn,
                     int64_t headdim, int64_t tap_ld, adnm_stream_t stream);
int64_t adnm_adnprep_bwd_ws_bytes(void);
int adnm_adnprep_bwd(float* const* params, float* const* gprepped, float* const* dparams, int64_t d_model,
                     int64_t d_inner, int64_t gn, int64_t headdim, int64_t tap_ld, void* ws, int64_t ws_bytes,
                     adnm_stream_t stream);
int adnm_wtprep_fwd(float* const* w, float* const* s, float* bias, float* const* taps, float* bias_t, int64_t C,
                    int64_t Cp, int64_t K, int64_t levels, adnm_stream_t stream);
int adnm_wtprep_bwd(float* const* w, float* const* s, float* bias, float* const* gtaps, float* gbias_t,
                    float* const* dw, float* const* ds, float* dbias, int64_t C, int64_t Cp, int64_t K, int64_t levels,
                    adnm_stream_t stream);
// ... 16 lines not shown
```

Measured before the change: 499.8 sequences/s.

## Group decoder skip-path depthwise conv and gate kernels into multi-problem launches

Adds grouped depthwise-conv and gated-activation kernels that take a table of up to eight independent problems in the kernel argument segment and dispatch blocks by prefix ranges. The decoder's encoder-to-decoder modules are routed through new forward_group paths so their feedforward and ConvFFD depthwise and gate stages run as single launches instead of one per module. This targets launch count and small-grid underutilization at low resolutions. It adds per-block problem lookup, a larger kernarg payload, and a requirement that all grouped problems share one storage dtype.

```diff
diff --git a/adnm-unet_amd/adnm_hip/ops.py b/adnm-unet_amd/adnm_hip/ops.py
--- a/adnm-unet_amd/adnm_hip/ops.py
+++ b/adnm-unet_amd/adnm_hip/ops.py
@@ -799,6 +799,46 @@
     return dx, dwt, db
 
 
+def k_dwconv_fwd_multi(xs, wts, biases, dims, K, act, chan_major=False):
+    _need_gpu(xs[0])
+    ys, ptrs, d = [], [], []
+    for x, wt, bias, (B, H, W, C) in zip(xs, wts, biases, dims):
+        y = torch.empty((B * H * W, C), dtype=x.dtype, device=x.device)
+        ys.append(y)
+        ptrs += [x, _f32(wt), _f32(bias), y]
+        d += [B, H, W, C, _rows(x)[1], C]
+    lib.call("adnm_dwconv_fwd_multi", len(xs), lib.ptr_table(ptrs), lib.i64_table(d), K, K, act, int(chan_major), _dt(xs[0]), _stream())
+    return ys
+
+
+def k_dwconv_bwd_multi(dys, xs, wts, biases, dims, K, act, chan_major=False):
+    dev = xs[0].device
+    dxs, dwts, dbs, dpres, ptrs, d = [], [], [], [], [], []
+    for dy, x, wt, bias, (B, H, W, C) in zip(dys, xs, wts, biases, dims):
+        dx = torch.empty((B * H * W, C), dtype=x.dtype, device=dev)
+        dpre = torch.empty((B * H * W, C), dtype=x.dtype, device=dev) if act != lib.ACT_NONE else None
+        dxs.append(dx)
+        dpres.append(dpre)
+        ptrs += [dy, x, wt, bias, dpre, dx]
+        d += [B, H, W, C, _rows(dy)[1], _rows(x)[1], C]
+    lib.call("adnm_dwconv_bwd_multi", len(xs), lib.ptr_table(ptrs), lib.i64_table(d), K, K, act, int(chan_major), _dt(xs[0]), _stream())
+    for dy, x, wt, bias, (B, H, W, C), dpre in zip(dys, xs, wts, biases, dims, dpres):
+        dwt = torch.empty((C, K * K) if chan_major else (K * K, C), dtype=torch.float32, device=dev)
+        db = torch.empty(C, dtype=torch.float32, device=dev) if bias is not None else None
+        dwts.append(dwt)
+        dbs.append(db)
+        nb = lib.query("adnm_dwconv_bwd_ws_bytes", B, H, W, C, K, K)
+        ws = _ws(nb, dev)
+        pdy, lddy = _rows(dy)
+        px, ldx = _rows(x)
+        g, ldg = (dpre.data_ptr(), C) if dpre is not None else (pdy, lddy)
+        pdw, pdb, dt_ = _p(dwt), _p(db), _dt(x)
+        SIDE.submit(dev, (dy, x, dpre), FOLDS.defer(dev, ws, dy, x, dpre), lambda g=g, ldg=ldg, px=px, ldx=ldx, pdw=pdw, pdb=pdb, ws=ws, nb=nb,
+                    B=B, H=H, W=W, C=C, dt_=dt_: lib.call("adnm_dwconv_wgrad", g, ldg, px, ldx, pdw, pdb, ws.data_ptr(), nb, B, H, W, C, K, K,
+                                                          int(chan_major), dt_, _stream()))
+    return dxs, dwts, dbs
+
+
 def k_haar_dwt(x, B, H, W, C, cx=1):
     _need_gpu(x)
     h2, w2 = (H + 1) // 2, (W + 1) // 2
@@ -885,6 +925,29 @@
     ph, ldh = _rows(h)
     lib.call("adnm_gate_bwd", pdy, lddy, ph, ldh, dh.data_ptr(), 2 * F, M, F, _dt(h), _stream())
     return dh
+
+
+def k_gate_fwd_multi(hs, Fs):
+    _need_gpu(hs[0])
+    ys, ptrs, d = [], [], []
+    for h, F in zip(hs, Fs):
+        y = torch.empty((h.shape[0], F), dtype=h.dtype, device=h.device)
+        ys.append(y)
+        ptrs += [h, y]
+        d += [h.shape[0], F, _rows(h)[1], F]
+    lib.call("adnm_gate_fwd_multi", len(hs), lib.ptr_table(ptrs), lib.i64_table(d), _dt(hs[0]), _stream())
+    return ys
+
+
+def k_gate_bwd_multi(dys, hs, Fs):
+    dhs, ptrs, d = [], [], []
+    for dy, h, F in zip(dys, hs, Fs):
+        dh = torch.empty((h.shape[0], 2 * F), dtype=h.dtype, device=h.device)
+        dhs.append(dh)
+        ptrs += [dy, h, dh]
+        d += [h.shape[0], F, _rows(dy)[1], _rows(h)[1], 2 * F]
+    lib.call("adnm_gate_bwd_multi", len(hs), lib.ptr_table(ptrs), lib.i64_table(d), _dt(hs[0]), _stream())
+    return dhs
 
 
 def tap_major(w):
@@ -1320,6 +1383,119 @@
         _unsupported("feedforward", f"is 1x1 d->4d, depthwise 3x3, gelu*sigmoid gate, 1x1 2d->d on fp32 (B, H*W, d) tokens with 8 | 4d, got "
                                     f"{x.dtype} {tuple(x.shape)}, weights {tuple(w_in.shape)}, {tuple(dw.shape)}, {tuple(w_out.shape)}")
     return FeedForwardFn.apply(x, w_in, b_in, dw, b_dw, w_out, b_out, H, W)
+
+
+class FeedForwardMultiFn(torch.autograd.Function):
+
+    @staticmethod
+    def forward(ctx, n, *args):
+        per = [args[9 * i:9 * i + 9] for i in range(n)]
+        x2s, w_ins, wts, h1s, metas, sts = [], [], [], [], [], []
+        for x, w_in, b_in, dw, b_dw, w_out, b_out, H, W in per:
+            B, L, d = x.shape
+            M = B * L
+            F4, F2 = w_in.shape[0], w_out.shape[1]
+            x2 = x.reshape(M, d)
+            x2 = x2 if x2.is_contiguous() else x2.contiguous()
+            w_in = w_in.contiguous()
+            wt = dw.reshape(F4, 9)
+            if wt.dtype != torch.float32 or not wt.is_contiguous():
+                wt = wt.contiguous().float()
+            st = low_storage(M, [(F4, d), (d, F4), (d, F2), (F2, d)])
+            h1s.append(k_linear(x2, w_in, b_in, out_dtype=st))
+            x2s.append(x2), w_ins.append(w_in), wts.append(wt), sts.append(st)
+            metas.append((B, L, d, H, W, F4, F2, dw.shape))
+        if len({t.dtype for t in h1s}) != 1:
+            _unsupported("feedforward (grouped)", "needs one storage type for the intermediates of every module")
+        h2s = k_dwconv_fwd_multi(h1s, wts, [p[4] for p in per], [(m[0], m[3], m[4], m[5]) for m in metas], 3, lib.ACT_NONE,
+                                 chan_major=True)
+        gs = k_gate_fwd_multi(h2s, [m[6] for m in metas])
+        outs, saved = [], []
+        for i, (x, w_in, b_in, dw, b_dw, w_out, b_out, H, W) in enumerate(per):
+            w_out = w_out.contiguous()
+            outs.append(k_linear(gs[i], w_out, b_out, out_dtype=x.dtype).view(metas[i][0], metas[i][1], w_out.shape[0]))
+            saved += [x2s[i], w_ins[i], b_in, wts[i], b_dw, w_out, b_out, h1s[i], h2s[i], gs[i]]
+        ctx.save_for_backward(*saved)
+        ctx.meta = metas
+        ctx.n = n
+        return tuple(outs)
+
+    @staticmethod
+    def backward(ctx, *douts):
+        n, metas = ctx.n, ctx.meta
+        sv = ctx.saved_tensors
+        per = [sv[10 * i:10 * i + 10] for i in range(n)]
+        dgs, grads = [], [None] * (9 * n)
+        for i, (x2, w_in, b_in, wt, b_dw, w_out, b_out, h1, h2, g) in enumerate(per):
+            B, L, d, H, W, F4, F2, dwshape = metas[i]
+            do = douts[i].reshape(B * L, w_out.shape[0])
+            do = do if do.is_contiguous() else do.contiguous()
+            dgs.append(k_linear_dx(do, w_out, out_dtype=g.dtype))
+            grads[9 * i + 5], grads[9 * i + 6] = k_linear_dw(do, g, b_out is not None, w_out.data_ptr(), b_out.data_ptr() if b_out is not None else 0)
+        dh2s = k_gate_bwd_multi(dgs, [p[8] for p in per], [m[6] for m in metas])
+        dh1s, dwts, dbs = k_dwconv_bwd_multi(dh2s, [p[7] for p in per], [p[3] for p in per], [p[4] for p in per],
+                                             [(m[0], m[3], m[4], m[5]) for m in metas], 3, lib.ACT_NONE, chan_major=True)
+        for i, (x2, w_in, b_in, wt, b_dw, w_out, b_out, h1, h2, g) in enumerate(per):
+            B, L, d, H, W, F4, F2, dwshape = metas[i]
+            if ctx.needs_input_grad[1 + 9 * i]:
+                grads[9 * i] = k_linear_dx(dh1s[i], w_in, out_dtype=x2.dtype).view(B, L, d)
+            grads[9 * i + 1], grads[9 * i + 2] = k_linear_dw(dh1s[i], x2, b_in is not None, w_in.data_ptr(),
+                                                             b_in.data_ptr() if b_in is not None else 0)
+            grads[9 * i + 3], grads[9 * i + 4] = dwts[i].view(dwshape), dbs[i]
+        return (None, *grads)
+
+
+def feedforward_multi(args):
+    for a in args:
+        x, w_in, b_in, dw, b_dw, w_out, b_out, H, W = a
+        _need_gpu(x)
+        F4, F2 = w_in.shape[0], w_out.shape[1]
+        if (x.dtype != torch.float32 or x.dim() != 3 or x.shape[1] != H * W or F4 != 2 * F2 or F2 % 4 or tuple(dw.shape) != (F4, 1, 3, 3)
+                or w_in.shape[1] != x.shape[-1]):
+            _unsupported("feedforward_multi", f"is 1x1 d->4d, depthwise 3x3, gelu*sigmoid gate, 1x1 2d->d on fp32 (B, H*W, d) tokens with 8 | 4d, "
+                                              f"got {x.dtype} {tuple(x.shape)}, weights {tuple(w_in.shape)}, {tuple(dw.shape)}, {tuple(w_out.shape)}")
+    return list(FeedForwardMultiFn.apply(len(args), *[t for a in args for t in a]))
+
+
+class DWConvMultiFn(torch.autograd.Function):
+
+    @staticmethod
+    def forward(ctx, n, act, *args):
+        per = [args[5 * i:5 * i + 5] for i in range(n)]
+        x2s, wts, dims, shapes = [], [], [], []
+        for x, w, bias, H, W in per:
+            B, L, C = x.shape
+            K = w.shape[-1]
+            x2 = x.reshape(B * L, C)
+            x2 = x2 if x2.stride(-1) == 1 else x2.contiguous()
+            wt = w.reshape(C, K * K)
+            if wt.dtype != torch.float32 or not wt.is_contiguous():
+                wt = wt.contiguous().float()
+            x2s.append(x2), wts.append(wt), dims.append((B, H, W, C)), shapes.append(w.shape)
+        ys = k_dwconv_fwd_multi(x2s, wts, [p[2] for p in per], dims, K, act, chan_major=True)
+        ctx.save_for_backward(*[t for i in range(n) for t in (x2s[i], wts[i], per[i][2])])
+        ctx.dims = (n, act, K, dims, shapes)
+        return tuple(y.view(p[0].shape) for y, p in zip(ys, per))
+
+    @staticmethod
+    def backward(ctx, *dys):
+        n, act, K, dims, shapes = ctx.dims
+        sv = ctx.saved_tensors
+        dy2s = []
+        for dy, (B, H, W, C) in zip(dys, dims):
+            dy2 = dy.reshape(B * H * W, C)
+            dy2s.append(dy2 if dy2.stride(-1) == 1 else dy2.contiguous())
+        dxs, dwts, dbs = k_dwconv_bwd_multi(dy2s, sv[0::3], sv[1::3], sv[2::3], dims, K, act, chan_major=True)
+        grads = []
+        for i, (B, H, W, C) in enumerate(dims):
+            grads += [dxs[i].view(B, H * W, C), dwts[i].view(shapes[i]), dbs[i], None, None]
+        return (None, None, *grads)
+
+
+def dwconv_multi(args, act=lib.ACT_NONE):
+    if len({a[1].shape[-1] for a in args}) != 1 or len({a[0].dtype for a in args}) != 1:
+        _unsupported("dwconv_multi", "takes problems of one kernel size and one storage type")
+    return list(DWConvMultiFn.apply(len(args), act, *[t for a in args for t in a]))
 
 
 class LinCombFn(torch.autograd.Function):
diff --git a/adnm-unet_amd/csrc/dwconv.hip b/adnm-unet_amd/csrc/dwconv.hip
--- a/adnm-unet_amd/csrc/dwconv.hip
+++ b/adnm-unet_amd/csrc/dwconv.hip
@@ -1,4 +1,6 @@
 #include "adnm_common.h"
+
+#include <vector>
 
 namespace {
 
@@ -84,16 +86,15 @@
 }
 
 template <typename T, int K, int MODE, bool WCM>
-__global__ __launch_bounds__(kBlock) void dwconv_kernel(const T* __restrict__ x, int64_t ldx, const float* __restrict__ wgt,
-                                                        const float* __restrict__ bias, const T* __restrict__ aux,
-                                                        int64_t ldaux, T* __restrict__ y, int64_t ldy, int B, int H, int W,
-                                                        int C, int act) {
+__device__ __forceinline__ void dwconv_body(const T* __restrict__ x, int64_t ldx, const float* __restrict__ wgt, const float* __restrict__ bias,
+                                            const T* __restrict__ aux, int64_t ldaux, T* __restrict__ y, int64_t ldy, int B, int H, int W, int C,
+                                            int act, unsigned blk, unsigned nblk) {
   constexpr int R = K / 2, N = CVec<T>::N, Q = CVec<T>::Q;
   using V = CVec<T>;
   const int C4 = C / N;
   const int WT = (W + TW - 1) / TW;
   const int64_t total = (int64_t)B * H * WT * C4;
-  const unsigned nb = gridDim.x, q8 = nb >> 3, r8 = nb & 7, xcd = blockIdx.x & 7, loc = blockIdx.x >> 3;
+  const unsigned nb = nblk, q8 = nb >> 3, r8 = nb & 7, xcd = blk & 7, loc = blk >> 3;
   const unsigned bid = (xcd < r8 ? xcd * (q8 + 1) : r8 * (q8 + 1) + (xcd - r8) * q8) + loc;
   const int64_t idx = (int64_t)bid * kBlock + threadIdx.x;
   if (idx >= total) return;
@@ -167,6 +168,41 @@
     }
     cv_st(y + pix * ldy + c, v);
   }
+}
+
+template <typename T, int K, int MODE, bool WCM>
+__global__ __launch_bounds__(kBlock) void dwconv_kernel(const T* __restrict__ x, int64_t ldx, const float* __restrict__ wgt,
+                                                        const float* __restrict__ bias, const T* __restrict__ aux,
+                                                        int64_t ldaux, T* __restrict__ y, int64_t ldy, int B, int H, int W,
+                                                        int C, int act) {
+  dwconv_body<T, K, MODE, WCM>(x, ldx, wgt, bias, aux, ldaux, y, ldy, B, H, W, C, act, blockIdx.x, gridDim.x);
+}
+
+constexpr int kMaxConv = 8;
+struct ConvProb {
+  const void* x;
+  const float* wgt;
+  const float* bias;
+  const void* aux;
+  void* y;
+  int64_t ldx, ldaux, ldy;
+  int B, H, W, C, act;
+};
+struct MultiConv {
+  int count, blk_end[kMaxConv];
+  ConvProb p[kMaxConv];
+};
+static_assert(sizeof(MultiConv) <= 4096, "MultiConv must fit the kernel argument segment");
+template <typename T, int K, int MODE, bool WCM>
+__global__ __launch_bounds__(kBlock) void dwconv_multi_kernel(MultiConv by_value) {
+  (void)by_value;
+  const auto& m = *(const __attribute__((address_space(4))) MultiConv*)__builtin_amdgcn_kernarg_segment_ptr();
+  int k = 0;
+  while (k + 1 < m.count && (int)blockIdx.x >= m.blk_end[k]) ++k;
+  const int beg = k ? m.blk_end[k - 1] : 0;
+  const auto& p = m.p[k];
+  dwconv_body<T, K, MODE, WCM>((const T*)p.x, p.ldx, p.wgt, p.bias, (const T*)p.aux, p.ldaux, (T*)p.y, p.ldy, p.B, p.H, p.W, p.C, p.act,
+                               blockIdx.x - beg, m.blk_end[k] - beg);
 }
 
 constexpr int kWgSlices = 2;
@@ -617,6 +653,34 @@
 #undef ADNM_DWCONV
 }
 
+template <typename T, int MODE>
+void launch_conv_multi(const ConvProb* probs, int64_t n, int K, int wcm, hipStream_t st) {
+  for (int64_t i = 0; i < n;) {
+    MultiConv m;
+    m.count = 0;
+    int blocks = 0;
+    double bytes = 0;
+    for (; i < n && m.count < kMaxConv; ++i) {
+      const ConvProb& p = probs[i];
+      m.p[m.count] = p;
+      blocks += (int)adnm_cdiv((int64_t)p.B * p.H * adnm_cdiv(p.W, TW) * (p.C / CVec<T>::N), kBlock);
+      m.blk_end[m.count++] = blocks;
+      bytes += (double)sizeof(T) * p.B * p.H * p.W * p.C * (MODE == 1 ? 3 : (p.aux ? 3 : 2));
+    }
+    for (int k = m.count; k < kMaxConv; ++k) m.blk_end[k] = blocks;
+    ADNM_PROF(K == 3 ? "dwconv_k3" : "dwconv_k5", st, bytes);
+#define ADNM_DWCONV_MULTI(KK, WCMV) dwconv_multi_kernel<T, KK, MODE, WCMV><<<(unsigned)blocks, kBlock, 0, st>>>(m)
+    if (K == 3) {
+      if (wcm) ADNM_DWCONV_MULTI(3, true);
+      else ADNM_DWCONV_MULTI(3, false);
+    } else {
+      if (wcm) ADNM_DWCONV_MULTI(5, true);
+      else ADNM_DWCONV_MULTI(5, false);
+    }
+#undef ADNM_DWCONV_MULTI
+  }
+}
+
 template <typename T>
 void launch_wgrad(const void* dpre, int64_t ldd, const void* x, int64_t ldx, float* part, float* dwgt, float* dbias, int64_t B, int64_t H,
                   int64_t W, int64_t C, int K, int wcm, hipStream_t st) {
@@ -730,6 +794,61 @@
   return ADNM_OK;
 }
 
+extern "C" int adnm_dwconv_fwd_multi(int64_t n, float* const* ptrs, const int64_t* dims, int KH, int KW, int act, int wlayout, int dtype,
+                                     adnm_stream_t stream) {
+  ADNM_REQUIRE(n > 0 && ptrs && dims, "dwconv_fwd_multi: %lld problems", (long long)n);
+  ADNM_REQUIRE(wlayout == 0 || wlayout == 1, "dwconv_fwd_multi: weight layout %d not in {0 tap-major, 1 channel-major}", wlayout);
+  const int al = dtype == ADNM_BF16 ? 8 : 4;
+  std::vector<ConvProb> probs((size_t)n);
+  for (int64_t i = 0; i < n; ++i) {
+    const float *x = ptrs[4 * i], *wgt = ptrs[4 * i + 1], *bias = ptrs[4 * i + 2], *y = ptrs[4 * i + 3];
+    const int64_t *d = dims + 6 * i, B = d[0], H = d[1], W = d[2], C = d[3], ldx = d[4], ldy = d[5];
+    if (int rc = check("dwconv_fwd_multi", x, B, H, W, C, KH, KW, act, dtype)) return rc;
+    ADNM_REQUIRE(wgt && y, "dwconv_fwd_multi: null pointer (problem %lld)", (long long)i);
+    ADNM_REQUIRE(ldx >= C && ldy >= C && ldx % al == 0 && ldy % al == 0 && ((uintptr_t)x | (uintptr_t)y) % 16 == 0,
+                 "dwconv_fwd_multi: pixel strides must be >= C, rows and strides 16-byte aligned (problem %lld)", (long long)i);
+    probs[i] = ConvProb{x, wgt, bias, nullptr, (void*)y, ldx, 0, ldy, (int)B, (int)H, (int)W, (int)C, act};
+  }
+  hipStream_t st = (hipStream_t)stream;
+  if (dtype == ADNM_F32) launch_conv_multi<float, 0>(probs.data(), n, KH, wlayout, st);
+  else launch_conv_multi<uint16_t, 0>(probs.data(), n, KH, wlayout, st);
+  ADNM_CHECK_LAUNCH("dwconv_fwd_multi");
+  return ADNM_OK;
+}
+
+extern "C" int adnm_dwconv_bwd_multi(int64_t n, float* const* ptrs, const int64_t* dims, int KH, int KW, int act, int wlayout, int dtype,
+                                     adnm_stream_t stream) {
+  ADNM_REQUIRE(n > 0 && ptrs && dims, "dwconv_bwd_multi: %lld problems", (long long)n);
+  ADNM_REQUIRE(wlayout == 0 || wlayout == 1, "dwconv_bwd_multi: weight layout %d not in {0 tap-major, 1 channel-major}", wlayout);
+  const int al = dtype == ADNM_BF16 ? 8 : 4;
+  std::vector<ConvProb> pre((size_t)n), flip((size_t)n);
+  for (int64_t i = 0; i < n; ++i) {
+    const float *dy = ptrs[6 * i], *x = ptrs[6 * i + 1], *wgt = ptrs[6 * i + 2], *bias = ptrs[6 * i + 3], *dpre = ptrs[6 * i + 4],
+                *dx = ptrs[6 * i + 5];
+    const int64_t *d = dims + 7 * i, B = d[0], H = d[1], W = d[2], C = d[3], lddy = d[4], ldx = d[5], lddx = d[6];
+    if (int rc = check("dwconv_bwd_multi", x, B, H, W, C, KH, KW, act, dtype)) return rc;
+    ADNM_REQUIRE(dy && wgt && dx, "dwconv_bwd_multi: null pointer (problem %lld)", (long long)i);
+    ADNM_REQUIRE(act == ADNM_ACT_NONE || dpre, "dwconv_bwd_multi: dpre scratch required when an activation is fused (problem %lld)", (long long)i);
+    ADNM_REQUIRE(ldx >= C && lddy >= C && lddx >= C && ldx % al == 0 && lddy % al == 0 && lddx % al == 0 &&
+                     ((uintptr_t)x | (uintptr_t)dy | (uintptr_t)dx | (uintptr_t)dpre) % 16 == 0,
+                 "dwconv_bwd_multi: pixel strides must be >= C, rows and strides 16-byte aligned (problem %lld)", (long long)i);
+    const void* g = act != ADNM_ACT_NONE ? (const void*)dpre : (const void*)dy;
+    const int64_t ldg = act != ADNM_ACT_NONE ? C : lddy;
+    pre[i] = ConvProb{x, wgt, bias, dy, (void*)dpre, ldx, lddy, C, (int)B, (int)H, (int)W, (int)C, act};
+    flip[i] = ConvProb{g, wgt, nullptr, nullptr, (void*)dx, ldg, 0, lddx, (int)B, (int)H, (int)W, (int)C, 0};
+  }
+  hipStream_t st = (hipStream_t)stream;
+  if (dtype == ADNM_F32) {
+    if (act != ADNM_ACT_NONE) launch_conv_multi<float, 1>(pre.data(), n, KH, wlayout, st);
+    launch_conv_multi<float, 2>(flip.data(), n, KH, wlayout, st);
+  } else {
+    if (act != ADNM_ACT_NONE) launch_conv_multi<uint16_t, 1>(pre.data(), n, KH, wlayout, st);
+    launch_conv_multi<uint16_t, 2>(flip.data(), n, KH, wlayout, st);
+  }
+  ADNM_CHECK_LAUNCH("dwconv_bwd_multi");
+  return ADNM_OK;
+}
+
 extern "C" int adnm_dwconv_wgrad(const void* g, int64_t ldg, const void* x, int64_t ldx, float* dwgt, float* dbias, void* ws, int64_t ws_bytes,
                                  int64_t B, int64_t H, int64_t W, int64_t C, int KH, int KW, int wlayout, int dtype, adnm_stream_t stream) {
   if (int rc = check("dwconv_wgrad", x, B, H, W, C, KH, KW, ADNM_ACT_NONE, dtype)) return rc;
diff --git a/adnm-unet_amd/csrc/elementwise.hip b/adnm-unet_amd/csrc/elementwise.hip
--- a/adnm-unet_amd/csrc/elementwise.hip
+++ b/adnm-unet_amd/csrc/elementwise.hip
@@ -1,14 +1,16 @@
 #include "adnm_common.h"
+
+#include <vector>
 
 namespace {
 constexpr int kBlock = 256;
 
 template <typename T>
-__global__ __launch_bounds__(kBlock) void gate_fwd_kernel(const T* __restrict__ h, int64_t ldh, T* __restrict__ y, int64_t ldy,
-                                                          int64_t M, int F) {
+__device__ __forceinline__ void gate_fwd_body(const T* __restrict__ h, int64_t ldh, T* __restrict__ y, int64_t ldy, int64_t M, int F, unsigned blk,
+                                              unsigned nblk) {
   const int F4 = F >> 2;
   const int64_t total = M * F4;
-  for (int64_t i = (int64_t)blockIdx.x * kBlock + threadIdx.x; i < total; i += (int64_t)gridDim.x * kBlock) {
+  for (int64_t i = (int64_t)blk * kBlock + threadIdx.x; i < total; i += (int64_t)nblk * kBlock) {
     const int64_t m = i / F4;
     const int f = (int)(i % F4) * 4;
     const float4 a = Io<T>::ld4(h + m * ldh + f), b = Io<T>::ld4(h + m * ldh + F + f);
@@ -18,11 +20,11 @@
 }
 
 template <typename T>
-__global__ __launch_bounds__(kBlock) void gate_bwd_kernel(const T* __restrict__ dy, int64_t lddy, const T* __restrict__ h, int64_t ldh,
-                                                          T* __restrict__ dh, int64_t lddh, int64_t M, int F) {
+__device__ __forceinline__ void gate_bwd_body(const T* __restrict__ dy, int64_t lddy, const T* __restrict__ h, int64_t ldh, T* __restrict__ dh,
+                                              int64_t lddh, int64_t M, int F, unsigned blk, unsigned nblk) {
   const int F4 = F >> 2;
   const int64_t total = M * F4;
-  for (int64_t i = (int64_t)blockIdx.x * kBlock + threadIdx.x; i < total; i += (int64_t)gridDim.x * kBlock) {
+  for (int64_t i = (int64_t)blk * kBlock + threadIdx.x; i < total; i += (int64_t)nblk * kBlock) {
     const int64_t m = i / F4;
     const int f = (int)(i % F4) * 4;
     const float4 a = Io<T>::ld4(h + m * ldh + f), b = Io<T>::ld4(h + m * ldh + F + f), g = Io<T>::ld4(dy + m * lddy + f);
@@ -37,6 +39,43 @@
     Io<T>::st4(dh + m * lddh + f, make_float4(d1[0], d1[1], d1[2], d1[3]));
     Io<T>::st4(dh + m * lddh + F + f, make_float4(d2[0], d2[1], d2[2], d2[3]));
   }
+}
+
+template <typename T>
+__global__ __launch_bounds__(kBlock) void gate_fwd_kernel(const T* __restrict__ h, int64_t ldh, T* __restrict__ y, int64_t ldy,
+                                                          int64_t M, int F) {
+  gate_fwd_body<T>(h, ldh, y, ldy, M, F, blockIdx.x, gridDim.x);
+}
+
+template <typename T>
+__global__ __launch_bounds__(kBlock) void gate_bwd_kernel(const T* __restrict__ dy, int64_t lddy, const T* __restrict__ h, int64_t ldh,
+                                                          T* __restrict__ dh, int64_t lddh, int64_t M, int F) {
+  gate_bwd_body<T>(dy, lddy, h, ldh, dh, lddh, M, F, blockIdx.x, gridDim.x);
+}
+
+constexpr int kMaxGate = 8;
+struct GateProb {
+  const void* dy;
+  const void* h;
+  void* out;
+  int64_t lddy, ldh, ldout, M;
+  int F;
+};
+struct MultiGate {
+  int count, blk_end[kMaxGate];
+  GateProb p[kMaxGate];
+};
+static_assert(sizeof(MultiGate) <= 4096, "MultiGate must fit the kernel argument segment");
+template <typename T, bool BWD>
+__global__ __launch_bounds__(kBlock) void gate_multi_kernel(MultiGate by_value) {
+  (void)by_value;
+  const auto& m = *(const __attribute__((address_space(4))) MultiGate*)__builtin_amdgcn_kernarg_segment_ptr();
+  int k = 0;
+  while (k + 1 < m.count && (int)blockIdx.x >= m.blk_end[k]) ++k;
+  const int beg = k ? m.blk_end[k - 1] : 0;
+  const auto& p = m.p[k];
+  if (BWD) gate_bwd_body<T>((const T*)p.dy, p.lddy, (const T*)p.h, p.ldh, (T*)p.out, p.ldout, p.M, p.F, blockIdx.x - beg, m.blk_end[k] - beg);
+  else gate_fwd_body<T>((const T*)p.h, p.ldh, (T*)p.out, p.ldout, p.M, p.F, blockIdx.x - beg, m.blk_end[k] - beg);
 }
 
 template <typename T>
@@ -233,6 +272,65 @@
   return ADNM_OK;
 }
 
+namespace {
+template <typename T, bool BWD>
+void launch_gate_multi(const GateProb* probs, int64_t n, hipStream_t st) {
+  for (int64_t i = 0; i < n;) {
+    MultiGate m;
+    m.count = 0;
+    int blocks = 0;
+    double bytes = 0;
+    for (; i < n && m.count < kMaxGate; ++i) {
+      m.p[m.count] = probs[i];
+      blocks += (int)grid_for(probs[i].M * probs[i].F / 4);
+      m.blk_end[m.count++] = blocks;
+      bytes += (double)sizeof(T) * probs[i].M * probs[i].F * (BWD ? 5 : 3);
+    }
+    for (int k = m.count; k < kMaxGate; ++k) m.blk_end[k] = blocks;
+    ADNM_PROF(BWD ? "gate_bwd" : "gate_fwd", st, bytes);
+    gate_multi_kernel<T, BWD><<<(unsigned)blocks, kBlock, 0, st>>>(m);
+  }
+}
+}
+
+extern "C" int adnm_gate_fwd_multi(int64_t n, float* const* ptrs, const int64_t* dims, int dtype, adnm_stream_t stream) {
+  ADNM_REQUIRE(n > 0 && ptrs && dims, "gate_fwd_multi: %lld problems", (long long)n);
+  ADNM_REQUIRE(dtype == ADNM_F32 || dtype == ADNM_BF16, "gate_fwd_multi: bad dtype %d", dtype);
+  std::vector<GateProb> probs((size_t)n);
+  for (int64_t i = 0; i < n; ++i) {
+    const float *h = ptrs[2 * i], *y = ptrs[2 * i + 1];
+    const int64_t *d = dims + 4 * i, M = d[0], F = d[1], ldh = d[2], ldy = d[3];
+    ADNM_REQUIRE(h && y, "gate_fwd_multi: null pointer (problem %lld)", (long long)i);
+    ADNM_REQUIRE(M > 0 && F > 0 && F % 4 == 0 && ldh >= 2 * F && ldy >= F && ldh % 4 == 0 && ldy % 4 == 0,
+                 "gate_fwd_multi: bad shape M=%lld F=%lld (problem %lld)", (long long)M, (long long)F, (long long)i);
+    probs[i] = GateProb{nullptr, h, (void*)y, 0, ldh, ldy, M, (int)F};
+  }
+  hipStream_t st = (hipStream_t)stream;
+  if (dtype == ADNM_F32) launch_gate_multi<float, false>(probs.data(), n, st);
+  else launch_gate_multi<uint16_t, false>(probs.data(), n, st);
+  ADNM_CHECK_LAUNCH("gate_fwd_multi");
+  return ADNM_OK;
+}
+
+extern "C" int adnm_gate_bwd_multi(int64_t n, float* const* ptrs, const int64_t* dims, int dtype, adnm_stream_t stream) {
+  ADNM_REQUIRE(n > 0 && ptrs && dims, "gate_bwd_multi: %lld problems", (long long)n);
+  ADNM_REQUIRE(dtype == ADNM_F32 || dtype == ADNM_BF16, "gate_bwd_multi: bad dtype %d", dtype);
+  std::vector<GateProb> probs((size_t)n);
+  for (int64_t i = 0; i < n; ++i) {
+    const float *dy = ptrs[3 * i], *h = ptrs[3 * i + 1], *dh = ptrs[3 * i + 2];
+    const int64_t *d = dims + 5 * i, M = d[0], F = d[1], lddy = d[2], ldh = d[3], lddh = d[4];
+    ADNM_REQUIRE(dy && h && dh, "gate_bwd_multi: null pointer (problem %lld)", (long long)i);
+    ADNM_REQUIRE(M > 0 && F > 0 && F % 4 == 0 && ldh >= 2 * F && lddh >= 2 * F && lddy >= F && ldh % 4 == 0 && lddh % 4 == 0 && lddy % 4 == 0,
+                 "gate_bwd_multi: bad shape M=%lld F=%lld (problem %lld)", (long long)M, (long long)F, (long long)i);
+    probs[i] = GateProb{dy, h, (void*)dh, lddy, ldh, lddh, M, (int)F};
+  }
+  hipStream_t st = (hipStream_t)stream;
+  if (dtype == ADNM_F32) launch_gate_multi<float, true>(probs.data(), n, st);
+  else launch_gate_multi<uint16_t, true>(probs.data(), n, st);
+  ADNM_CHECK_LAUNCH("gate_bwd_multi");
+  return ADNM_OK;
+}
+
 extern "C" int adnm_gate_bwd(const void* dy, int64_t lddy, const void* h, int64_t ldh, void* dh, int64_t lddh, int64_t M, int64_t F,
                              int dtype, adnm_stream_t stream) {
   ADNM_REQUIRE(dy && h && dh, "gate_bwd: null pointer");
diff --git a/adnm-unet_amd/models/ADNMUNet.py b/adnm-unet_amd/models/ADNMUNet.py
--- a/adnm-unet_amd/models/ADNMUNet.py
+++ b/adnm-unet_amd/models/ADNMUNet.py
@@ -225,6 +225,9 @@
         return [self.encoder4, self.down_sample4, self.encoder5, self.down_sample5, self.encoder6, self.attn2]
 
 
+E2D_GROUP = [os.environ.get("ADNM_E2D_GROUP", "1") != "0"]
+
+
 class Decoder(nn.Module):
     def __init__(self, img_size=256, depth=[1, 1, 1], embed_dim=[64, 128, 128], headdim=8, refine_dim=[32, 32, 32], kernel=[5, 4, 3],
                  ratio=[2, 2, 2], wt_levels=[4, 3, 2], simple_patch=False, norm_epsilon=1e-5, ssm_cfg=None, InstanceNorm=True,
@@ -262,7 +265,11 @@
         aliases = []
         gates = self.fusion(skips, live=None if dead else {4, 5, 6}, alias_out=aliases)
         skips = aliases
-        feats = [self.e2ds[i](x=skips[6 - i], res=gates[6 - i]) for i in range(7 if dead else 3)]
+        live = range(7 if dead else 3)
+        if E2D_GROUP[0]:
+            feats = EncoderToDecoder.forward_group([self.e2ds[i] for i in live], [skips[6 - i] for i in live], [gates[6 - i] for i in live])
+        else:
+            feats = [self.e2ds[i](x=skips[6 - i], res=gates[6 - i]) for i in live]
         return skips, feats
 
     def forward_blocks(self, x, skips, feats):
diff --git a/adnm-unet_amd/models/model_untils.py b/adnm-unet_amd/models/model_untils.py
--- a/adnm-unet_amd/models/model_untils.py
+++ b/adnm-unet_amd/models/model_untils.py
@@ -325,6 +325,13 @@
         c = self.dw_conv.conv
         x = ops.dwconv(x, c.weight, c.bias, h, w, lib.ACT_GELU)
         return ops.linear(x, self.out_proj.weight, self.out_proj.bias)
+
+    @staticmethod
+    def forward_group(mods, xs):
+        hw = [_hw(x.shape[1]) for x in xs]
+        hs = [ops.linear(x, m.in_proj.weight, m.in_proj.bias) for m, x in zip(mods, xs)]
+        hs = ops.dwconv_multi([(x, m.dw_conv.conv.weight, m.dw_conv.conv.bias, h, w) for m, x, (h, w) in zip(mods, hs, hw)], lib.ACT_GELU)
+        return [ops.linear(x, m.out_proj.weight, m.out_proj.bias) for m, x in zip(mods, hs)]
 
 
 class PatchEmbed(nn.Module):
@@ -516,6 +523,31 @@
             self.alpha1, self.alpha2, self.alpha3, self.gamma))
         return self.mlp(self.ffd.forward_tokens(xp, h, w))
 
+    @staticmethod
+    def forward_group(mods, xs, ress):
+        hw = [_hw(x.shape[1]) for x in xs]
+        xps = []
+        for m, x, res, (h, w) in zip(mods, xs, ress, hw):
+            d = x.shape[2]
+            if not (isinstance(m.norm, nn.InstanceNorm2d) and d % 4 == 0):
+                raise RuntimeError(f"EncoderToDecoder: the HIP kernels take InstanceNorm2d and a multiple of 4 channels, got {m.norm}, dim {d} "
+                                   "(the HIP path has no PyTorch fallback)")
+            x = ops.igate_res(x, res, m.gama, m.act.enhance, m.act.threshold)
+            x = ops.instnorm(x, m.scale, m.shift, m.norm.eps, lib.ACT_NONE)
+            f13, f33 = m.ffd13.conv, m.ffd33.conv
+            xps.append(ops.skipgate(x, h, w, (
+                m.conv13pool.conv.weight, m.conv13pool.conv.bias, m.conv31pool.conv.weight, m.conv31pool.conv.bias,
+                m.conv33pool.conv.weight, m.conv33pool.conv.bias, f13.weight.reshape(-1), f13.bias, f33.weight.reshape(-1), f33.bias,
+                m.act_func13.enhance, m.act_func13.threshold, m.act_func33.enhance, m.act_func33.threshold,
+                m.alpha1, m.alpha2, m.alpha3, m.gamma)))
+        ffs = []
+        for m, xp, (h, w) in zip(mods, xps, hw):
+            f = m.ffd
+            pi, dc, po = f.project_in.conv, f.dwconv.conv, f.project_out.conv
+            ffs.append((xp, pi.weight.reshape(pi.out_channels, -1), pi.bias, dc.weight, dc.bias, po.weight.reshape(po.out_channels, -1), po.bias,
+                        h, w))
+        return ConvFFD.forward_group([m.mlp for m in mods], ops.feedforward_multi(ffs))
+
 
 class OutProj(nn.Module):
     def __init__(self, num_frames=3, embed_dim=256, img_size=[256, 256], act_func=Swish, wt_levels=2, ls_init_value=1,
diff --git a/include/adnm_hip.h b/include/adnm_hip.h
--- a/include/adnm_hip.h
+++ b/include/adnm_hip.h
@@ -87,6 +87,10 @@
                     int wlayout, int dtype, adnm_stream_t stream);
 int adnm_dwconv_wgrad(const void* g, int64_t ldg, const void* x, int64_t ldx, float* dwgt, float* dbias, void* ws, int64_t ws_bytes,
                       int64_t B, int64_t H, int64_t W, int64_t C, int KH, int KW, int wlayout, int dtype, adnm_stream_t stream);
+int adnm_dwconv_fwd_multi(int64_t n, float* const* ptrs, const int64_t* dims, int KH, int KW, int act, int wlayout, int dtype,
+                          adnm_stream_t stream);
+int adnm_dwconv_bwd_multi(int64_t n, float* const* ptrs, const int64_t* dims, int KH, int KW, int act, int wlayout, int dtype,
+                          adnm_stream_t stream);
 
 int adnm_haar_dwt(const void* x, int64_t ldx, int64_t cx, void* y, int64_t B, int64_t H, int64_t W, int64_t C,
                   int dtype, adnm_stream_t stream);
@@ -112,6 +116,8 @@
                   adnm_stream_t stream);
 int adnm_gate_bwd(const void* dy, int64_t lddy, const void* h, int64_t ldh, void* dh, int64_t lddh, int64_t M,
                   int64_t F, int dtype, adnm_stream_t stream);
+int adnm_gate_fwd_multi(int64_t n, float* const* ptrs, const int64_t* dims, int dtype, adnm_stream_t stream);
+int adnm_gate_bwd_multi(int64_t n, float* const* ptrs, const int64_t* dims, int dtype, adnm_stream_t stream);
 
 int adnm_igate_fwd(const void* x, const float* enhance, const float* threshold, void* y, int64_t n, int dtype,
                    adnm_stream_t stream);
```

Measured after the change: 504.9 sequences/s, median of 6. 1.01x the previous value.
